# Ben-Bussch/Lunar_Module_Ascent_Trajectory_Optimiser

Measured on AMD Instinct MI355X. Metric: solved ascent NLPs/sec (N=200 collocation nodes), higher is better.
Workload: dtype f64; 1 GPU; BASELINE.json configs[2]: 4096-NLP Isp x dry-mass sweep (64x64, Isp 300-320 s, dry mass 2345-2545 kg), N=200 nodes, backward Euler (reference NODES=2), DCOST applied (the script's MV move penalty 1e-05, Launch_Optimiser.py:99, as an l1 term: the model the reference declares); move_penalty=True, batch_per_gpu=4096, global_batch=4096, n_nodes=200, parallelism=problem-sharded x1, gather only, converged=4096, of=4096

## Files before the change

### include/ascent.h

```cpp
#ifndef ASCENT_H
#define ASCENT_H
#include <stdint.h>

#ifdef __cplusplus
extern "C" {
#endif

typedef struct ascent_params {
  double G;
  double M;
  double R0;
  double Ft;
  double M0;
  double mdot;
  double fuel_mass;
  double mass_scalar;
  double ang_acc_max;
  double r_peri;
  double r_apo;
  double T_scale;
  double angle_ub;
  double tf_lb;
  double tf_ub;
  double dcost;
} ascent_params;

typedef struct ascent_opts {
  int32_t n_nodes;
  int32_t scheme;
  int32_t max_iter;
  int32_t warm_start;
  double tol;
  double mu_init;
  int32_t formulation;
  int32_t coarse_nodes;
  int32_t terminal;
  int32_t solver_path;
  int32_t move_penalty;
  int32_t reserved;
} ascent_opts;

enum ascent_status {
  ASCENT_OK = 0,
  ASCENT_E_ARG = -1,
  ASCENT_E_HIP = -2,
  ASCENT_E_NODEVICE = -3,
  ASCENT_E_NOMEM = -4,
  ASCENT_E_NOTERM = -5
};

enum ascent_problem_status {
  ASCENT_CONVERGED = 0,
  ASCENT_MAX_ITER = 1,
  ASCENT_LINESEARCH_FAILED = 2,
  ASCENT_REGULARISATION_FAILED = 3
};

#define ASCENT_BLOB_ROWS(n_nodes) (21 * ((n_nodes) - 1) + 10)
#define ASCENT_TRAJ_FIELDS 10

int ascent_version(void);
int ascent_device_count(void);
const char *ascent_strerror(int code);

int ascent_solve_batch(const ascent_params *p, int64_t batch, const ascent_opts *o,
                       const double *guess_or_null, double *traj_out, double *tf_out,
                       int32_t *status_out, int32_t *iters_out, double *sol_blob_out_or_null,
                       int device_id, void *hip_stream_or_null, int ptr_is_device);

int ascent_eval_nodes(const ascent_params *p, int64_t batch, const ascent_opts *o,
                      const double *iterate, double *defects, double *jac_blocks,
                      double *hess_blocks, int device_id);

int ascent_kkt_step(const ascent_params *p, int64_t batch, const ascent_opts *o,
                    const double *iterate, const double *mu, const double *delta_w, double *step,
                    int32_t *inertia_out, int device_id);

enum ascent_path { ASCENT_PATH_AUTO = 0, ASCENT_PATH_FUSED = 1, ASCENT_PATH_SPLIT_LANE = 2, ASCENT_PATH_SPLIT_WIDE = 3,
                   ASCENT_PATH_DENSE = 4,
                   ASCENT_PATH_PERSIST = 5  };
int ascent_default_path(int64_t batch, const ascent_opts *o);
int ascent_workspace_layout(int64_t batch, const ascent_opts *o, int64_t *out4);
int ascent_eval_nodes_path(const ascent_params *p, int64_t batch, const ascent_opts *o,
                           const double *iterate, double *defects, double *jac_blocks,
                           double *hess_blocks, int device_id, int path);
int ascent_kkt_step_path(const ascent_params *p, int64_t batch, const ascent_opts *o,
                         const double *iterate, const double *mu, const double *delta_w, double *step,
                         int32_t *inertia_out, int device_id, int path);

int ascent_dense_records(const ascent_params *p, int64_t batch, const ascent_opts *o, const double *iterate,
                         double *records, int device_id);

int ascent_coast_batch(const ascent_params *p, int64_t batch, const double *final_state, int32_t coast_nodes,
                       double *coast_traj, double *coast_tf, double *apsides, int device_id,
                       void *hip_stream_or_null, int ptr_is_device);

int ascent_param_sensitivity(const ascent_params *p, int64_t batch, const ascent_opts *o,
                             const double *sol_blob, double *grad_out,
                             int device_id, void *hip_stream_or_null, int ptr_is_device);

#define ASCENT_FLIGHT_ROWS 10
#define ASCENT_FLIGHT_MAX_SUBSTEPS 4096
int ascent_fly_batch(const ascent_params *p, int64_t batch, const ascent_opts *o, const double *sol_blob,
                     int32_t substeps, double *flown_traj_out_or_null, double *local_err_out_or_null,
                     double *summary_out, int device_id, void *hip_stream_or_null, int ptr_is_device);

int ascent_flight_jacobian(const ascent_params *p, int64_t batch, const ascent_opts *o, const double *sol_blob,
                           int32_t substeps, double *jac_out, double *jac_u_out_or_null, int device_id,
                           void *hip_stream_or_null, int ptr_is_device);

#define ASCENT_TRIM_ROWS 10
int ascent_trim_batch(const ascent_params *p, int64_t batch, const ascent_opts *o, const double *sol_blob, int32_t substeps,
                      int32_t rounds, double tol, double *trim_blob_out, double *summary_out, int device_id,
                      void *hip_stream_or_null, int ptr_is_device);

#define ASCENT_DISPERSE_COLS 24
#define ASCENT_DISPERSE_ROWS 9
#define ASCENT_DISPERSE_STAT_ROWS 82
#define ASCENT_DISPERSE_MAX_SAMPLES 65536
int ascent_disperse_batch(const ascent_params *p, int64_t batch, const ascent_opts *o, const double *sol_blob,
                          int32_t substeps, int32_t samples, const double *xi, const double *sigma,
                          const double *sigma_u_or_null, double *stats_out, double *samples_out_or_null, int device_id,
                          void *hip_stream_or_null, int ptr_is_device);

#define ASCENT_GUIDE_ROWS 5
int ascent_guidance_gains(const ascent_params *p, int64_t batch, const ascent_opts *o, const double *sol_blob, int32_t substeps,
                          const double *weights, double *gain_u_out, double *gain_t_out, double *summary_out,
                          double *jac_cl_out_or_null, double *jac_u_cl_out_or_null, int device_id, void *hip_stream_or_null,
                          int ptr_is_device);

#define ASCENT_GUIDED_SAMPLE_ROWS 12
int ascent_disperse_guided_batch(const ascent_params *p, int64_t batch, const ascent_opts *o, const double *sol_blob,
                                 int32_t substeps, int32_t samples, const double *xi, const double *sigma,
                                 const double *sigma_u_or_null, const double *gain_u, const double *gain_t_or_null,
                                 const double *stretch_max_or_null, double *stats_out, double *samples_out_or_null,
                                 int device_id, void *hip_stream_or_null, int ptr_is_device);

int ascent_kkt_solve(int64_t batch, int32_t n_nodes, int32_t bs, int32_t nb, const double *diag, const double *lower,
                     const double *upper, const double *border, const double *border_diag, const double *rhs,
                     double *sol, int device_id, int algo);

double ascent_last_kernel_ms(int device_id);

#ifdef __cplusplus
}
#endif
#endif
```

### lunar_module_ascent_trajectory_optimiser_amd/csrc/ascent_dense.hip

```cpp
#include <hip/hip_runtime.h>

#include <cstdio>
#include <cstdlib>

#include "ascent.h"
#include "ascent_device.hpp"
#include "ascent_tile.hpp"
#include "ascent_dense.hpp"
#include "ascent_blocktri.hpp"
#include "ascent_flight_dev.hpp"

using namespace ascent;

namespace {

constexpr int NIT = 26;
constexpr int O_Z = 0, O_U = 7, O_L = 8, O_ZB = 15;
constexpr int O_LU = 21, O_PP = 22, O_PN = 23, O_ZP = 24, O_ZN = 25;
constexpr int NV_GA = 0, NV_GB = 8, NV_P = 16, NNV = 27;
constexpr int G_JA = 0, G_JB = 1, G_HAA = 2, G_HAB = 3, G_HBB = 4, G_V = 5, NGRID = 6;
constexpr int F_EA = 0, F_LA = 1, F_EL2 = 2, F_GAIN = 3;
constexpr int FWD_DOUBLES = 3 * 64 + 16;
enum {
  X_STATE, X_ITERS, X_STATUS, X_CUR, X_FIRST, X_LS, X_MU, X_NUP, X_DWL, X_ALPHA, X_ADU, X_PHI0, X_DM, X_C1, X_SL,
  X_S,
  X_D = X_S + 10,
  X_T = X_D + 10,
  X_REFAC = X_T + 10, X_RTH, X_DW, X_MV,
  NSCAL = 64
};
enum { ST_TRIAL = 0, ST_NEWTON = 1, ST_DONE = 3 };

struct DGeo {
  int K, scheme, terminal, dc;
  __host__ __device__ size_t nlp_doubles() const {
    return (size_t)K * (3 * NIT + NNV + NGRID * 64 + FWD_DOUBLES) + NSCAL;
  }
  __host__ __device__ size_t off_it(int buf) const { return (size_t)buf * NIT * K; }
  __host__ __device__ size_t off_st() const { return (size_t)2 * NIT * K; }
  __host__ __device__ size_t off_nv() const { return (size_t)3 * NIT * K; }
  __host__ __device__ size_t off_rec() const { return (size_t)(3 * NIT + NNV) * K; }
  __host__ __device__ size_t off_fwd() const { return off_rec() + (size_t)K * NGRID * 64; }
  __host__ __device__ size_t off_sc() const { return off_fwd() + (size_t)K * FWD_DOUBLES; }
};

ASC_DEV Scal load_scal(const double *sc, int r0) {
  Scal s;
  s.th = sc[r0 + S_TH]; s.zlt = sc[r0 + S_ZLT]; s.zut = sc[r0 + S_ZUT]; s.s1 = sc[r0 + S_S1]; s.s2 = sc[r0 + S_S2];
  s.zs1 = sc[r0 + S_ZS1]; s.zs2 = sc[r0 + S_ZS2]; s.nu3 = sc[r0 + S_NU3]; s.nu1 = sc[r0 + S_NU1]; s.nu2 = sc[r0 + S_NU2];
  return s;
}
ASC_DEV void store_scal(double *sc, int r0, const Scal &s) {
  sc[r0 + S_TH] = s.th; sc[r0 + S_ZLT] = s.zlt; sc[r0 + S_ZUT] = s.zut; sc[r0 + S_S1] = s.s1; sc[r0 + S_S2] = s.s2;
  sc[r0 + S_ZS1] = s.zs1; sc[r0 + S_ZS2] = s.zs2; sc[r0 + S_NU3] = s.nu3; sc[r0 + S_NU1] = s.nu1; sc[r0 + S_NU2] = s.nu2;
}
ASC_DEV Scal trial_scal(const Der &d, const Scal &s, const Scal &ds, double alpha, double adu, double mu, bool first) {
  Scal t = s;
  if (first) return t;
  t.th += alpha * ds.th; t.s1 += alpha * ds.s1; t.s2 += alpha * ds.s2;
  t.nu3 += alpha * ds.nu3; t.nu1 += alpha * ds.nu1; t.nu2 += alpha * ds.nu2;
  t.zlt = clipz(s.zlt + adu * ds.zlt, t.th - d.tlb, mu);
  t.zut = clipz(s.zut + adu * ds.zut, d.tub - t.th, mu);
  t.zs1 = clipz(s.zs1 + adu * ds.zs1, t.s1, mu);
  t.zs2 = clipz(s.zs2 + adu * ds.zs2, t.s2, mu);
  return t;
}

__global__ __launch_bounds__(WAVE) void d_init(const ascent_params *params, long batch, DGeo g, double *ws,
                                               const double *guess, int warm, double mu_init, int probe,
                                               const double *probe_mu) {
  const long p = blockIdx.y;
  const int k = blockIdx.x * WAVE + threadIdx.x, K = g.K;
  if (k >= K) return;
  double *w = ws + (size_t)p * g.nlp_doubles();
  const Der d = derive_t(params[p], g.terminal);
  const int asked_warm = warm;
  if (warm && !(guess[(21L * K + S_TH) * batch + p] > 0.0)) warm = 0;
  const double tf0 = 0.9, dr = 0.166, aend = 0.5, vp = sqrt(d.vp2), dt0 = (1.0 / K) * d.T * tf0;
  const double sdr = sin(dr), cdr = cos(dr);
  const double xf = -d.rhof * sdr, yf = d.rhof * cdr - d.rho0;
  double z[7], l[7], zb[6], u;
  if (warm) {
    ASC_UNROLL
    for (int i = 0; i < 7; i++) {
      z[i] = guess[(7L * k + i) * batch + p];
      l[i] = guess[(8L * K + 7L * k + i) * batch + p];
    }
    u = guess[(7L * K + k) * batch + p];
    ASC_UNROLL
    for (int b = 0; b < 6; b++) zb[b] = guess[(15L * K + 6L * k + b) * batch + p];
  } else {
    const double fr = (double)(k + 1) / K;
    z[IX] = fr * xf; z[IY] = fr * yf; z[IVX] = -fr * vp * cdr; z[IVY] = -fr * vp * sdr; z[IA] = fr * aend;
    z[IW] = aend / (K * dt0); z[IM] = d.mrate * dt0 * (k + 1);
    u = 0.0;
  }
  if (!probe) {
    z[IA] = push_in(z[IA], 0.0, d.aub);
    z[IM] = push_in(z[IM], 0.0, 1.0);
    u = push_in(u, -1.0, 1.0);
  }
  ASC_UNROLL
  for (int b = 0; b < 6; b++) zb[b] = warm == 2 ? (probe ? zb[b] : fmax(zb[b], 1e-12)) : 1.0;
  ASC_UNROLL
  for (int i = 0; i < 7; i++) l[i] = warm == 2 ? l[i] : 0.0;
  double *it = w + g.off_it(0), *st = w + g.off_st();
  ASC_UNROLL
  for (int i = 0; i < 7; i++) { it[(O_Z + i) * K + k] = z[i]; it[(O_L + i) * K + k] = l[i]; }
  it[O_U * K + k] = u;
  ASC_UNROLL
  for (int b = 0; b < 6; b++) it[(O_ZB + b) * K + k] = zb[b];
  for (int r = 0; r < NIT; r++) st[r * K + k] = 0.0;
  if (g.dc) {
    double up = (k > 0 && warm) ? guess[(7L * K + k - 1) * batch + p] : 0.0;
    if (k > 0 && !probe) up = push_in(up, -1.0, 1.0);
    const double dl = u - up, eps = warm ? 1e-4 : 1e-2, dc = params[p].dcost;
    it[O_LU * K + k] = 0.0;
    it[O_PP * K + k] = fmax(dl, 0.0) + eps; it[O_PN * K + k] = fmax(-dl, 0.0) + eps;
    it[O_ZP * K + k] = dc; it[O_ZN * K + k] = dc;
  }
  if (k != K - 1) return;
  double *sc = w + g.off_sc();
  Scal s;
  if (warm) {
    const double *gs = guess + (21L * K) * batch + p;
    s.th = gs[S_TH * batch]; s.zlt = gs[S_ZLT * batch]; s.zut = gs[S_ZUT * batch]; s.s1 = gs[S_S1 * batch];
    s.s2 = gs[S_S2 * batch]; s.zs1 = gs[S_ZS1 * batch]; s.zs2 = gs[S_ZS2 * batch]; s.nu3 = gs[S_NU3 * batch];
    s.nu1 = gs[S_NU1 * batch]; s.nu2 = gs[S_NU2 * batch];
  } else {
    s.th = tf0;
  }
  if (!probe) s.th = push_in(s.th, d.tlb, d.tub);
  const Terminal tm = terminal_of(d, z);
  if (probe) {
  } else if (warm != 2) {
    s.s1 = fmax(tm.g1, 1e-2); s.s2 = fmax(tm.g2, 1e-2);
    s.zlt = s.zut = s.zs1 = s.zs2 = 1.0;
    s.nu3 = s.nu1 = s.nu2 = 0.0;
  } else {
    s.s1 = fmax(s.s1, 1e-10); s.s2 = fmax(s.s2, 1e-10);
    s.zlt = fmax(s.zlt, 1e-12); s.zut = fmax(s.zut, 1e-12);
    s.zs1 = fmax(s.zs1, 1e-12); s.zs2 = fmax(s.zs2, 1e-12);
  }
  for (int r = 0; r < NSCAL; r++) sc[r] = 0.0;
  store_scal(sc, X_S, s);
  sc[X_STATE] = ST_TRIAL; sc[X_FIRST] = 1.0; sc[X_STATUS] = ASCENT_MAX_ITER;
  sc[X_MU] = probe ? probe_mu[p] : ((asked_warm && !warm) ? 0.1 : mu_init);
  sc[X_NUP] = 1.0;
}

struct QMap { int q; double c; };

ASC_DEV void h4_full(const double *H10, double H4[4][4]) {
  H4[0][0] = H10[0]; H4[0][1] = H4[1][0] = H10[1]; H4[0][2] = H4[2][0] = H10[2]; H4[0][3] = H4[3][0] = H10[3];
  H4[1][1] = H10[4]; H4[1][2] = H4[2][1] = H10[5]; H4[1][3] = H4[3][1] = H10[6];
  H4[2][2] = H10[7]; H4[2][3] = H4[3][2] = H10[8]; H4[3][3] = H10[9];
}

__global__ __launch_bounds__(WAVE) void d_eval(const ascent_params *params, long batch, DGeo g, double *ws) {
  const long p = blockIdx.y;
  const int k = blockIdx.x * WAVE + threadIdx.x, K = g.K;
  double *w = ws + (size_t)p * g.nlp_doubles();
  double *sc = w + g.off_sc();
  if ((int)sc[X_STATE] != ST_TRIAL || k >= K) return;
  const Der d = derive_t(params[p], g.terminal);
  const bool first = sc[X_FIRST] != 0.0;
  const double alpha = first ? 0.0 : sc[X_ALPHA], adu = first ? 0.0 : sc[X_ADU], mu = sc[X_MU];
  const Scal s = load_scal(sc, X_S), ds = load_scal(sc, X_D);
  const Scal stt = trial_scal(d, s, ds, alpha, adu, mu, first);
  const int cur = (int)sc[X_CUR];
  const double *ic = w + g.off_it(cur), *st = w + g.off_st();
  double *in = w + g.off_it(1 - cur), *nv = w + g.off_nv(), *rec = w + g.off_rec() + (size_t)k * NGRID * 64;
  const double hT = (1.0 / K) * d.T, dt = hT * stt.th;
  const double wa = g.scheme == 0 ? 0.0 : g.scheme == 1 ? 0.5 : 1.0 / 6.0;
  const double wm = g.scheme == 2 ? 4.0 / 6.0 : 0.0;
  const double wb = g.scheme == 0 ? 1.0 : g.scheme == 1 ? 0.5 : 1.0 / 6.0;
  const double sa = dt * wa, sm = dt * wm, sb = dt * wb, e8 = 0.125 * dt, h8 = 0.125 * hT;
  double za[7], zb[7], lam[7], zbd[6], u;
  ASC_UNROLL
  for (int i = 0; i < 7; i++) {
    zb[i] = ic[(O_Z + i) * K + k] + alpha * st[(O_Z + i) * K + k];
    za[i] = k ? ic[(O_Z + i) * K + k - 1] + alpha * st[(O_Z + i) * K + k - 1] : 0.0;
    lam[i] = ic[(O_L + i) * K + k] + alpha * st[(O_L + i) * K + k];
  }
  u = ic[O_U * K + k] + alpha * st[O_U * K + k];
  const double dist[6] = {zb[IA], d.aub - zb[IA], zb[IM], 1.0 - zb[IM], u + 1.0, 1.0 - u};
  const double mlo = mu * 1e-10, mhi = mu * 1e10;
  ASC_UNROLL
  for (int b = 0; b < 6; b++) {
    double v = ic[(O_ZB + b) * K + k];
    if (!first) { const double id = rcp(dist[b]); v = fmin(fmax(v + adu * st[(O_ZB + b) * K + k], mlo * id), mhi * id); }
    zbd[b] = v;
    in[(O_ZB + b) * K + k] = v;
  }
  ASC_UNROLL
  for (int i = 0; i < 7; i++) { in[(O_Z + i) * K + k] = zb[i]; in[(O_L + i) * K + k] = lam[i]; }
  in[O_U * K + k] = u;
  double lu = 0.0, pp = 1.0, pn = 1.0, zp = 0.0, zn = 0.0, cu = 0.0;
  if (g.dc) {
    const double up = k ? ic[O_U * K + k - 1] + alpha * st[O_U * K + k - 1] : 0.0;
    lu = ic[O_LU * K + k] + alpha * st[O_LU * K + k];
    pp = ic[O_PP * K + k] + alpha * st[O_PP * K + k];
    pn = ic[O_PN * K + k] + alpha * st[O_PN * K + k];
    zp = ic[O_ZP * K + k]; zn = ic[O_ZN * K + k];
    if (!first) {
      const double ip = rcp(pp), in_ = rcp(pn);
      zp = fmin(fmax(zp + adu * st[O_ZP * K + k], mlo * ip), mhi * ip);
      zn = fmin(fmax(zn + adu * st[O_ZN * K + k], mlo * in_), mhi * in_);
    }
    in[O_LU * K + k] = lu; in[O_PP * K + k] = pp; in[O_PN * K + k] = pn; in[O_ZP * K + k] = zp; in[O_ZN * K + k] = zn;
    cu = u - up - pp + pn;
  }
  if (k == K - 1) store_scal(sc, X_T, stt);
  double Ga[8], Gb[8], Gm[8], Hw[10], fa[7], fb[7], fm[7], zm[7], ax, ay;
  ASC_UNROLL
  for (int i = 0; i < 8; i++) { Ga[i] = 0.0; Gm[i] = 0.0; }
  ASC_UNROLL
  for (int i = 0; i < 7; i++) { fa[i] = 0.0; fm[i] = 0.0; zm[i] = 0.0; }
  accel<1>(d, zb[IX], zb[IY], zb[IA], zb[IM], 0.0, 0.0, ax, ay, Gb, nullptr);
  rhs_f(d, zb, u, ax, ay, fb);
  if (g.scheme != 0) {
    accel<1>(d, za[IX], za[IY], za[IA], za[IM], 0.0, 0.0, ax, ay, Ga, nullptr);
    rhs_f(d, za, u, ax, ay, fa);
  }
  double H4m[4][4];
  ASC_UNROLL
  for (int i = 0; i < 4; i++) {
    ASC_UNROLL
    for (int j = 0; j < 4; j++) H4m[i][j] = 0.0;
  }
  double gm[7], mth[7];
  ASC_UNROLL
  for (int i = 0; i < 7; i++) { gm[i] = 0.0; mth[i] = 0.0; }
  if (g.scheme == 2) {
    ASC_UNROLL
    for (int i = 0; i < 7; i++) { mth[i] = h8 * (fa[i] - fb[i]); zm[i] = 0.5 * (za[i] + zb[i]) + e8 * (fa[i] - fb[i]); }
    accel<2>(d, zm[IX], zm[IY], zm[IA], zm[IM], lam[IVX], lam[IVY], ax, ay, Gm, Hw);
    rhs_f(d, zm, u, ax, ay, fm);
    h4_full(Hw, H4m);
    fzt_lambda(Gm, lam, gm);
  }
  double H4a[4][4], H4b[4][4];
  {
    double t1, t2, Gx[8];
    accel<2>(d, zb[IX], zb[IY], zb[IA], zb[IM], sb * lam[IVX] - sm * e8 * gm[IVX], sb * lam[IVY] - sm * e8 * gm[IVY], t1, t2, Gx, Hw);
    h4_full(Hw, H4b);
    if (g.scheme != 0) {
      accel<2>(d, za[IX], za[IY], za[IA], za[IM], sa * lam[IVX] + sm * e8 * gm[IVX], sa * lam[IVY] + sm * e8 * gm[IVY], t1, t2, Gx, Hw);
      h4_full(Hw, H4a);
    } else {
      ASC_UNROLL
      for (int i = 0; i < 4; i++) {
        ASC_UNROLL
        for (int j = 0; j < 4; j++) H4a[i][j] = 0.0;
      }
    }
  }
  const QMap qa[7] = {{0, 0.5}, {1, 0.5}, {0, e8}, {1, e8}, {2, 0.5}, {2, e8}, {3, 0.5}};
  const QMap qb[7] = {{0, 0.5}, {1, 0.5}, {0, -e8}, {1, -e8}, {2, 0.5}, {2, -e8}, {3, 0.5}};
  constexpr int q2s[4] = {IX, IY, IA, IM};
  double c[7], Jth[7], Hath[7], Hbth[7], ga[7], gb[7], t7[7], t7b[7];
  double Hmm[4];
  {
    const double mq[4] = {mth[IX], mth[IY], mth[IA], mth[IM]};
    ASC_UNROLL
    for (int i = 0; i < 4; i++) Hmm[i] = H4m[i][0] * mq[0] + H4m[i][1] * mq[1] + H4m[i][2] * mq[2] + H4m[i][3] * mq[3];
  }
  fz_mul(Gm, mth, t7);
  double c1 = 0.0, cinf = 0.0;
  ASC_UNROLL
  for (int i = 0; i < 7; i++) {
    c[i] = zb[i] - za[i] - dt * (wa * fa[i] + wm * fm[i] + wb * fb[i]);
    Jth[i] = -hT * (wa * fa[i] + wm * fm[i] + wb * fb[i]) - sm * t7[i];
    c1 += fabs(c[i]);
    cinf = fmax(cinf, fabs(c[i]));
  }
  double Fal[7], Fbl[7], Fag[7], Fbg[7];
  fzt_lambda(Ga, lam, Fal); fzt_lambda(Gb, lam, Fbl); fzt_lambda(Ga, gm, Fag); fzt_lambda(Gb, gm, Fbg);
  double rth = 0.0, mHm = 0.0, gmm = 0.0;
  ASC_UNROLL
  for (int i = 0; i < 7; i++) {
    const double Mag = 0.5 * gm[i] + e8 * Fag[i], Mbg = 0.5 * gm[i] - e8 * Fbg[i];
    ga[i] = -lam[i] - sa * Fal[i] - sm * Mag;
    gb[i] = lam[i] - sb * Fbl[i] - sm * Mbg;
    const double MaHm = qa[i].c * Hmm[qa[i].q], MbHm = qb[i].c * Hmm[qb[i].q];
    Hath[i] = -hT * (wa * Fal[i] + wm * Mag) - sm * (h8 * Fag[i] + MaHm);
    Hbth[i] = -hT * (wb * Fbl[i] + wm * Mbg) - sm * (-h8 * Fbg[i] + MbHm);
    rth += Jth[i] * lam[i];
    gmm += gm[i] * mth[i];
  }
  mHm = mth[IX] * Hmm[0] + mth[IY] * Hmm[1] + mth[IA] * Hmm[2] + mth[IM] * Hmm[3];
  (void)t7b;
  const double Hthth = -2.0 * hT * wm * gmm - sm * mHm;
  const double Huth = -hT * d.alpha * lam[IW];
  if (g.dc) { c1 += fabs(cu); cinf = fmax(cinf, fabs(cu)); }
  auto frow = [&](const double *G, int r, double *row) __attribute__((always_inline)) {
    ASC_UNROLL
    for (int j = 0; j < 7; j++) row[j] = 0.0;
    if (r == IX) row[IVX] = 1.0;
    if (r == IY) row[IVY] = 1.0;
    if (r == IVX) { row[IX] = G[0]; row[IY] = G[1]; row[IA] = G[2]; row[IM] = G[3]; }
// ... 1100 lines not shown
```

### lunar_module_ascent_trajectory_optimiser_amd/csrc/ascent_persist.hip

```cpp
#include <hip/hip_runtime.h>

#pragma clang fp contract(on)

#include <cstdio>
#include <cstdlib>

#include "ascent.h"
#include "ascent_device.hpp"
#include "ascent_tile.hpp"
#include "ascent_persist.hpp"
#include "ascent_persist_dev.hpp"

using namespace ascent;

namespace {


ASC_DEV void start_move(double *w, int Kp, int k, double u, double up, bool warm, double dcw) {
  const double dl = u - up, eps = warm ? 1e-4 : 1e-2;
  w[(R_IT + O_LU) * Kp + k] = 0.0;
  w[(R_IT + O_PP) * Kp + k] = fmax(dl, 0.0) + eps;
  w[(R_IT + O_PN) * Kp + k] = fmax(-dl, 0.0) + eps;
  w[(R_IT + O_ZP) * Kp + k] = dcw;
  w[(R_IT + O_ZN) * Kp + k] = dcw;
}
struct MovePivot { double ip, in_, sgp, sgn, rp, rn, Rd, gdl; };
ASC_DEV MovePivot move_pivot(double pp, double pn, double zp, double zn, double lu, double dcw, double mu, double dw) {
  MovePivot m;
  m.ip = rcp(pp); m.in_ = rcp(pn);
  m.sgp = zp * m.ip + dw; m.sgn = zn * m.in_ + dw;
  m.rp = dcw - mu * m.ip - lu; m.rn = dcw - mu * m.in_ + lu;
  const double isp = rcp(m.sgp), isn = rcp(m.sgn);
  m.Rd = rcp(isp + isn);
  m.gdl = m.Rd * (m.rp * isp - m.rn * isn);
  return m;
}

ASC_DEV void start_node(const Der &d, int K, int kk, int warm, bool probe, int form, double *z, double *l, double *zb, double &u) {
  if (!warm) {
    const double tf0 = 0.9, dr = 0.166, aend = 0.5, vp = sqrt(d.vp2), dt0 = (1.0 / K) * d.T * tf0;
    const double sdr = sin(dr), cdr = cos(dr);
    const double xf = -d.rhof * sdr, yf = d.rhof * cdr - d.rho0;
    const double fr = (double)(kk + 1) / K;
    z[IX] = fr * xf; z[IY] = fr * yf; z[IVX] = -fr * vp * cdr; z[IVY] = -fr * vp * sdr; z[IA] = fr * aend;
    z[IW] = aend / (K * dt0); z[IM] = d.mrate * dt0 * (kk + 1);
    u = 0.0;
    if (form == 1) {
      z[IW] = 0.0;
      u = z[IA] / (0.5 * d.aub) - 1.0;
    }
  }
  if (!probe) {
    z[IA] = push_in(z[IA], 0.0, d.aub);
    z[IM] = push_in(z[IM], 0.0, 1.0);
    u = push_in(u, -1.0, 1.0);
  }
  ASC_UNROLL
  for (int b = 0; b < 6; b++) zb[b] = probe ? zb[b] : warm == 2 ? fmax(zb[b], 1e-12) : 1.0;
  ASC_UNROLL
  for (int i = 0; i < 7; i++) l[i] = warm == 2 ? l[i] : 0.0;
}
ASC_DEV void start_scal(const Der &d, int warm, bool probe, const double *zK, Scal &s) {
  if (!warm) s.th = 0.9;
  if (!probe) s.th = push_in(s.th, d.tlb, d.tub);
  const Terminal tm = terminal_of(d, zK);
  if (probe) {
  } else if (warm != 2) {
    s.s1 = fmax(tm.g1, 1e-2); s.s2 = fmax(tm.g2, 1e-2);
    s.zlt = s.zut = s.zs1 = s.zs2 = 1.0;
    s.nu3 = s.nu1 = s.nu2 = 0.0;
  } else {
    s.s1 = fmax(s.s1, 1e-10); s.s2 = fmax(s.s2, 1e-10);
    s.zlt = fmax(s.zlt, 1e-12); s.zut = fmax(s.zut, 1e-12);
    s.zs1 = fmax(s.zs1, 1e-12); s.zs2 = fmax(s.zs2, 1e-12);
  }
}
ASC_DEV void store_start(double *w, int Kp, int k, const double *z, const double *l, const double *zb, double u) {
  ASC_UNROLL
  for (int i = 0; i < 7; i++) { w[(R_IT + O_Z + i) * Kp + k] = z[i]; w[(R_IT + O_L + i) * Kp + k] = l[i]; }
  w[(R_IT + O_U) * Kp + k] = u;
  ASC_UNROLL
  for (int b = 0; b < 6; b++) w[(R_IT + O_ZB + b) * Kp + k] = zb[b];
}

__global__ __launch_bounds__(WAVE) void p_init(const ascent_params *params, long batch, PGeo g, double *ws, const double *guess,
                                               int warm, double mu_init, const double *probe_mu, const double *probe_dw, int probe_kind) {
  const long p = blockIdx.y;
  const int k = blockIdx.x * WAVE + threadIdx.x, K = g.K, Kp = g.Kp;
  if (k >= Kp) return;
  double *w = ws + (size_t)p * g.nlp_doubles();
  const Der d = derive_t(params[p], g.term);
  const int asked_warm = warm;
  if (warm && !(guess[(21L * K + S_TH) * batch + p] > 0.0)) warm = 0;
  const bool probe = probe_mu != nullptr;
  double z[7], l[7], zb[6], u = 0.0;
  const int kk = k < K ? k : K - 1;
  if (warm) {
    ASC_UNROLL
    for (int i = 0; i < 7; i++) { z[i] = guess[(7L * kk + i) * batch + p]; l[i] = guess[(8L * K + 7L * kk + i) * batch + p]; }
    u = guess[(7L * K + kk) * batch + p];
    ASC_UNROLL
    for (int b = 0; b < 6; b++) zb[b] = guess[(15L * K + 6L * kk + b) * batch + p];
  }
  start_node(d, K, kk, warm, probe, g.form, z, l, zb, u);
  store_start(w, Kp, k, z, l, zb, u);
  if (g.mp) {
    const double ha = 0.5 * d.aub, f0 = (double)kk / K * 0.5;
    double up = kk == 0 ? (g.form == 1 ? -1.0 : 0.0) : warm ? guess[(7L * K + kk - 1) * batch + p] : (g.form == 1 ? f0 / ha - 1.0 : 0.0);
    if (kk > 0 && !probe) up = push_in(up, -1.0, 1.0);
    start_move(w, Kp, k, u, up, warm != 0, g.form == 1 ? params[p].dcost * ha : params[p].dcost);
  }
  if (k != K - 1) return;
  double *sc = w + (size_t)g.nrows() * Kp;
  Scal s;
  if (warm) {
    const double *gs = guess + (21L * K) * batch + p;
    s.th = gs[S_TH * batch]; s.zlt = gs[S_ZLT * batch]; s.zut = gs[S_ZUT * batch]; s.s1 = gs[S_S1 * batch];
    s.s2 = gs[S_S2 * batch]; s.zs1 = gs[S_ZS1 * batch]; s.zs2 = gs[S_ZS2 * batch]; s.nu3 = gs[S_NU3 * batch];
    s.nu1 = gs[S_NU1 * batch]; s.nu2 = gs[S_NU2 * batch];
  }
  start_scal(d, warm, probe, z, s);
  for (int r = 0; r < NSCAL; r++) sc[r] = 0.0;
  put_scal(sc, X_S, s);
  sc[X_STATE] = ST_TRIAL; sc[X_FIRST] = 1.0; sc[X_STATUS] = ASCENT_MAX_ITER;
  sc[X_MU] = (asked_warm && !warm) ? 0.1 : mu_init; sc[X_NUP] = 1.0;
  if (probe) { sc[X_MU] = probe_mu[p]; sc[X_PDW] = probe_dw[p]; sc[X_PROBE] = (double)probe_kind; }
}

__global__ __launch_bounds__(WAVE) void p_transfer(const ascent_params *params, long batch, PGeo gc, const double *wsc, PGeo gf,
                                                   double *wsf, double mu) {
  const long p = blockIdx.y;
  const int k = blockIdx.x * WAVE + threadIdx.x, Kc = gc.K, Kf = gf.K, Kpc = gc.Kp, Kpf = gf.Kp;
  if (k >= Kpf) return;
  const double *wc = wsc + (size_t)p * gc.nlp_doubles(), *scc = wc + (size_t)gc.nrows() * Kpc;
  double *wf = wsf + (size_t)p * gf.nlp_doubles();
  const Der d = derive_t(params[p], gf.term);
  const int warm = (int)scc[X_STATUS] == ASCENT_CONVERGED ? 2 : 0;
  const double *ic = wc + (size_t)((int)scc[X_CUR] * gc.nit()) * Kpc;
  double z[7], l[7], zb[6], u = 0.0, up = 0.0;
  const int kk = k < Kf ? k : Kf - 1;
  if (warm && gf.mp && kk > 0) {
    const double x = (double)kk / (double)Kf * (double)Kc;
    int j = (int)x;
    if (j > Kc - 1) j = Kc - 1;
    const double wt = x - (double)j;
    const int ja = j ? j - 1 : 0;
    const double a = ic[O_U * Kpc + ja], b = ic[O_U * Kpc + j];
    up = push_in(fma(wt, b - a, a), -1.0, 1.0);
  }
  if (warm) {
    const double x = (double)(kk + 1) / (double)Kf * (double)Kc;
    int j = (int)x;
    if (j > Kc - 1) j = Kc - 1;
    const double wt = x - (double)j;
    const int ja = j ? j - 1 : 0;
    const double zsc = (double)Kc / (double)Kf;
    ASC_UNROLL
    for (int i = 0; i < 7; i++) {
      const double a = j ? ic[(O_Z + i) * Kpc + ja] : ((gf.form == 1 && i == IA) ? ic[(O_Z + i) * Kpc] : 0.0), b = ic[(O_Z + i) * Kpc + j];
      z[i] = fma(wt, b - a, a);
      const double la = ic[(O_L + i) * Kpc + ja], lb = ic[(O_L + i) * Kpc + j];
      l[i] = fma(wt, lb - la, la);
    }
    { const double a = ic[O_U * Kpc + ja], b = ic[O_U * Kpc + j]; u = fma(wt, b - a, a); }
    ASC_UNROLL
    for (int b6 = 0; b6 < 6; b6++) {
      const double a = ic[(O_ZB + b6) * Kpc + ja], b = ic[(O_ZB + b6) * Kpc + j];
      zb[b6] = fma(wt, b - a, a) * zsc;
    }
  }
  start_node(d, Kf, kk, warm, false, gf.form, z, l, zb, u);
  store_start(wf, Kpf, k, z, l, zb, u);
  if (gf.mp) {
    if (kk == 0) up = gf.form == 1 ? -1.0 : 0.0;
    else if (!warm && gf.form == 1) up = push_in((double)kk / Kf * 0.5 / (0.5 * d.aub) - 1.0, -1.0, 1.0);
    start_move(wf, Kpf, k, u, up, warm != 0, gf.form == 1 ? params[p].dcost * 0.5 * d.aub : params[p].dcost);
  }
  if (k != Kf - 1) return;
  double *sc = wf + (size_t)gf.nrows() * Kpf;
  Scal s;
  if (warm) s = lds_scal(scc, X_S);
  start_scal(d, warm, false, z, s);
  for (int r = 0; r < NSCAL; r++) sc[r] = 0.0;
  put_scal(sc, X_S, s);
  sc[X_STATE] = ST_TRIAL; sc[X_FIRST] = 1.0; sc[X_STATUS] = ASCENT_MAX_ITER;
  sc[X_MU] = warm ? mu : 0.1; sc[X_NUP] = 1.0;
  sc[X_ITB] = scc[X_ITB] + scc[X_ITERS];
}

constexpr int FIN_WAVES = 8, FIN_SUB = CH / FIN_WAVES;
__global__ __launch_bounds__(WAVE * FIN_WAVES) void p_finish(const ascent_params *params, long batch, PGeo g, const double *ws, double *traj,
                                                 double *tf_out, int *status_out, int *iters_out, double *blob) {
  const long p = (long)blockIdx.y * WAVE + threadIdx.x;
  if (p >= batch) return;
  const int c = blockIdx.x, K = g.K, Kp = g.Kp, nt = K + 1;
  const double *w = ws + (size_t)p * g.nlp_doubles();
  const double *sc = w + (size_t)g.nrows() * Kp;
  const Der d = derive_t(params[p], g.term);
  const double *it = w + (size_t)((int)sc[X_CUR] * g.nit()) * Kp;
  if (c == 0 && threadIdx.y == 0) {
    const Scal s = lds_scal(sc, X_S);
    tf_out[p] = s.th;
    status_out[p] = (int)sc[X_STATUS];
    iters_out[p] = (int)sc[X_ITERS] + (int)sc[X_ITB];
    if (blob) {
      double *bs = blob + (21L * K) * batch + p;
      bs[S_TH * batch] = s.th; bs[S_ZLT * batch] = s.zlt; bs[S_ZUT * batch] = s.zut; bs[S_S1 * batch] = s.s1;
      bs[S_S2 * batch] = s.s2; bs[S_ZS1 * batch] = s.zs1; bs[S_ZS2 * batch] = s.zs2; bs[S_NU3 * batch] = s.nu3;
      bs[S_NU1 * batch] = s.nu1; bs[S_NU2 * batch] = s.nu2;
    }
    if (traj) {
      double ax, ay;
      accel<0>(d, 0.0, 0.0, 0.0, 0.0, 0.0, 0.0, ax, ay, nullptr, nullptr);
      const double v[10] = {0.0, 0.0, 0.0, 0.0, ax, ay, 0.0, 0.0, 0.0, 0.0};
      ASC_UNROLL
      for (int f = 0; f < 10; f++) traj[((long)f * nt) * batch + p] = v[f];
    }
  }
  for (int k = c * CH + threadIdx.y * FIN_SUB; k < min(K, c * CH + (threadIdx.y + 1) * FIN_SUB); k++) {
    double z[7];
    ASC_UNROLL
    for (int q = 0; q < 7; q++) z[q] = it[(O_Z + q) * Kp + k];
    const double u = it[O_U * Kp + k];
    if (blob) {
      ASC_UNROLL
      for (int q = 0; q < 7; q++) {
        blob[(7L * k + q) * batch + p] = z[q];
        blob[(8L * K + 7L * k + q) * batch + p] = it[(O_L + q) * Kp + k];
      }
      blob[(7L * K + k) * batch + p] = u;
      ASC_UNROLL
      for (int b = 0; b < 6; b++) blob[(15L * K + 6L * k + b) * batch + p] = it[(O_ZB + b) * Kp + k];
    }
    if (traj) {
      double ax, ay;
      accel<0>(d, z[IX], z[IY], z[IA], z[IM], 0.0, 0.0, ax, ay, nullptr, nullptr);
      const double v[10] = {z[IX], z[IY], z[IVX], z[IVY], ax, ay, z[IA], z[IW], u, z[IM]};
      ASC_UNROLL
      for (int f = 0; f < 10; f++) traj[((long)f * nt + k + 1) * batch + p] = v[f];
    }
  }
}

__global__ __launch_bounds__(WAVE) void p_probe_out(long batch, PGeo g, const double *ws, double *step, int *inertia) {
  const long p = blockIdx.y;
  const int k = blockIdx.x * WAVE + threadIdx.x, K = g.K, Kp = g.Kp;
  if (k >= K) return;
  const double *w = ws + (size_t)p * g.nlp_doubles();
  const double *sc = w + (size_t)g.nrows() * Kp, *stp = w + (size_t)g.r_st() * Kp;
  const bool ok = (int)sc[X_STATE] == ST_TRIAL;
  if (k == 0) {
    inertia[p] = ok ? 0 : 1;
    for (int r = 0; r < 10; r++) step[(21L * K + r) * batch + p] = ok ? sc[X_D + r] : 0.0;
  }
  ASC_UNROLL
  for (int i = 0; i < 7; i++) {
    step[(7L * k + i) * batch + p] = ok ? stp[(O_Z + i) * Kp + k] : 0.0;
    step[(8L * K + 7L * k + i) * batch + p] = ok ? stp[(O_L + i) * Kp + k] : 0.0;
  }
  step[(7L * K + k) * batch + p] = ok ? stp[O_U * Kp + k] : 0.0;
  ASC_UNROLL
  for (int b = 0; b < 6; b++) step[(15L * K + 6L * k + b) * batch + p] = ok ? stp[(O_ZB + b) * Kp + k] : 0.0;
}

__global__ __launch_bounds__(WAVE) void p_probe_rows_out(const ascent_params *params, long batch, PGeo g, const double *ws, double *defects,
                                                         double *jac, double *hess) {
  const long p = blockIdx.y;
  const int k = blockIdx.x * WAVE + threadIdx.x, K = g.K, Kp = g.Kp;
  if (k >= K) return;
  const double *w = ws + (size_t)p * g.nlp_doubles();
  const double *sc = w + (size_t)g.nrows() * Kp, *rows = w + (size_t)g.r_st() * Kp;
  const double *it = w + (size_t)((int)sc[X_CUR] * g.nit()) * Kp;
  const Der d = derive_t(params[p], g.term);
  const double a_ = it[(O_Z + IA) * Kp + k], m_ = it[(O_Z + IM) * Kp + k];
  const double siga = it[(O_ZB + 0) * Kp + k] * rcp(a_) + it[(O_ZB + 1) * Kp + k] * rcp(d.aub - a_);
  const double sigm = it[(O_ZB + 2) * Kp + k] * rcp(m_) + it[(O_ZB + 3) * Kp + k] * rcp(1.0 - m_);
  ASC_UNROLL
  for (int i = 0; i < 8; i++) jac[(8L * k + i) * batch + p] = rows[i * Kp + k];
  ASC_UNROLL
  for (int i = 0; i < 10; i++) hess[(10L * k + i) * batch + p] = rows[(8 + i) * Kp + k] - (i == 7 ? siga : i == 9 ? sigm : 0.0);
  ASC_UNROLL
  for (int i = 0; i < 7; i++) defects[(7L * k + i) * batch + p] = rows[(18 + i) * Kp + k];
}


template <int FORM>
ASC_DEV void ainv_vrows(const double *G, const double *E, double dt, double *rvx, double *rvy) {
  double c1[7], c2[7];
  c1[IX] = dt * G[0]; c1[IY] = dt * G[1]; c1[IVX] = 1.0; c1[IVY] = 0.0; c1[IA] = dt * G[2]; c1[IW] = FORM == 1 ? 0.0 : dt * c1[IA]; c1[IM] = dt * G[3];
  c2[IX] = dt * G[4]; c2[IY] = dt * G[5]; c2[IVX] = 0.0; c2[IVY] = 1.0; c2[IA] = dt * G[6]; c2[IW] = FORM == 1 ? 0.0 : dt * c2[IA]; c2[IM] = dt * G[7];
  ASC_UNROLL
  for (int i = 0; i < 7; i++) { rvx[i] = E[0] * c1[i] + E[1] * c2[i]; rvy[i] = E[2] * c1[i] + E[3] * c2[i]; }
}


struct TrialKeep { double G[8], F[7], dza, dzm, zb4, zb5, zpp, zpn; };

template <int SCHEME, int FORM, int MP = 0, int TERM = 0>
ASC_DEV void trial_primal(const Der &d, int K, int Kp, int k, const NodeIn &n, const NodeIn &dn, const TrialCtx &t, bool live,
                          double *in, Part &P, TrialKeep &kp) {
  const double alpha = t.alpha;
  double z[7], zp[7], zb[6];
  ASC_UNROLL
  for (int i = 0; i < 7; i++) { z[i] = n.z[i] + alpha * dn.z[i]; zp[i] = n.zp[i] + alpha * dn.zp[i]; }
  const double u = n.u + alpha * dn.u;
  const double dist[6] = {z[IA], d.aub - z[IA], z[IM], 1.0 - z[IM], u + 1.0, 1.0 - u};
  ASC_UNROLL
  for (int b = 0; b < 6; b++) {
    const double id = rcp(dist[b]);
    zb[b] = t.first ? n.zb[b] : fmin(fmax(n.zb[b] + t.adu * dn.zb[b], t.mlo * id), t.mhi * id);
  }
  if (live) {
    ASC_UNROLL
    for (int i = 0; i < 7; i++) in[(O_Z + i) * Kp + k] = z[i];
    in[O_U * Kp + k] = u;
    ASC_UNROLL
    for (int b = 0; b < 6; b++) in[(O_ZB + b) * Kp + k] = zb[b];
  }
  kp.zpp = 0.0; kp.zpn = 0.0;
  if constexpr (MP) {
    const double up = n.up + alpha * dn.up, pp = n.pp + alpha * dn.pp, pn = n.pn + alpha * dn.pn;
    const double ip = rcp(pp), in_ = rcp(pn);
    const double zpp = t.first ? n.zpp : fmin(fmax(n.zpp + t.adu * dn.zpp, t.mlo * ip), t.mhi * ip);
    const double zpn = t.first ? n.zpn : fmin(fmax(n.zpn + t.adu * dn.zpn, t.mlo * in_), t.mhi * in_);
    if (live) { in[O_PP * Kp + k] = pp; in[O_PN * Kp + k] = pn; in[O_ZP * Kp + k] = zpp; in[O_ZN * Kp + k] = zpn; }
    const double cu = u - up - pp + pn;
    P.c1 += fabs(cu);
    P.cinf = fmax(P.cinf, fabs(cu));
    const double prp = pp * zpp, prn = pn * zpn;
    P.pmin = fmin(P.pmin, fmin(prp, prn)); P.pmax = fmax(P.pmax, fmax(prp, prn));
    P.zsum += zpp + zpn;
    P.mv += pp + pn;
    const double ps = pp * pn;
    P.sl += ps > 0.0 ? log(ps) : NAN;
    kp.zpp = zpp; kp.zpn = zpn;
  }
  double ax, ay;
  accel<1>(d, z[IX], z[IY], z[IA], z[IM], 0.0, 0.0, ax, ay, kp.G, nullptr);
  rhs_f<FORM>(d, z, u, ax, ay, kp.F);
  if (SCHEME == 1) {
    double Fb[7], axp, ayp;
    accel<0>(d, zp[IX], zp[IY], zp[IA], zp[IM], 0.0, 0.0, axp, ayp, nullptr, nullptr);
    rhs_f<FORM>(d, zp, u, axp, ayp, Fb);
    ASC_UNROLL
    for (int i = 0; i < 7; i++) kp.F[i] = 0.5 * (kp.F[i] + Fb[i]);
  }
  ASC_UNROLL
  for (int i = 0; i < 7; i++) {
    const double cc = (FORM == 1 && i == IA) ? z[IA] - 0.5 * d.aub * (u + 1.0) : z[i] - zp[i] - t.dt * kp.F[i];
    P.c1 += fabs(cc);
    P.cinf = fmax(P.cinf, fabs(cc));
  }
  if (k == K - 1) {
    const Scal &stt = t.stt;
    const Terminal tt = TERM == 2 ? terminal_eval_any(d, z) : terminal_eval(d, z);
    const double e1 = fabs(tt.e3), e2 = fabs(tt.g1 - stt.s1), e3 = fabs(tt.g2 - stt.s2);
    P.cinf = fmax(P.cinf, fmax(e1, fmax(e2, e3)));
    P.c1 += e1 + e2 + e3;
    const double ps = ((stt.th - d.tlb) * (d.tub - stt.th)) * (stt.s1 * stt.s2);
    P.sl += ps > 0.0 ? log(ps) : NAN;
  }
  ASC_UNROLL
  for (int b = 0; b < 6; b++) { const double pr = dist[b] * zb[b]; P.pmin = fmin(P.pmin, pr); P.pmax = fmax(P.pmax, pr); P.zsum += zb[b]; }
  const double pa = dist[0] * dist[1], pm = dist[2] * dist[3], pu = dist[4] * dist[5];
  P.sl += (pa > 0.0 && pm > 0.0 && pu > 0.0) ? log(pa * pm * pu) : NAN;
  kp.dza = zb[1] - zb[0]; kp.dzm = zb[3] - zb[2]; kp.zb4 = zb[4]; kp.zb5 = zb[5];
}

template <int SCHEME, int FORM, int MP = 0, int TERM = 0>
ASC_DEV void trial_dual(const Der &d, int K, int Kp, int k, const TrialKeep &kp, const double *l, const double *ln, double lu, double lun,
                        const TrialCtx &t, bool live, double *in, Part &P) {
  if (live) {
    ASC_UNROLL
    for (int i = 0; i < 7; i++) in[(O_L + i) * Kp + k] = l[i];
    if constexpr (MP) in[O_LU * Kp + k] = lu;
  }
  if constexpr (MP) {
    P.l1 += fabs(lu);
    P.rd = fmax(P.rd, fmax(fabs(t.dcw - lu - kp.zpp), fabs(t.dcw + lu - kp.zpn)));
  }
  const double cs = SCHEME == 1 ? 0.5 * t.dt : t.dt;
  double fl[7], lt[7];
  ASC_UNROLL
  for (int i = 0; i < 7; i++) lt[i] = SCHEME == 1 ? l[i] + ln[i] : l[i];
  fzt_lambda<FORM>(kp.G, lt, fl);
  double r[7];
  ASC_UNROLL
  for (int i = 0; i < 7; i++) {
    r[i] = (FORM == 1 && i == IA) ? l[i] - cs * fl[i] : l[i] - cs * fl[i] - ln[i];
    P.rth -= t.hT * kp.F[i] * l[i];
    P.l1 += fabs(l[i]);
  }
  r[IA] += kp.dza;
  r[IM] += kp.dzm;
  if (k == K - 1) {
    const Scal &stt = t.stt;
    double z[7];
    ASC_UNROLL
    for (int i = 0; i < 7; i++) z[i] = in[(O_Z + i) * Kp + k];
    if constexpr (TERM == 2) {
      const Terminal tt = terminal_eval_any(d, z);
      double g4[4];
      terminal_grad_any(tt, stt.nu1, stt.nu2, g4);
      r[IX] += g4[0]; r[IY] += g4[1]; r[IVX] += g4[2]; r[IVY] += g4[3];
    } else {
      const Terminal tt = terminal_eval(d, z);
      r[IX] += stt.nu3 * tt.e3g[0] + stt.nu1 * tt.g1g[0];
      r[IY] += stt.nu3 * tt.e3g[1] + stt.nu1 * tt.g1g[1];
      r[IVX] += stt.nu3 * tt.e3g[2] + stt.nu2 * tt.g2g[0];
      r[IVY] += stt.nu3 * tt.e3g[3] + stt.nu2 * tt.g2g[1];
    }
  }
  ASC_UNROLL
  for (int i = 0; i < 7; i++) P.rd = fmax(P.rd, fabs(r[i]));
  double ruv = (FORM == 1 ? -0.5 * d.aub * l[IA] : -t.be * l[IW]) - kp.zb4 + kp.zb5;
  if constexpr (MP) ruv += lu - lun;
  P.rd = fmax(P.rd, fabs(ruv));
}

template <int SCHEME, int FORM, int MP = 0, int TERM = 0>
ASC_DEV void trial_node(const Der &d, int K, int Kp, int k, const NodeIn &n, const NodeIn &dn, const TrialCtx &t, bool live,
                        double *in, Part &P) {
  TrialKeep kp;
  trial_primal<SCHEME, FORM, MP, TERM>(d, K, Kp, k, n, dn, t, live, in, P, kp);
  double l[7], ln[7];
  ASC_UNROLL
  for (int i = 0; i < 7; i++) { l[i] = n.l[i] + t.alpha * dn.l[i]; ln[i] = n.ln[i] + t.alpha * dn.ln[i]; }
  const double lu = MP ? n.lu + t.alpha * dn.lu : 0.0, lun = MP ? n.lun + t.alpha * dn.lun : 0.0;
  trial_dual<SCHEME, FORM, MP, TERM>(d, K, Kp, k, kp, l, ln, lu, lun, t, live, in, P);
}


template <int SCHEME, int FORM, int MP = 0, int TERM = 0, int WIDE = 0>
__global__ __launch_bounds__(WAVE) void p_solve(const ascent_params *params, long batch, PGeo g, double *ws, int max_iter, double tol) {
  using L = Lay<MP>;
  constexpr int NS = L::NS, NIT = L::NIT, R_ST = L::R_ST, R_KA = L::R_KA, R_K0 = L::R_K0, NROWS = L::NROWS;
  constexpr int S_G = L::S_G, S_E = L::S_E, S_H = L::S_H, S_F = L::S_F, S_C = L::S_C, S_RZ = L::S_RZ, S_GT = L::S_GT, S_SC = L::S_SC;
  constexpr int RL = NS;
  static_assert(FORM == 0 || SCHEME == 0, "the v1 formulation is restated with backward Euler");
  __shared__ double stage[L::S_ROWS * LDW];
  __shared__ double outb[L::OUT_ROWS * LDW];
  __shared__ double lds_t[NPW][NS][NS];
  __shared__ double lds_d[NPW][3][8];
  __shared__ double lsc[NPW][NSCAL];
  __shared__ double lds_c[NPW][8];
  constexpr int CHN = WIDE ? 64 : CH;
  const int lane = threadIdx.x, grp = lane >> 4, role = lane & 15;
  const int nl = WIDE ? lane : role;
  const int cbase = WIDE ? 0 : grp * 16;
  const long p = WIDE ? (long)blockIdx.x : (long)blockIdx.x * NPW + grp;
  const bool live = p < batch;
  const long pc = live ? p : batch - 1;
  const int K = g.K, Kp = g.Kp, nch = g.nch;
  double *w = ws + (size_t)pc * g.nlp_doubles();
  double *gsc = w + (size_t)NROWS * Kp;
  double *sc = lsc[WIDE ? 0 : grp];
  const Der d = TERM == 2 ? derive_t(params[pc], 2) : derive(params[pc]);
  static_assert(TERM == 0 || (TERM == 2 && FORM == 0), "terminal 2 is carried for the current formulation");
  for (int r = role; r < NSCAL; r += 16) sc[r] = gsc[r];
  if (role < 8) lds_d[grp][2][role] = 0.0;
  wsync();
  if (!live && role == 0) sc[X_STATE] = ST_DONE;
  wsync();
  const int col = grp * 16 + role;
  const double hT = (1.0 / K) * d.T;
  constexpr int IB = FORM == 1 ? IA : IW;
  const double dcw = MP ? (FORM == 1 ? params[pc].dcost * 0.5 * d.aub : params[pc].dcost) : 0.0;
  constexpr double UINIT = FORM == 1 ? -1.0 : 0.0;

  PROF_DECL
  for (int round = 0; round < 64 * (max_iter + 2); round++) {
    PROF(9);
    int state = (int)sc[X_STATE];
    if (__all(state == ST_DONE)) break;
    int pass = 0;
    do {
      if (state == ST_TRIAL) {
        const bool first = sc[X_FIRST] != 0.0;
        const double alpha = first ? 0.0 : sc[X_ALPHA], adu = first ? 0.0 : sc[X_ADU], mu = sc[X_MU];
        const Scal s = lds_scal(sc, X_S), ds = lds_scal(sc, X_D);
        const Scal stt = trial_scal(d, s, ds, alpha, adu, mu, first);
        const int cur = (int)sc[X_CUR];
        const double *ic = w + (size_t)(cur * NIT) * Kp, *stp = w + (size_t)R_ST * Kp;
        double *in = w + (size_t)((1 - cur) * NIT) * Kp;
        const double dt = hT * stt.th, be = dt * d.alpha;
        const double mlo = mu * 1e-10, mhi = mu * 1e10;
        Part P;
        if (sc[X_TEVAL] != 0.0) {
          P.rd = sc[X_P + 0]; P.cinf = sc[X_P + 1]; P.pmin = sc[X_P + 2]; P.pmax = sc[X_P + 3]; P.l1 = sc[X_P + 4];
          P.zsum = sc[X_P + 5]; P.rth = sc[X_P + 6]; P.c1 = sc[X_P + 7]; P.sl = sc[X_P + 8]; P.mv = sc[X_P + 9];
        } else {
          TrialCtx t;
          t.alpha = alpha; t.adu = adu; t.mlo = mlo; t.mhi = mhi; t.dt = dt; t.be = be; t.hT = hT; t.first = first; t.stt = stt; t.dcw = dcw;
          P.clear();
          for (int c = 0; c < nch; c++) {
            const int k = c * CHN + nl;
            if (k < K) {
              NodeIn n, dn;
              load_node<MP>(ic, Kp, K, k, n, UINIT);
              if (first) dn = NodeIn{};
              else load_node<MP>(stp, Kp, K, k, dn);
              trial_node<SCHEME, FORM, MP, TERM>(d, K, Kp, k, n, dn, t, live, in, P);
            }
          }
          P.template reduceW<MP, WIDE>();
        }
        double rd = P.rd, cinf = P.cinf, pmin = P.pmin, pmax = P.pmax, l1 = P.l1, zsum = P.zsum;
        const double rth = 1.0 + P.rth, c1 = P.c1, sl = P.sl;
        double nu_pen = sc[X_NUP], iters = sc[X_ITERS], mu2 = mu;
        int nstate = ST_FACTOR;
        bool accepted = true;
        if (!first) {
          const double phi0 = sc[X_PHI0], Dm = sc[X_DM];
          const double phit = (MP ? stt.th + dcw * P.mv : stt.th) - mu * sl + nu_pen * c1;
          if (!(isfinite(phit) && phit <= phi0 + 1e-8 * alpha * Dm + 2.220446049250313e-15 * fabs(phi0))) {
            accepted = false;
            const int ls = (int)sc[X_LS] + 1;
            wsync();
            if (role == 0) {
              sc[X_LS] = ls; sc[X_TEVAL] = 0.0;
              if (ls >= 40) { sc[X_STATUS] = ASCENT_LINESEARCH_FAILED; sc[X_STATE] = ST_DONE; }
              else sc[X_ALPHA] = 0.5 * alpha;
            }
          } else {
            iters += 1.0;
          }
        }
        if (accepted) {
          ErrParts e;
          e.rd = fmax(rd, fabs(rth - stt.zlt + stt.zut));
          e.rd = fmax(e.rd, fmax(fabs(-stt.nu1 - stt.zs1), fabs(-stt.nu2 - stt.zs2)));
          e.cinf = cinf;
          const double pr[4] = {(stt.th - d.tlb) * stt.zlt, (d.tub - stt.th) * stt.zut, stt.s1 * stt.zs1, stt.s2 * stt.zs2};
          ASC_UNROLL
          for (int q = 0; q < 4; q++) { pmin = fmin(pmin, pr[q]); pmax = fmax(pmax, pr[q]); }
          e.pmin = pmin; e.pmax = pmax;
          l1 += fabs(stt.nu3) + fabs(stt.nu1) + fabs(stt.nu2);
          zsum += stt.zlt + stt.zut + stt.zs1 + stt.zs2;
          e.sd = fmax(100.0, (l1 + zsum) / (double)((MP ? 16 : 13) * K + 7)) * 0.01;
          int status = -1;
          const bool probe = sc[X_PROBE] != 0.0;
          if (probe) { }
          else if (e.err(0.0) <= tol) { status = ASCENT_CONVERGED; nstate = ST_DONE; }
          else if ((int)iters >= max_iter) { status = ASCENT_MAX_ITER; nstate = ST_DONE; }
          else {
            while (mu2 > tol * 0.1 && e.err(mu2) <= 10.0 * mu2) {
              mu2 = fmax(tol * 0.1, fmin(0.2 * mu2, mu2 * sqrt(mu2)));
              nu_pen = 1.0;
            }
          }
#ifdef PERSIST_TRACE
          if (role == 0 && p == PERSIST_TRACE && K > 100)
            printf("[persist] K=%d iter %2d mu %.1e E0 %.2e (dual %.1e primal %.1e compl %.1e..%.1e s_d %.2g) alpha %.3g adu %.3g ls %d dw %.1e nu_pen %.2g c1 %.2e\n", K, (int)iters, mu,
                   e.err(0.0), e.rd, e.cinf, e.pmin, e.pmax, e.sd, alpha, adu, (int)sc[X_LS], sc[X_DWL], nu_pen, c1);
          if (role == 0 && p == PERSIST_TRACE && K > 100)
            printf("[persist]      dual rows: nodes %.2e | th %.2e s1 %.2e s2 %.2e\n", rd, fabs(rth - stt.zlt + stt.zut), fabs(-stt.nu1 - stt.zs1), fabs(-stt.nu2 - stt.zs2));
#endif
          wsync();
          if (role == 0) {
            put_scal(sc, X_S, stt);
            sc[X_CUR] = 1 - cur; sc[X_FIRST] = 0.0; sc[X_ITERS] = iters; sc[X_LS] = 0.0; sc[X_C1] = c1; sc[X_SL] = sl; sc[X_RTH] = rth;
            sc[X_MU] = mu2; sc[X_NUP] = nu_pen; sc[X_DW] = probe ? sc[X_PDW] : 0.0; sc[X_STATE] = nstate; sc[X_TEVAL] = 0.0;
            if (MP) sc[X_MV] = P.mv;
            if (status >= 0) sc[X_STATUS] = status;
          }
        }
      }
      wsync();
      state = (int)sc[X_STATE];
    } while (__builtin_expect(__any(state == ST_TRIAL) && ++pass < 41, 0));
    PROF(0);
    state = (int)sc[X_STATE];
    if (__any(state == ST_FACTOR)) {
      const bool act = state == ST_FACTOR;
      const Scal s = lds_scal(sc, X_S);
      const double mu = sc[X_MU], dw = sc[X_DW];
      const double *it = w + (size_t)((int)sc[X_CUR] * NIT) * Kp;
      const double dt = hT * s.th, be = dt * d.alpha, ith = rcp(s.th), cs = SCHEME == 1 ? 0.5 * dt : dt;
      const double ha = 0.5 * d.aub, bu = FORM == 1 ? ha : be;
      const double hTc = SCHEME == 1 ? 0.5 * hT : hT;
      int grow[NS];
      double gsgn[NS];
      {
        constexpr int hmap[8] = {0, 1, -1, -1, 2, -1, 3, -1};
        constexpr int hrow[4][4] = {{0, 1, 2, 3}, {1, 4, 5, 6}, {2, 5, 7, 8}, {3, 6, 8, 9}};
        ASC_UNROLL
        for (int i = 0; i < NS; i++) {
          int row = S_H; double sgn = 0.0;
          if (role < 7) {
            ASC_UNROLL
            for (int c = 0; c < 7; c++)
              if (c == role && hmap[i] >= 0 && hmap[c] >= 0) { row = S_H + hrow[hmap[i]][hmap[c]]; sgn = 1.0; }
          } else if (MP && role == 7) { if (i == 7) { row = S_SC; sgn = 1.0; } }
          else if (role == RL) { row = S_RZ + i; sgn = -1.0; }
          else if (role == RL + 1) { row = S_GT + i; sgn = -1.0; }
          grow[i] = row * LDW;
          gsgn[i] = sgn;
        }
      }
      const double bsc = role == RL ? -mu : 0.0;
      const int rowA = (role < 8 ? S_G + role : role < 12 ? S_E + role - 8
                        : MP ? (role == 12 ? S_SC + 1 : role == 13 ? S_SC + 2 : S_SC)
                        : (role == 12 ? S_SC : role == 13 ? S_SC + 1 : role == 14 ? S_SC + 4 : S_SC + 2)) * LDW;
      const int rowB = (role < 7 ? S_C + role
                        : MP ? (role < 13 ? S_F + role - 7 : role == 15 ? S_C + 7 : S_SC)
                        : (role < 14 ? S_F + role - 7 : role == 14 ? S_SC + 3 : S_SC)) * LDW;
      const int rowK = (role < NS + 3 ? role : NS + 3) * LDW;
      const bool colr = role < NS;
      const int drow = role == RL ? 0 : role == RL + 1 ? 1 : 2;
      double a[NS];
      ASC_UNROLL
      for (int i = 0; i < NS; i++) a[i] = 0.0;
      double U = 0.0, V = 0.0, k10 = 0.0, k11 = 0.0, k12 = 0.0, k20 = 0.0, k22 = 0.0;
      int bad = 0;
      double zK[7];
      ASC_UNROLL
      for (int i = 0; i < 7; i++) zK[i] = it[(O_Z + i) * Kp + K - 1];
      const Terminal tm = TERM == 2 ? terminal_eval_any(d, zK) : terminal_eval(d, zK);
      const double is1 = rcp(s.s1), is2 = rcp(s.s2);
      const double sig1 = s.zs1 * is1 + dw, sig2 = s.zs2 * is2 + dw;
      const double rs1 = -mu * is1 - s.nu1, rs2 = -mu * is2 - s.nu2;
      {
        const double cg1 = tm.g1 - s.s1, cg2 = tm.g2 - s.s2;
        double Qt[28];
        ASC_UNROLL
        for (int i = 0; i < 28; i++) Qt[i] = 0.0;
        if constexpr (TERM == 2) terminal_hessian_any(Qt, tm, s.nu1, s.nu2, sig1, sig2);
        else terminal_hessian(Qt, tm, s.nu3, s.nu1, s.nu2, sig1, sig2);
        const double w1 = s.nu1 + sig1 * cg1 + rs1, w2 = s.nu2 + sig2 * cg2 + rs2;
        double r0[4] = {s.nu3 * tm.e3g[0] + w1 * tm.g1g[0], s.nu3 * tm.e3g[1] + w1 * tm.g1g[1],
                        s.nu3 * tm.e3g[2] + w2 * tm.g2g[0], s.nu3 * tm.e3g[3] + w2 * tm.g2g[1]};
        if constexpr (TERM == 2) terminal_grad_any(tm, w1, w2, r0);
        ASC_UNROLL
        for (int i = 0; i < 7; i++) {
          double v = 0.0;
          ASC_UNROLL
          for (int c = 0; c < 7; c++) v = role == c ? Qt[sid(i, c)] : v;
          if (i < 4) { v = role == RL ? -r0[i] : v; v = role == RL + 2 ? -tm.e3g[i] : v; }
          a[i] = v;
        }
      }
      const bool probe_rows = sc[X_PROBE] == 2.0;
      for (int c = nch - 1; c >= 0; c--) {
        {
          const int k = c * CHN + nl;
          if (k < K && act) {
            NodeIn n;
            load_node<MP>(it, Kp, K, k, n, UINIT);
            double G[8], E[4], H[10], F[7], fl[7], lt[7], ax, ay;
            ASC_UNROLL
            for (int i = 0; i < 7; i++) lt[i] = SCHEME == 1 ? n.l[i] + n.ln[i] : n.l[i];
            accel<2>(d, n.z[IX], n.z[IY], n.z[IA], n.z[IM], -cs * lt[IVX], -cs * lt[IVY], ax, ay, G, H);
            rhs_f<FORM>(d, n.z, n.u, ax, ay, F);
            if (SCHEME == 1) {
              double Fb[7], axp, ayp;
              accel<0>(d, n.zp[IX], n.zp[IY], n.zp[IA], n.zp[IM], 0.0, 0.0, axp, ayp, nullptr, nullptr);
              rhs_f<FORM>(d, n.zp, n.u, axp, ayp, Fb);
              ASC_UNROLL
              for (int i = 0; i < 7; i++) F[i] = 0.5 * (F[i] + Fb[i]);
            }
            implicit_block(G, cs, E);
            fzt_lambda<FORM>(G, lt, fl);
            const double dist[6] = {n.z[IA], d.aub - n.z[IA], n.z[IM], 1.0 - n.z[IM], n.u + 1.0, 1.0 - n.u};
            double id[6];
            ASC_UNROLL
            for (int b = 0; b < 6; b++) id[b] = rcp(dist[b]);
            H[7] += n.zb[0] * id[0] + n.zb[1] * id[1];
            H[9] += n.zb[2] * id[2] + n.zb[3] * id[3];
            ASC_UNROLL
            for (int i = 0; i < 8; i++) stage[(S_G + i) * LDW + col] = G[i];
            ASC_UNROLL
            for (int i = 0; i < 4; i++) stage[(S_E + i) * LDW + col] = E[i];
            ASC_UNROLL
            for (int i = 0; i < 10; i++) stage[(S_H + i) * LDW + col] = H[i];
            ASC_UNROLL
            for (int i = 0; i < 7; i++) {
              if (!MP || i != IM) stage[(S_F + i) * LDW + col] = hT * F[i];
              stage[(S_C + i) * LDW + col] = (FORM == 1 && i == IA) ? n.z[IA] - ha * (n.u + 1.0) : n.z[i] - n.zp[i] - dt * F[i];
              stage[(S_RZ + i) * LDW + col] = (FORM == 1 && i == IA) ? n.l[i] - cs * fl[i] : n.l[i] - cs * fl[i] - n.ln[i];
              stage[(S_GT + i) * LDW + col] = -hTc * fl[i];
            }
            const double scr[5] = {n.zb[4] * id[4] + n.zb[5] * id[5], FORM == 1 ? -ha * n.l[IA] : -be * n.l[IW], id[1] - id[0], id[3] - id[2],
                                   id[5] - id[4]};
            if constexpr (MP) {
              const MovePivot mvp = move_pivot(n.pp, n.pn, n.zpp, n.zpn, n.lu, dcw, mu, dw);
              stage[(S_C + 7) * LDW + col] = n.u - n.up - n.pp + n.pn;
              stage[(S_RZ + 7) * LDW + col] = (scr[1] + (n.lu - n.lun)) + mu * scr[4];
              stage[(S_GT + 7) * LDW + col] = FORM == 1 ? 0.0 : -hT * d.alpha * n.l[IW];
              stage[S_SC * LDW + col] = scr[0];
              stage[(S_SC + 1) * LDW + col] = mvp.Rd;
              stage[(S_SC + 2) * LDW + col] = mvp.gdl;
              stage[(S_RZ + IA) * LDW + col] += mu * scr[2];
              stage[(S_RZ + IM) * LDW + col] += mu * scr[3];
            } else {
              ASC_UNROLL
              for (int i = 0; i < 5; i++) stage[(S_SC + i) * LDW + col] = scr[i];
            }
          }
        }
        wsync();
        PROF(1);
        if (probe_rows) {
          const int k = c * CHN + nl;
          if (k < K && act && live) {
            ASC_UNROLL
            for (int i = 0; i < 8; i++) w[(size_t)(R_ST + i) * Kp + k] = stage[(S_G + i) * LDW + col];
            ASC_UNROLL
            for (int i = 0; i < 10; i++) w[(size_t)(R_ST + 8 + i) * Kp + k] = stage[(S_H + i) * LDW + col];
            ASC_UNROLL
            for (int i = 0; i < 7; i++) w[(size_t)(R_ST + 18 + i) * Kp + k] = stage[(S_C + i) * LDW + col];
          }
          wsync();
          continue;
        }
        if (act) {
          for (int jj = CHN - 1; jj >= 0; jj--) {
            const int k = c * CHN + jj;
            if (k >= K) continue;
            const int cj = cbase + jj;
            double gq[NS];
            ASC_UNROLL
            for (int i = 0; i < NS; i++) gq[i] = stage[grow[i] + cj];
            const double gA = stage[rowA + cj], gB = stage[rowB + cj];
            const double G[8] = {bcast16<0>(gA), bcast16<1>(gA), bcast16<2>(gA), bcast16<3>(gA),
                                 bcast16<4>(gA), bcast16<5>(gA), bcast16<6>(gA), bcast16<7>(gA)};
            const double E[4] = {bcast16<8>(gA), bcast16<9>(gA), bcast16<10>(gA), bcast16<11>(gA)};
            const double R0 = bcast16<12>(gA), ru0 = bcast16<13>(gA), bur = bcast16<14>(gA);
            const double bza = bcast16<15>(gA), bzm = bcast16<14>(gB);
            const double cc[8] = {bcast16<0>(gB), bcast16<1>(gB), bcast16<2>(gB), bcast16<3>(gB),
                                  bcast16<4>(gB), bcast16<5>(gB), bcast16<6>(gB), MP ? bcast16<15>(gB) : 0.0};
            const double rc1[7] = {bcast16<7>(gB), bcast16<8>(gB), bcast16<9>(gB), bcast16<10>(gB), bcast16<11>(gB),
                                   bcast16<12>(gB), MP ? hT * d.mrate : bcast16<13>(gB)};
            if (FORM == 1 && k < K - 1) {
              a[IA] = 0.0;
              if (role == IA) {
                ASC_UNROLL
                for (int i = 0; i < NS; i++) a[i] = 0.0;
              }
            }
            if (SCHEME == 1 && k < K - 1) {
              double t[7];
              fzt_lambda(G, a, t);
              ASC_UNROLL
              for (int i = 0; i < 7; i++) a[i] += cs * t[i];
              if (colr) {
                ASC_UNROLL
                for (int i = 0; i < NS; i++) lds_t[grp][role][i] = a[i];
                wsync();
                double r[NS];
                ASC_UNROLL
                for (int l2 = 0; l2 < NS; l2++) r[l2] = lds_t[grp][l2][role];
                fzt_lambda(G, r, t);
                ASC_UNROLL
                for (int i = 0; i < 7; i++) a[i] = r[i] + cs * t[i];
                if constexpr (MP) a[7] = r[7];
              }
              wsync();
            }
            ASC_UNROLL
            for (int i = 0; i < NS; i++) a[i] += gsgn[i] * gq[i];
            if constexpr (!MP) {
              a[IA] += bsc * bza;
              a[IM] += bsc * bzm;
            }
            if (dw != 0.0) {
              ASC_UNROLL
              for (int i = 0; i < NS; i++) a[i] += role == i ? dw : 0.0;
            }
            double b[NS];
            solveAT<FORM>(G, E, cs, a, b);
            if constexpr (MP) b[7] = a[7] + bu * b[IB];
            if (colr) {
              ASC_UNROLL
              for (int i = 0; i < NS; i++) lds_t[grp][role][i] = b[i];
              wsync();
              double t[NS];
              ASC_UNROLL
              for (int l2 = 0; l2 < NS; l2++) t[l2] = lds_t[grp][l2][role];
              solveAT<FORM>(G, E, cs, t, b);
              if constexpr (MP) b[7] = t[7] + bu * b[IB];
            }
            double mw[NS], D, coef;
            if constexpr (MP) {
              ASC_UNROLL
              for (int i = 0; i < NS; i++) mw[i] = bcast16<7>(b[i]);
              D = R0 + mw[7];
            } else {
              ASC_UNROLL
              for (int i = 0; i < NS; i++) mw[i] = bu * bcast16<IB>(b[i]);
              D = R0 + dw + bu * mw[IB];
            }
            const double iD = rcp(D);
            if constexpr (MP) {
              const double rsel = role == RL ? ru0 : 0.0;
              coef = (b[7] - rsel) * iD;
            } else {
              const double ru = ru0 + mu * bur, gu = FORM == 1 ? 0.0 : ru0 * ith;
              const double rsel = role == 7 ? ru : role == 8 ? gu : 0.0;
              coef = (bu * b[IB] - rsel) * iD;
            }
            ASC_UNROLL
            for (int i = 0; i < NS; i++) a[i] = b[i] - mw[i] * coef;
            outb[rowK + cj] = role < NS + 3 ? coef : D;
            if (colr) {
              double d0 = 0.0, d1 = 0.0;
              ASC_UNROLL
              for (int i = 0; i < NS; i++) {
                d0 -= a[i] * cc[i];
                if (i < 7) d1 += a[i] * rc1[i];
              }
              lds_d[grp][0][role] = d0;
              lds_d[grp][1][role] = d1;
            }
            wsync();
            {
              double prc[NS];
              ASC_UNROLL
              for (int i = 0; i < NS; i++) prc[i] = lds_d[grp][drow][i];
              double uu = 0.0, vv = 0.0;
              ASC_UNROLL
              for (int i = 0; i < NS; i++) {
                const double pj = a[i] - prc[i], sj = a[i] + pj;
                if (i < 7) uu += rc1[i] * sj;
                vv += cc[i] * sj;
                a[i] = pj;
              }
              U += uu; V += vv;
            }
          }
        }
        wsync();
        PROF(2);
        {
          const int k = c * CHN + nl;
          if (k < K && act) {
            if (live) {
              ASC_UNROLL
              for (int i = 0; i < NS + 3; i++) w[(size_t)(R_KA + i) * Kp + k] = outb[i * LDW + col];
            }
            const double k00 = outb[NS * LDW + col], k01 = outb[(NS + 1) * LDW + col], k02 = outb[(NS + 2) * LDW + col], D = outb[(NS + 3) * LDW + col];
            const double Dk1 = D * k01, Dk2 = D * k02;
            k10 += Dk1 * k00; k11 += Dk1 * k01; k12 += Dk1 * k02; k20 += Dk2 * k00; k22 += Dk2 * k02;
            if (!(D > 0.0)) bad = 1;
          }
        }
        wsync();
        PROF(3);
      }
      const double U0 = bcast16<RL>(U), U1 = bcast16<RL + 1>(U), V1 = bcast16<RL + 1>(V), U2 = bcast16<RL + 2>(U), V2 = bcast16<RL + 2>(V);
      k10 = gsumW<WIDE>(k10); k11 = gsumW<WIDE>(k11); k12 = gsumW<WIDE>(k12); k20 = gsumW<WIDE>(k20); k22 = gsumW<WIDE>(k22);
      bad = (int)gmaxW<WIDE>((double)bad);
      if (probe_rows) {
        if (act && role == 0) sc[X_STATE] = ST_DONE;
      } else if (act) {
        const double S10 = k10 + 0.5 * (U0 - V1), S11 = k11 + U1, S12 = k12 + 0.5 * U2, S20 = k20 - 0.5 * V2, S22 = k22;
        int ok = !bad;
        double dth = 0.0, dnu3 = 0.0;
        if (ok) {
          const double itl = rcp(s.th - d.tlb), itu = rcp(d.tub - s.th);
          const double rthp = sc[X_RTH] + mu * (itu - itl);
          const double sth = s.zlt * itl + s.zut * itu + dw;
          const double a11 = sth - S11, a12 = -S12, a22 = TERM == 2 ? -1.0 : -S22;
          const double b1 = -rthp + S10, b2 = -tm.e3 + S20;
          const double det = a11 * a22 - a12 * a12;
          if (det < 0.0) {
            const double idet = 1.0 / det;
            dth = (b1 * a22 - a12 * b2) * idet;
            dnu3 = (a11 * b2 - a12 * b1) * idet;
          } else {
            ok = 0;
          }
        }
        if (role == 0) {
          if (ok) {
            sc[X_DTH] = dth; sc[X_DNU3] = dnu3; sc[X_SIG1] = sig1; sc[X_SIG2] = sig2; sc[X_RS1] = rs1; sc[X_RS2] = rs2;
            sc[X_CG1] = tm.g1 - s.s1; sc[X_CG2] = tm.g2 - s.s2;
            sc[X_DWL] = dw; sc[X_STATE] = ST_FACTORED;
          } else {
            const double ndw = next_delta_w(dw, sc[X_DWL]);
            if (sc[X_PROBE] != 0.0) sc[X_STATE] = ST_DONE;
            else if (ndw > 1e10) { sc[X_STATUS] = ASCENT_REGULARISATION_FAILED; sc[X_STATE] = ST_DONE; }
            else sc[X_DW] = ndw;
          }
        }
      }
    }
    wsync();
    state = (int)sc[X_STATE];
    if (__any(state == ST_FACTORED)) {
      const bool act = state == ST_FACTORED;
      const Scal s = lds_scal(sc, X_S);
      const double mu = sc[X_MU], dw = sc[X_DWL], dth = sc[X_DTH], dnu3 = sc[X_DNU3];
      const double sig1 = sc[X_SIG1], sig2 = sc[X_SIG2], rs1 = sc[X_RS1], rs2 = sc[X_RS2];
      const double *it = w + (size_t)((int)sc[X_CUR] * NIT) * Kp;
      double *stp = w + (size_t)R_ST * Kp;
      const double dt = hT * s.th, be = dt * d.alpha, cs = SCHEME == 1 ? 0.5 * dt : dt, hTc = SCHEME == 1 ? 0.5 * hT : hT;
      const double ha = 0.5 * d.aub, bu = FORM == 1 ? ha : be;
      const double tau = fmax(0.99, 1.0 - mu);
      {
        constexpr int NC = 6 + MP, FS = NC + 1;
        const int fbase = (role < 7 ? FS * role : 0) * LDW;
        const int fout = (role < 6 ? role : role == 6 ? 7 : 8) * LDW;
        double yown = 0.0, carry_m = 0.0, carry_u = 0.0;
        double rmax = 0.0, gsum = 0.0, adu = 1.0, gmove = 0.0, clu = 0.0;
        double dzK[7] = {0, 0, 0, 0, 0, 0, 0};
        for (int c = 0; c < nch; c++) {
          const int kn = c * CHN + nl;
          const bool on = kn < K && act;
          double a_ = 0.5, m_ = 0.5, u_ = 0.0, zb[6] = {1, 1, 1, 1, 1, 1};
          double G[8], Gp[8], E[4], x0[7], ka[NS], du00 = 0.0;
          double x0u = 0.0, pp_ = 1.0, pn_ = 1.0, zpp_ = 0.0, zpn_ = 0.0, lu_ = 0.0;
          ASC_UNROLL
          for (int i = 0; i < 7; i++) x0[i] = 0.0;
          ASC_UNROLL
          for (int i = 0; i < NS; i++) ka[i] = 0.0;
          if (on) {
            double z[7], zp[7], F[7], ax, ay;
            ASC_UNROLL
            for (int i = 0; i < 7; i++) { z[i] = it[(O_Z + i) * Kp + kn]; zp[i] = kn > 0 ? it[(O_Z + i) * Kp + kn - 1] : 0.0; }
            u_ = it[O_U * Kp + kn];
            a_ = z[IA]; m_ = z[IM];
            ASC_UNROLL
            for (int b = 0; b < 6; b++) zb[b] = it[(O_ZB + b) * Kp + kn];
            ASC_UNROLL
            for (int i = 0; i < NS; i++) ka[i] = w[(size_t)(R_KA + i) * Kp + kn];
            if constexpr (MP) {
              pp_ = it[O_PP * Kp + kn]; pn_ = it[O_PN * Kp + kn]; zpp_ = it[O_ZP * Kp + kn]; zpn_ = it[O_ZN * Kp + kn]; lu_ = it[O_LU * Kp + kn];
              x0u = -(u_ - (kn > 0 ? it[O_U * Kp + kn - 1] : UINIT) - pp_ + pn_);
            }
            du00 = w[(size_t)R_K0 * Kp + kn] + w[(size_t)(R_K0 + 1) * Kp + kn] * dth + w[(size_t)(R_K0 + 2) * Kp + kn] * dnu3;
            accel<1>(d, z[IX], z[IY], z[IA], z[IM], 0.0, 0.0, ax, ay, G, nullptr);
            rhs_f<FORM>(d, z, u_, ax, ay, F);
            if (SCHEME == 1) {
              double Fb[7], axp, ayp;
              accel<1>(d, zp[IX], zp[IY], zp[IA], zp[IM], 0.0, 0.0, axp, ayp, Gp, nullptr);
              rhs_f<FORM>(d, zp, u_, axp, ayp, Fb);
              ASC_UNROLL
              for (int i = 0; i < 7; i++) F[i] = 0.5 * (F[i] + Fb[i]);
            }
            implicit_block(G, cs, E);
            ASC_UNROLL
            for (int i = 0; i < 7; i++) {
              x0[i] = hT * F[i] * dth - ((FORM == 1 && i == IA) ? z[IA] - ha * (u_ + 1.0) : z[i] - zp[i] - dt * F[i]);
              du00 -= ka[i] * x0[i];
            }
            if constexpr (MP) du00 -= ka[7] * x0u;
          }
          double incl = x0[IM];
          ASC_UNROLL
          for (int sft = 1; sft < CHN; sft *= 2) {
            const double t = __shfl_up(incl, sft, CHN);
            if (nl >= sft) incl += t;
          }
          const double dzm_k = carry_m + incl, dzm_p = dzm_k - x0[IM];
          carry_m += WIDE ? __shfl(incl, 63) : bcast16<15>(incl);
          if (on) {
            const double du00p = du00 - ka[IM] * dzm_p;
            double rvx[7], rvy[7];
            ainv_vrows<FORM>(G, E, cs, rvx, rvy);
            auto emit = [&](int i, const double *r, double aw) {
              const double bw = bu * aw;
              if constexpr (MP) stage[(FS * i + 6) * LDW + col] = bw * (1.0 - ka[7]);
              if (SCHEME == 1) {
                double m7[7], t[7];
                ASC_UNROLL
                for (int j = 0; j < 7; j++) m7[j] = r[j] - bw * ka[j];
                fzt_lambda(Gp, m7, t);
                ASC_UNROLL
                for (int j = 0; j < 7; j++) m7[j] += cs * t[j];
                double v = bw * (MP ? x0u + du00 : du00) + m7[IM] * dzm_p;
                ASC_UNROLL
                for (int j = 0; j < 7; j++) v += r[j] * x0[j];
                ASC_UNROLL
                for (int j = 0; j < 6; j++) stage[(FS * i + j) * LDW + col] = m7[j];
                stage[(FS * i + NC) * LDW + col] = v;
                return;
              }
              double v = bw * (MP ? x0u + du00p : du00p) + r[IM] * dzm_p;
              ASC_UNROLL
              for (int j = 0; j < 7; j++) v += r[j] * x0[j];
              ASC_UNROLL
              for (int j = 0; j < 6; j++) stage[(FS * i + j) * LDW + col] = (FORM == 1 && j == IA) ? 0.0 : r[j] - bw * ka[j];
              stage[(FS * i + NC) * LDW + col] = v;
            };
            emit(IVX, rvx, rvx[IB]);
            emit(IVY, rvy, rvy[IB]);
            {
              double r[7];
              ASC_UNROLL
              for (int j = 0; j < 7; j++) r[j] = (j == IX ? 1.0 : 0.0) + cs * rvx[j];
              emit(IX, r, cs * rvx[IB]);
              ASC_UNROLL
              for (int j = 0; j < 7; j++) r[j] = (j == IY ? 1.0 : 0.0) + cs * rvy[j];
              emit(IY, r, cs * rvy[IB]);
              ASC_UNROLL
              for (int j = 0; j < 7; j++) r[j] = j == IA ? 1.0 : (j == IW && FORM == 0) ? cs : 0.0;
              emit(IA, r, FORM == 1 ? 1.0 : cs);
              ASC_UNROLL
              for (int j = 0; j < 7; j++) r[j] = j == IW ? 1.0 : 0.0;
              emit(IW, r, FORM == 1 ? 0.0 : 1.0);
            }
            if constexpr (MP) {
              double kj[7], v0;
              if (SCHEME == 1) {
                double t[7];
                fzt_lambda(Gp, ka, t);
                ASC_UNROLL
                for (int j = 0; j < 7; j++) kj[j] = ka[j] + cs * t[j];
                v0 = du00 - kj[IM] * dzm_p;
              } else {
                ASC_UNROLL
                for (int j = 0; j < 7; j++) kj[j] = ka[j];
                v0 = du00p;
              }
              ASC_UNROLL
              for (int j = 0; j < 6; j++) stage[(FS * 6 + j) * LDW + col] = (FORM == 1 && j == IA) ? 0.0 : -kj[j];
              stage[(FS * 6 + 6) * LDW + col] = 1.0 - ka[7];
              stage[(FS * 6 + NC) * LDW + col] = x0u + v0;
            } else if (SCHEME == 1) {
              double t[7];
              fzt_lambda(Gp, ka, t);
              ASC_UNROLL
              for (int j = 0; j < 6; j++) stage[(42 + j) * LDW + col] = -(ka[j] + cs * t[j]);
              stage[48 * LDW + col] = du00 - (ka[IM] + cs * t[IM]) * dzm_p;
            } else {
              ASC_UNROLL
              for (int j = 0; j < 6; j++) stage[(42 + j) * LDW + col] = (FORM == 1 && j == IA) ? 0.0 : -ka[j];
              stage[48 * LDW + col] = du00p;
            }
            outb[6 * LDW + col] = dzm_k;
          }
          wsync();
          PROF(4);
          if (act) {
            const int jn = min(CHN, K - c * CHN);
            for (int jj = 0; jj < jn; jj++) {
              const int cj = cbase + jj;
              const double *sj = stage + fbase + cj;
              const double m0 = sj[0], m1 = sj[LDW], m2 = sj[2 * LDW], m3 = sj[3 * LDW], m4 = sj[4 * LDW], m5 = sj[5 * LDW], vv = sj[NC * LDW];
              const double b0 = bcast16<0>(yown), b1 = bcast16<1>(yown), b2 = bcast16<2>(yown), b3 = bcast16<3>(yown),
                           b4 = bcast16<4>(yown), b5 = bcast16<5>(yown);
              const double e0 = (vv + m0 * b0) + m2 * b2, e1 = m1 * b1 + m3 * b3, e2 = m4 * b4 + m5 * b5;
              if constexpr (MP) {
                const double m6 = sj[6 * LDW], b6 = bcast16<6>(yown);
                yown = ((e0 + e1) + e2) + m6 * b6;
              } else {
                yown = (e0 + e1) + e2;
              }
              outb[fout + cj] = yown;
            }
          }
          wsync();
          PROF(5);
          if (kn < K && act) {
            double dzn[8];
            ASC_UNROLL
            for (int i = 0; i < 8; i++) dzn[i] = outb[i * LDW + col];
            const double id[6] = {rcp(a_), rcp(d.aub - a_), rcp(m_), rcp(1.0 - m_), rcp(u_ + 1.0), rcp(1.0 - u_)};
            const double dza = dzn[IA], dzm = dzn[IM], du = dzn[7];
            if (kn == K - 1) cpy<7>(dzK, dzn);
            ASC_FTBR(rmax, id[0], dza); ASC_FTBR(rmax, id[1], -dza);
            ASC_FTBR(rmax, id[2], dzm); ASC_FTBR(rmax, id[3], -dzm);
            ASC_FTBR(rmax, id[4], du); ASC_FTBR(rmax, id[5], -du);
            gsum += dza * (id[1] - id[0]) + dzm * (id[3] - id[2]) + du * (id[5] - id[4]);
            const double dx3[3] = {dza, dzm, du};
            double dzb[6];
            ASC_UNROLL
            for (int b = 0; b < 3; b++) {
              const double zl = zb[2 * b], zu = zb[2 * b + 1];
              dzb[2 * b] = id[2 * b] * (mu - zl * dx3[b]) - zl;
              dzb[2 * b + 1] = id[2 * b + 1] * (mu + zu * dx3[b]) - zu;
              ASC_FTB(adu, zl, dzb[2 * b]);
              ASC_FTB(adu, zu, dzb[2 * b + 1]);
            }
            if (live) {
              ASC_UNROLL
              for (int i = 0; i < 7; i++) stp[(O_Z + i) * Kp + kn] = dzn[i];
              stp[O_U * Kp + kn] = du;
              ASC_UNROLL
              for (int b = 0; b < 6; b++) stp[(O_ZB + b) * Kp + kn] = dzb[b];
            }
            if constexpr (MP) {
              const double du_p = nl > 0 ? outb[7 * LDW + col - 1] : carry_u;
              const double ddel = (du - du_p) - x0u;
              const MovePivot mvp = move_pivot(pp_, pn_, zpp_, zpn_, lu_, dcw, mu, dw);
              const double dlu = mvp.Rd * ddel + mvp.gdl;
              double dpp, dpn;
              if (mvp.sgp >= mvp.sgn) { dpp = (dlu - mvp.rp) * rcp(mvp.sgp); dpn = dpp - ddel; }
              else { dpn = (-dlu - mvp.rn) * rcp(mvp.sgn); dpp = ddel + dpn; }
              const double dzp = mvp.ip * (mu - zpp_ * dpp) - zpp_, dzn_ = mvp.in_ * (mu - zpn_ * dpn) - zpn_;
              ASC_FTBR(rmax, mvp.ip, dpp); ASC_FTBR(rmax, mvp.in_, dpn);
              ASC_FTB(adu, zpp_, dzp); ASC_FTB(adu, zpn_, dzn_);
              gsum -= dpp * mvp.ip + dpn * mvp.in_;
              gmove += dpp + dpn;
              clu -= x0u * (lu_ + dlu);
              if (live) {
                stp[O_LU * Kp + kn] = dlu; stp[O_PP * Kp + kn] = dpp; stp[O_PN * Kp + kn] = dpn; stp[O_ZP * Kp + kn] = dzp; stp[O_ZN * Kp + kn] = dzn_;
              }
            }
          }
          if constexpr (MP) carry_u = outb[7 * LDW + cbase + CHN - 1];
          wsync();
          PROF(6);
        }
        rmax = gmaxW<WIDE>(rmax); gsum = gsumW<WIDE>(gsum); adu = gminW<WIDE>(adu);
        if constexpr (MP) { gmove = gsumW<WIDE>(gmove); clu = gsumW<WIDE>(clu); }
        ASC_UNROLL
        for (int i = 0; i < 7; i++) dzK[i] = gsumW<WIDE>(dzK[i]);
        double zK[7];
        ASC_UNROLL
        for (int i = 0; i < 7; i++) zK[i] = it[(O_Z + i) * Kp + K - 1];
        const Terminal tmK = TERM == 2 ? terminal_eval_any(d, zK) : terminal_eval(d, zK);
        Scal ds;
        ds.th = dth; ds.nu3 = dnu3;
        ds.s1 = sc[X_CG1] + tmK.g1g[0] * dzK[IX] + tmK.g1g[1] * dzK[IY];
        ds.s2 = sc[X_CG2] + tmK.g2g[0] * dzK[IVX] + tmK.g2g[1] * dzK[IVY];
        if constexpr (TERM == 2) {
          ds.s1 += tmK.g1v[0] * dzK[IVX] + tmK.g1v[1] * dzK[IVY];
          ds.s2 += tmK.g2p[0] * dzK[IX] + tmK.g2p[1] * dzK[IY];
        }
        ds.nu1 = sig1 * ds.s1 + rs1;
        ds.nu2 = sig2 * ds.s2 + rs2;
        ds.zs1 = mu / s.s1 - s.zs1 - s.zs1 / s.s1 * ds.s1;
        ds.zs2 = mu / s.s2 - s.zs2 - s.zs2 / s.s2 * ds.s2;
        const double dl_ = s.th - d.tlb, dU = d.tub - s.th;
        ds.zlt = mu / dl_ - s.zlt - s.zlt / dl_ * ds.th;
        ds.zut = mu / dU - s.zut + s.zut / dU * ds.th;
        double apr = 1.0;
        if (rmax * apr > tau) apr = tau / rmax;
        ASC_FTB(apr, dl_, ds.th); ASC_FTB(apr, dU, -ds.th);
        ASC_FTB(apr, s.s1, ds.s1); ASC_FTB(apr, s.s2, ds.s2);
        ASC_FTB(adu, s.zlt, ds.zlt); ASC_FTB(adu, s.zut, ds.zut);
        ASC_FTB(adu, s.zs1, ds.zs1); ASC_FTB(adu, s.zs2, ds.zs2);
        TrialCtx tc;
        tc.alpha = apr; tc.adu = adu; tc.mlo = mu * 1e-10; tc.mhi = mu * 1e10; tc.hT = hT; tc.first = false; tc.dcw = dcw;
        tc.stt = trial_scal(d, s, ds, apr, adu, mu, false);
        tc.dt = hT * tc.stt.th; tc.be = tc.dt * d.alpha;
        double *in = w + (size_t)((1 - (int)sc[X_CUR]) * NIT) * Kp;
        Part P;
        P.clear();
        const int abase = (role < 7 ? 6 * role : 0) * LDW;
        const int aout = (role < 7 ? role : 8) * LDW;
        const double aself = (role == IW || role == IM) ? 1.0 : 0.0;
        double lown = 0.0;
        double cl = 0.0, ccl = 0.0;
        for (int c = nch - 1; c >= 0; c--) {
          const int kn = c * CHN + nl;
          double ccn[7] = {0, 0, 0, 0, 0, 0, 0};
          TrialKeep kp;
          if (kn < K && act) {
            NodeIn n, dn;
            load_node<MP>(it, Kp, K, kn, n, UINIT);
            ASC_UNROLL
            for (int i = 0; i < 7; i++) { dn.z[i] = stp[(O_Z + i) * Kp + kn]; dn.zp[i] = kn > 0 ? stp[(O_Z + i) * Kp + kn - 1] : 0.0; }
            dn.u = stp[O_U * Kp + kn];
            ASC_UNROLL
            for (int b = 0; b < 6; b++) dn.zb[b] = stp[(O_ZB + b) * Kp + kn];
            if constexpr (MP) {
              dn.up = kn > 0 ? stp[O_U * Kp + kn - 1] : 0.0;
              dn.lu = stp[O_LU * Kp + kn];
              dn.lun = kn + 1 < K ? stp[O_LU * Kp + kn + 1] : 0.0;
              dn.pp = stp[O_PP * Kp + kn]; dn.pn = stp[O_PN * Kp + kn]; dn.zpp = stp[O_ZP * Kp + kn]; dn.zpn = stp[O_ZN * Kp + kn];
            }
            const double *dz = dn.z;
            double G[8], E[4], H[10], F[7], fl[7], lt[7], ax, ay;
            ASC_UNROLL
            for (int i = 0; i < 7; i++) lt[i] = SCHEME == 1 ? n.l[i] + n.ln[i] : n.l[i];
            accel<2>(d, n.z[IX], n.z[IY], n.z[IA], n.z[IM], -cs * lt[IVX], -cs * lt[IVY], ax, ay, G, H);
            rhs_f<FORM>(d, n.z, n.u, ax, ay, F);
            if (SCHEME == 1) {
              double Fb[7], axp, ayp;
              accel<0>(d, n.zp[IX], n.zp[IY], n.zp[IA], n.zp[IM], 0.0, 0.0, axp, ayp, nullptr, nullptr);
              rhs_f<FORM>(d, n.zp, n.u, axp, ayp, Fb);
              ASC_UNROLL
              for (int i = 0; i < 7; i++) F[i] = 0.5 * (F[i] + Fb[i]);
            }
            implicit_block(G, cs, E);
            fzt_lambda<FORM>(G, lt, fl);
            const double id0 = rcp(n.z[IA]), id1 = rcp(d.aub - n.z[IA]), id2 = rcp(n.z[IM]), id3 = rcp(1.0 - n.z[IM]);
            H[7] += n.zb[0] * id0 + n.zb[1] * id1;
            H[9] += n.zb[2] * id2 + n.zb[3] * id3;
            double r[7];
            ASC_UNROLL
            for (int i = 0; i < 7; i++) {
              const double rz = (FORM == 1 && i == IA) ? n.l[i] - cs * fl[i] : n.l[i] - cs * fl[i] - n.ln[i], gt = -hTc * fl[i];
              r[i] = -rz - gt * dth - dw * dz[i];
              ccn[i] = (FORM == 1 && i == IA) ? n.z[IA] - ha * (n.u + 1.0) : n.z[i] - n.zp[i] - dt * F[i];
              ccl += ccn[i] * n.l[i];
            }
            r[IA] -= mu * (id1 - id0);
            r[IM] -= mu * (id3 - id2);
            r[IX] -= H[0] * dz[IX] + H[1] * dz[IY] + H[2] * dz[IA] + H[3] * dz[IM];
            r[IY] -= H[1] * dz[IX] + H[4] * dz[IY] + H[5] * dz[IA] + H[6] * dz[IM];
            r[IA] -= H[2] * dz[IX] + H[5] * dz[IY] + H[7] * dz[IA] + H[8] * dz[IM];
            r[IM] -= H[3] * dz[IX] + H[6] * dz[IY] + H[8] * dz[IA] + H[9] * dz[IM];
            if (kn == K - 1) {
              double QT[28], qd[7];
              const Terminal tm = TERM == 2 ? terminal_eval_any(d, n.z) : terminal_eval(d, n.z);
              ASC_UNROLL
              for (int i = 0; i < 28; i++) QT[i] = 0.0;
              if constexpr (TERM == 2) terminal_hessian_any(QT, tm, s.nu1, s.nu2, sig1, sig2);
              else terminal_hessian(QT, tm, s.nu3, s.nu1, s.nu2, sig1, sig2);
              symv(QT, dz, qd);
              ASC_UNROLL
              for (int i = 0; i < 7; i++) r[i] -= qd[i];
              const double w1 = s.nu1 + sig1 * sc[X_CG1] + rs1, w2 = s.nu2 + sig2 * sc[X_CG2] + rs2;
              if constexpr (TERM == 2) {
                double g4[4];
                terminal_grad_any(tm, w1, w2, g4);
                r[IX] -= g4[0]; r[IY] -= g4[1]; r[IVX] -= g4[2]; r[IVY] -= g4[3];
              } else {
              r[IX] -= s.nu3 * tm.e3g[0] + w1 * tm.g1g[0] + tm.e3g[0] * dnu3;
              r[IY] -= s.nu3 * tm.e3g[1] + w1 * tm.g1g[1] + tm.e3g[1] * dnu3;
              r[IVX] -= s.nu3 * tm.e3g[2] + w2 * tm.g2g[0] + tm.e3g[2] * dnu3;
              r[IVY] -= s.nu3 * tm.e3g[3] + w2 * tm.g2g[1] + tm.e3g[3] * dnu3;
              }
            }
            double wv[7];
            solveAT<FORM>(G, E, cs, r, wv);
            {
              double rvx[7], rvy[7];
              ainv_vrows<FORM>(G, E, cs, rvx, rvy);
              ASC_UNROLL
              for (int i = 0; i < 7; i++) {
                double nr[7];
                nr[IVX] = rvx[i]; nr[IVY] = rvy[i];
                nr[IX] = (i == IX ? 1.0 : 0.0) + cs * rvx[i];
                nr[IY] = (i == IY ? 1.0 : 0.0) + cs * rvy[i];
                nr[IA] = FORM == 1 ? 0.0 : i == IA ? 1.0 : i == IW ? cs : 0.0;
                nr[IW] = i == IW ? 1.0 : 0.0;
                nr[IM] = i == IM ? 1.0 : 0.0;
                if (SCHEME == 1) {
                  double t[7];
                  fz_mul(G, nr, t);
                  ASC_UNROLL
                  for (int j = 0; j < 7; j++) nr[j] += cs * t[j];
                }
                ASC_UNROLL
                for (int j = 0; j < 5; j++) stage[(6 * i + j) * LDW + col] = nr[j];
              }
            }
            ASC_UNROLL
            for (int i = 0; i < 7; i++) stage[(6 * i + 5) * LDW + col] = wv[i];
            trial_primal<SCHEME, FORM, MP, TERM>(d, K, Kp, kn, n, dn, tc, live, in, P, kp);
          }
          wsync();
          PROF(7);
          if (act) {
            const int jj0 = min(CHN, K - c * CHN) - 1;
            for (int jj = jj0; jj >= 0; jj--) {
              const int cj = cbase + jj;
              const double *sj = stage + abase + cj;
              const double n0 = sj[0], n1 = sj[LDW], n2 = sj[2 * LDW], n3 = sj[3 * LDW], n4 = sj[4 * LDW], wv = sj[5 * LDW];
              const double b0 = bcast16<0>(lown), b1 = bcast16<1>(lown), b2 = bcast16<2>(lown), b3 = bcast16<3>(lown), b4 = bcast16<4>(lown);
              const double e0 = (wv + aself * lown) + n0 * b0, e1 = n1 * b1 + n2 * b2, e2 = n3 * b3 + n4 * b4;
              lown = (e0 + e1) + e2;
              outb[aout + cj] = lown;
            }
          }
          wsync();
          double dl[7], dln[7];
          if (kn < K && act) {
            ASC_UNROLL
            for (int i = 0; i < 7; i++) {
              dl[i] = outb[i * LDW + col];
              dln[i] = kn + 1 < K ? (nl < CHN - 1 ? outb[i * LDW + col + 1] : lds_c[WIDE ? 0 : grp][i]) : 0.0;
              ccl += ccn[i] * dl[i];
            }
            if (live) {
              ASC_UNROLL
              for (int i = 0; i < 7; i++) stp[(O_L + i) * Kp + kn] = dl[i];
            }
          }
          wsync();
          PROF(8);
          if (kn < K && act) {
            if (nl == 0) {
              ASC_UNROLL
              for (int i = 0; i < 7; i++) lds_c[WIDE ? 0 : grp][i] = dl[i];
            }
            double l[7], ln[7], lu = 0.0, lun = 0.0;
            ASC_UNROLL
            for (int i = 0; i < 7; i++) {
              l[i] = it[(O_L + i) * Kp + kn] + tc.alpha * dl[i];
              ln[i] = (kn + 1 < K ? it[(O_L + i) * Kp + kn + 1] : 0.0) + tc.alpha * dln[i];
            }
            if constexpr (MP) {
              lu = it[O_LU * Kp + kn] + tc.alpha * stp[O_LU * Kp + kn];
              lun = (kn + 1 < K ? it[O_LU * Kp + kn + 1] : 0.0) + tc.alpha * (kn + 1 < K ? stp[O_LU * Kp + kn + 1] : 0.0);
            }
            trial_dual<SCHEME, FORM, MP, TERM>(d, K, Kp, kn, kp, l, ln, lu, lun, tc, live, in, P);
          }
          PROF(0);
        }
        P.template reduceW<MP, WIDE>();
        ccl = gsumW<WIDE>(ccl);
        if (act) {
          cl += ccl;
          const Terminal &tm = tmK;
          double gd = MP ? mu * gsum + dcw * gmove : mu * gsum;
          if constexpr (MP) cl += clu;
          gd += ds.th * (1.0 - mu / dl_ + mu / dU) - mu * ds.s1 / s.s1 - mu * ds.s2 / s.s2;
          cl += tm.e3 * (s.nu3 + ds.nu3) + sc[X_CG1] * (s.nu1 + ds.nu1) + sc[X_CG2] * (s.nu2 + ds.nu2);
          const double c1 = sc[X_C1], slog = sc[X_SL];
          double nu_pen = sc[X_NUP];
          const double curv = -gd + cl;
          if (c1 > 0.0) {
            const double need = (gd + 0.5 * fmax(curv, 0.0)) / (0.9 * c1);
            if (nu_pen < need) nu_pen = need + 1.0;
          }
          wsync();
          if (role == 0) {
            put_scal(sc, X_D, ds);
            sc[X_NUP] = nu_pen;
            sc[X_DM] = gd - nu_pen * c1;
            sc[X_PHI0] = (MP ? s.th + dcw * sc[X_MV] : s.th) - mu * slog + nu_pen * c1;
            sc[X_ALPHA] = apr; sc[X_ADU] = adu; sc[X_LS] = 0.0;
            sc[X_P + 0] = P.rd; sc[X_P + 1] = P.cinf; sc[X_P + 2] = P.pmin; sc[X_P + 3] = P.pmax; sc[X_P + 4] = P.l1;
            sc[X_P + 5] = P.zsum; sc[X_P + 6] = P.rth; sc[X_P + 7] = P.c1; sc[X_P + 8] = P.sl; sc[X_P + 9] = P.mv;
            sc[X_TEVAL] = 1.0;
            sc[X_STATE] = ST_TRIAL;
          }
        }
      }
    }
    wsync();
    if (sc[X_PROBE] != 0.0) break;
  }
  wsync();
  PROF_END;
  if (live)
    for (int r = role; r < NSCAL; r += 16) gsc[r] = sc[r];
}

}

namespace ascent {

static PGeo geo_of(int K, int form = 0, int mp = 0, int term = 0, int wide = 0, int scheme = 0) {
  PGeo g;
  const int ch = scheme == 2 ? hs_chunk_nodes(wide) : wide ? 64 : CH;
  g.K = K; g.nch = (K + ch - 1) / ch; g.Kp = (g.nch * ch + 15) / 16 * 16;
  g.form = form; g.mp = mp ? 1 : 0; g.term = term == 2 ? 2 : 0; g.wide = wide ? 1 : 0;
  return g;
}

static size_t level_doubles(int K, int mp) {
  size_t m = 0;
  for (int scheme = 0; scheme <= 2; scheme += 2)
    for (int wide = 0; wide <= 1; wide++) {
      const size_t n = geo_of(K, 0, mp, 0, wide, scheme).nlp_doubles();
      m = n > m ? n : m;
    }
  return m;
}
size_t persist_ws_bytes(int K, long batch, int mp) {
  const size_t b = (size_t)batch * level_doubles(K, mp) * sizeof(double) + 64;
  return (b + 255) & ~(size_t)255;
}
size_t persist_region1_offset(const int *levels, long batch, int mp) { return persist_ws_bytes(levels[0] - 1, batch, mp); }
size_t persist_level_bytes_used(int K, long batch, int mp) { return (size_t)batch * level_doubles(K, mp) * sizeof(double); }
size_t persist_ws_bytes_nested(const int *levels, int nlev, long batch, int mp) {
  size_t b = persist_region1_offset(levels, batch, mp);
  if (nlev > 1) b += persist_ws_bytes(levels[1] - 1, batch, mp);
  return b;
}

using SolveKernel = void (*)(const ascent_params *, long, PGeo, double *, int, double);
struct SolveVariant { int scheme, form, mp, term, wide; SolveKernel kernel; };
#define ASC_VARIANT(S, F, M, T, W) {S, F, M, T, W, p_solve<S, F, M, T, W>}
static const SolveVariant solve_variants[] = {
    ASC_VARIANT(1, 0, 1, 2, 1), ASC_VARIANT(0, 0, 1, 2, 1), ASC_VARIANT(1, 0, 0, 2, 1), ASC_VARIANT(0, 0, 0, 2, 1),
    ASC_VARIANT(1, 0, 1, 0, 1), ASC_VARIANT(0, 1, 1, 0, 1), ASC_VARIANT(0, 1, 0, 0, 1), ASC_VARIANT(0, 0, 1, 0, 1),
    ASC_VARIANT(1, 0, 0, 0, 1), ASC_VARIANT(0, 0, 0, 0, 1),
    ASC_VARIANT(1, 0, 1, 2, 0), ASC_VARIANT(0, 0, 1, 2, 0), ASC_VARIANT(1, 0, 0, 2, 0), ASC_VARIANT(0, 0, 0, 2, 0),
    ASC_VARIANT(1, 0, 1, 0, 0), ASC_VARIANT(0, 1, 1, 0, 0), ASC_VARIANT(0, 0, 1, 0, 0), ASC_VARIANT(1, 0, 0, 0, 0),
    ASC_VARIANT(0, 1, 0, 0, 0), ASC_VARIANT(0, 0, 0, 0, 0)};
#undef ASC_VARIANT

static void launch_solve(int scheme, int form, int mp, long batch, hipStream_t stream, const ascent_params *dp, const PGeo &g, double *w,
                         int max_iter, double tol) {
  if (scheme == 2) {
    hs_launch_solve(batch, stream, dp, g.K, g.Kp, g.nch, g.term, g.wide, w, max_iter, tol);
    return;
  }
  SolveKernel kernel = g.wide ? p_solve<0, 0, 0, 0, 1> : p_solve<0, 0, 0, 0, 0>;
  for (const SolveVariant &v : solve_variants)
    if (v.scheme == scheme && v.form == form && v.mp == (mp ? 1 : 0) && v.term == g.term && v.wide == g.wide) kernel = v.kernel;
  hipLaunchKernelGGL(kernel, dim3((unsigned)(g.wide ? batch : (batch + NPW - 1) / NPW)), dim3(WAVE), 0, stream, dp, batch, g, w, max_iter, tol);
}

int persist_run_nested(const Call &c, bool wide, const int *levels, int nlev, double *ws, const SolveIO &io, double tol_coarse,
                       double mu_first, double mu_next) {
  const ascent_params *dp = c.dp;
  const long batch = c.batch;
  const int scheme = c.scheme, form = c.form, mp = c.mp, term = c.term;
  hipStream_t stream = c.stream;
  double *region[2] = {ws, (double *)((char *)ws + persist_region1_offset(levels, batch, mp))};
  PGeo g = geo_of(levels[nlev - 1] - 1, form, mp, term, wide, scheme);
  double *w = region[(nlev - 1) & 1];
  hipLaunchKernelGGL(p_init, dim3((unsigned)((g.Kp + WAVE - 1) / WAVE), (unsigned)batch), dim3(WAVE), 0, stream, dp, batch, g, w, io.guess,
                     io.warm, io.mu0, (const double *)nullptr, (const double *)nullptr, 0);
  for (int l = nlev - 1; l >= 0; l--) {
    launch_solve(scheme, form, mp, batch, stream, dp, g, w, io.max_iter, l == 0 ? io.tol : tol_coarse);
    if (l > 0) {
      const PGeo gf = geo_of(levels[l - 1] - 1, form, mp, term, wide, scheme);
      double *wf = region[(l - 1) & 1];
      hipLaunchKernelGGL(p_transfer, dim3((unsigned)((gf.Kp + WAVE - 1) / WAVE), (unsigned)batch), dim3(WAVE), 0, stream, dp, batch, g,
                         (const double *)w, gf, wf, l == nlev - 1 ? mu_first : mu_next);
      g = gf; w = wf;
    }
  }
  hipLaunchKernelGGL(p_finish, dim3((unsigned)((g.K + CH - 1) / CH), (unsigned)((batch + WAVE - 1) / WAVE)), dim3(WAVE, FIN_WAVES), 0, stream, dp, batch, g,
                     (const double *)w, io.traj, io.tf, io.status, io.iters, io.blob);
  ASC_CHK(c.err, c.errlen, hipGetLastError());
  return ASCENT_OK;
}

int persist_probe(const Call &c, bool wide, double *ws, const ProbeIO &io) {
  const PGeo g = geo_of(c.K, c.form, c.mp, c.term, wide, c.scheme);
  const dim3 ng((unsigned)((g.Kp + WAVE - 1) / WAVE), (unsigned)c.batch);
  hipLaunchKernelGGL(p_init, ng, dim3(WAVE), 0, c.stream, c.dp, c.batch, g, ws, io.iterate, 2, 0.1, io.mu, io.dw, 1);
  launch_solve(c.scheme, c.form, c.mp, c.batch, c.stream, c.dp, g, ws, 1000, -1.0);
  hipLaunchKernelGGL(p_probe_out, ng, dim3(WAVE), 0, c.stream, c.batch, g, (const double *)ws, io.step, io.inertia);
  ASC_CHK(c.err, c.errlen, hipGetLastError());
  return ASCENT_OK;
}

int persist_probe_rows(const Call &c, bool wide, double *ws, const ProbeIO &io) {
  const PGeo g = geo_of(c.K, c.form, 0, 0, wide);
  const dim3 ng((unsigned)((g.Kp + WAVE - 1) / WAVE), (unsigned)c.batch);
  hipLaunchKernelGGL(p_init, ng, dim3(WAVE), 0, c.stream, c.dp, c.batch, g, ws, io.iterate, 2, 0.1, io.mu, io.mu, 2);
  launch_solve(c.scheme, c.form, 0, c.batch, c.stream, c.dp, g, ws, 1000, -1.0);
  hipLaunchKernelGGL(p_probe_rows_out, ng, dim3(WAVE), 0, c.stream, c.dp, c.batch, g, (const double *)ws, io.defects, io.jac, io.hess);
  ASC_CHK(c.err, c.errlen, hipGetLastError());
  return ASCENT_OK;
}

}
```

### lunar_module_ascent_trajectory_optimiser_amd/csrc/ascent_persist.hpp

```cpp
#pragma once
#include <hip/hip_runtime.h>
#include <cstddef>
#include "ascent.h"
#include "ascent_host.hpp"

namespace ascent {

size_t persist_ws_bytes(int K, long batch, int mp);

size_t persist_region1_offset(const int *levels, long batch, int mp);
size_t persist_ws_bytes_nested(const int *levels, int nlev, long batch, int mp);
size_t persist_level_bytes_used(int K, long batch, int mp);
int persist_run_nested(const Call &c, bool wide, const int *levels, int nlev, double *ws, const SolveIO &io, double tol_coarse,
                       double mu_first, double mu_next);

int persist_probe(const Call &c, bool wide, double *ws, const ProbeIO &io);

int persist_probe_rows(const Call &c, bool wide, double *ws, const ProbeIO &io);

void hs_launch_solve(long batch, hipStream_t stream, const ascent_params *dp, int K, int Kp, int nch, int term, int wide, double *w, int max_iter, double tol);
int hs_chunk_nodes(int wide);

}
```

### lunar_module_ascent_trajectory_optimiser_amd/csrc/ascent_persist_dev.hpp

```cpp
#pragma once
#include <hip/hip_runtime.h>

#include "ascent.h"
#include "ascent_device.hpp"
#include "ascent_tile.hpp"

namespace {
using namespace ascent;

constexpr int NPW = 4, CH = 16;
constexpr int O_Z = 0, O_U = 7, O_L = 8, O_ZB = 15;
constexpr int O_LU = 21, O_PP = 22, O_PN = 23, O_ZP = 24, O_ZN = 25;
template <int MP>
struct Lay {
  static constexpr int NS = 7 + MP, NIT = 21 + 5 * MP;
  static constexpr int R_IT = 0, R_ST = 2 * NIT, R_KA = 3 * NIT, R_K0 = R_KA + NS, NROWS = R_K0 + 3;
  static constexpr int S_G = 0, S_E = 8, S_H = 12, S_F = 22, S_C = S_F + 7 - MP, S_RZ = S_C + NS, S_GT = S_RZ + NS, S_SC = S_GT + NS;
  static constexpr int S_ROWS = MP ? 56 : 55;
  static constexpr int OUT_ROWS = 11 + MP;
  static_assert(S_SC + (MP ? 3 : 5) <= S_ROWS, "stage rows");
};
constexpr int R_IT = 0;
constexpr int LDW = 65;
enum {
  X_STATE, X_ITERS, X_STATUS, X_CUR, X_FIRST, X_LS, X_MU, X_NUP, X_DW, X_DWL, X_ALPHA, X_ADU, X_PHI0, X_DM, X_C1, X_SL,
  X_RTH, X_DTH, X_DNU3, X_SIG1, X_SIG2, X_RS1, X_RS2, X_CG1, X_CG2,
  X_ITB,
  X_PROBE, X_PDW,
  X_TEVAL,
  X_P,
  X_PEND = X_P + 9,
  X_MV,
  X_S,
  X_D = X_S + 10,
  NSCAL = X_D + 10
};
constexpr int NSCAL_PAD = 64;
static_assert(NSCAL <= NSCAL_PAD, "scalar record");
enum { ST_TRIAL = 0, ST_FACTOR = 1, ST_FACTORED = 2, ST_DONE = 3 };

struct PGeo {
  int K, Kp, nch, form, mp, term, wide;
  __host__ __device__ int nit() const { return mp ? Lay<1>::NIT : Lay<0>::NIT; }
  __host__ __device__ int r_st() const { return 2 * nit(); }
  __host__ __device__ int nrows() const { return mp ? Lay<1>::NROWS : Lay<0>::NROWS; }
  __host__ __device__ size_t nlp_doubles() const { return (size_t)nrows() * Kp + NSCAL_PAD; }
};

template <int SRC>
ASC_DEV double bcast16(double v) {
  const long x = __builtin_amdgcn_mov_dpp(__builtin_bit_cast(long, v), 0x150 + SRC, 0xf, 0xf, false);
  return __builtin_bit_cast(double, x);
}
template <int N>
struct OneHot {
  double m[N];
  ASC_DEV explicit OneHot(int role) {
    ASC_UNROLL
    for (int i = 0; i < N; i++) m[i] = (role == i || (i == 0 && role >= N)) ? 1.0 : 0.0;
  }
  ASC_DEV double pick(const double *v) const {
    double r = m[0] * v[0];
    ASC_UNROLL
    for (int i = 1; i < N; i++) r += m[i] * v[i];
    return r;
  }
};
ASC_DEV void wsync() {
  __builtin_amdgcn_fence(__ATOMIC_RELEASE, "wavefront");
  __builtin_amdgcn_wave_barrier();
  __builtin_amdgcn_fence(__ATOMIC_ACQUIRE, "wavefront");
}
ASC_DEV double gsum16(double v) { v += __shfl_xor(v, 1); v += __shfl_xor(v, 2); v += __shfl_xor(v, 4); v += __shfl_xor(v, 8); return v; }
ASC_DEV double gmax16(double v) { v = fmax(v, __shfl_xor(v, 1)); v = fmax(v, __shfl_xor(v, 2)); v = fmax(v, __shfl_xor(v, 4)); return fmax(v, __shfl_xor(v, 8)); }
ASC_DEV double gmin16(double v) { v = fmin(v, __shfl_xor(v, 1)); v = fmin(v, __shfl_xor(v, 2)); v = fmin(v, __shfl_xor(v, 4)); return fmin(v, __shfl_xor(v, 8)); }
template <int WIDE> ASC_DEV double gsumW(double v) { v = gsum16(v); if constexpr (WIDE) { v += __shfl_xor(v, 16); v += __shfl_xor(v, 32); } return v; }
template <int WIDE> ASC_DEV double gmaxW(double v) { v = gmax16(v); if constexpr (WIDE) { v = fmax(v, __shfl_xor(v, 16)); v = fmax(v, __shfl_xor(v, 32)); } return v; }
template <int WIDE> ASC_DEV double gminW(double v) { v = gmin16(v); if constexpr (WIDE) { v = fmin(v, __shfl_xor(v, 16)); v = fmin(v, __shfl_xor(v, 32)); } return v; }

template <typename PT>
ASC_DEV Scal lds_scal(PT sc, int r0) {
  Scal s;
  s.th = sc[r0 + S_TH]; s.zlt = sc[r0 + S_ZLT]; s.zut = sc[r0 + S_ZUT]; s.s1 = sc[r0 + S_S1]; s.s2 = sc[r0 + S_S2];
  s.zs1 = sc[r0 + S_ZS1]; s.zs2 = sc[r0 + S_ZS2]; s.nu3 = sc[r0 + S_NU3]; s.nu1 = sc[r0 + S_NU1]; s.nu2 = sc[r0 + S_NU2];
  return s;
}
ASC_DEV void put_scal(double *sc, int r0, const Scal &s) {
  sc[r0 + S_TH] = s.th; sc[r0 + S_ZLT] = s.zlt; sc[r0 + S_ZUT] = s.zut; sc[r0 + S_S1] = s.s1; sc[r0 + S_S2] = s.s2;
  sc[r0 + S_ZS1] = s.zs1; sc[r0 + S_ZS2] = s.zs2; sc[r0 + S_NU3] = s.nu3; sc[r0 + S_NU1] = s.nu1; sc[r0 + S_NU2] = s.nu2;
}
ASC_DEV Scal trial_scal(const Der &d, const Scal &s, const Scal &ds, double alpha, double adu, double mu, bool first) {
  Scal t = s;
  if (first) return t;
  t.th += alpha * ds.th; t.s1 += alpha * ds.s1; t.s2 += alpha * ds.s2;
  t.nu3 += alpha * ds.nu3; t.nu1 += alpha * ds.nu1; t.nu2 += alpha * ds.nu2;
  t.zlt = clipz(s.zlt + adu * ds.zlt, t.th - d.tlb, mu);
  t.zut = clipz(s.zut + adu * ds.zut, d.tub - t.th, mu);
  t.zs1 = clipz(s.zs1 + adu * ds.zs1, t.s1, mu);
  t.zs2 = clipz(s.zs2 + adu * ds.zs2, t.s2, mu);
  return t;
}

struct NodeIn {
  double z[7], zp[7], l[7], ln[7], zb[6], u;
  double up, lu, lun, pp, pn, zpp, zpn;
};
template <int MP = 0>
ASC_DEV void load_node(const double *it, int Kp, int K, int k, NodeIn &n, double uinit = 0.0) {
  ASC_UNROLL
  for (int i = 0; i < 7; i++) {
    n.z[i] = it[(O_Z + i) * Kp + k];
    n.l[i] = it[(O_L + i) * Kp + k];
    n.zp[i] = k > 0 ? it[(O_Z + i) * Kp + k - 1] : 0.0;
    n.ln[i] = k + 1 < K ? it[(O_L + i) * Kp + k + 1] : 0.0;
  }
  n.u = it[O_U * Kp + k];
  ASC_UNROLL
  for (int b = 0; b < 6; b++) n.zb[b] = it[(O_ZB + b) * Kp + k];
  if constexpr (MP) {
    n.up = k > 0 ? it[O_U * Kp + k - 1] : uinit;
    n.lu = it[O_LU * Kp + k];
    n.lun = k + 1 < K ? it[O_LU * Kp + k + 1] : 0.0;
    n.pp = it[O_PP * Kp + k]; n.pn = it[O_PN * Kp + k]; n.zpp = it[O_ZP * Kp + k]; n.zpn = it[O_ZN * Kp + k];
  }
}

struct Part {
  double rd, cinf, pmin, pmax, l1, zsum, rth, c1, sl, mv;
  ASC_DEV void clear() { rd = 0.0; cinf = 0.0; pmin = 1e300; pmax = -1e300; l1 = 0.0; zsum = 0.0; rth = 0.0; c1 = 0.0; sl = 0.0; mv = 0.0; }
  template <int MP = 0>
  ASC_DEV void reduce16() {
    rd = gmax16(rd); cinf = gmax16(cinf); pmin = gmin16(pmin); pmax = gmax16(pmax);
    l1 = gsum16(l1); zsum = gsum16(zsum); rth = gsum16(rth); c1 = gsum16(c1); sl = gsum16(sl);
    if constexpr (MP) mv = gsum16(mv);
  }
  template <int MP, int WIDE>
  ASC_DEV void reduceW() {
    rd = gmaxW<WIDE>(rd); cinf = gmaxW<WIDE>(cinf); pmin = gminW<WIDE>(pmin); pmax = gmaxW<WIDE>(pmax);
    l1 = gsumW<WIDE>(l1); zsum = gsumW<WIDE>(zsum); rth = gsumW<WIDE>(rth); c1 = gsumW<WIDE>(c1); sl = gsumW<WIDE>(sl);
    if constexpr (MP) mv = gsumW<WIDE>(mv);
  }
};
struct TrialCtx {
  double alpha, adu, mlo, mhi, dt, be, hT, dcw;
  bool first;
  Scal stt;
};

#ifdef PERSIST_PROFILE
#define PROF_DECL long long prof_[10] = {0, 0, 0, 0, 0, 0, 0, 0, 0, 0}; long long pt_ = clock64();
#define PROF(i_) do { const long long t1_ = clock64(); prof_[i_] += t1_ - pt_; pt_ = t1_; } while (0)
#define PROF_END do { if (blockIdx.x == 0 && threadIdx.x == 0) printf("[persist profile] cycles: A %lld | B eval %lld serial %lld flush %lld | F eval %lld serial %lld post %lld | Adj eval %lld serial %lld | rest %lld\n", prof_[0], prof_[1], prof_[2], prof_[3], prof_[4], prof_[5], prof_[6], prof_[7], prof_[8], prof_[9]); } while (0)
#else
#define PROF_DECL
#define PROF(i_) do { } while (0)
#define PROF_END do { } while (0)
#endif

}
```

### lunar_module_ascent_trajectory_optimiser_amd/csrc/ascent_solver.hip

```cpp
#include <hip/hip_runtime.h>

#include <cstdio>
#include <cstdlib>
#include <cstring>
#include <mutex>
#include <vector>
#include <cmath>

#include "ascent.h"
#include "ascent_host.hpp"
#include "ascent_device.hpp"
#include "ascent_tile.hpp"
#include "ascent_pipeline.hpp"
#include "ascent_dense.hpp"
#include "ascent_blocktri.hpp"
#include "ascent_persist.hpp"
#include "ascent_fused.hpp"
#include "ascent_sens.hpp"
#include "ascent_flight.hpp"
#include "ascent_trim.hpp"
#include "ascent_disperse.hpp"
#include "ascent_guide.hpp"

using namespace ascent;
// ... 324 lines not shown
  unsigned long long z[8] = {0};
  if (hipMemcpyFromSymbol(out8, HIP_SYMBOL(g_prof), sizeof z) != hipSuccess) return -1;
  if (reset && hipMemcpyToSymbol(HIP_SYMBOL(g_prof), z, sizeof z) != hipSuccess) return -1;
  return 0;
}
#endif

int ascent_version(void) { return 300; }

int ascent_device_count(void) {
  int n = 0;
  if (hipGetDeviceCount(&n) != hipSuccess) return 0;
  return n;
}

const char *ascent_strerror(int code) {
  switch (code) {
    case ASCENT_OK: return "ok";
    case ASCENT_E_ARG: case ASCENT_E_HIP: case ASCENT_E_NODEVICE: case ASCENT_E_NOMEM: case ASCENT_E_NOTERM:
      return g_err[0] ? g_err : "error";
    default: return "unknown error code";
  }
}

double ascent_last_kernel_ms(int device_id) {
  if (device_id < 0 || device_id >= MAX_DEV) return -1.0;
  std::lock_guard<std::mutex> lock(g_mu[device_id]);
  DeviceWs &w = g_wss[device_id][g_ws_last[device_id]];
  if (!w.launched) return -1.0;
  if (hipSetDevice(device_id) != hipSuccess) return -1.0;
  if (hipEventSynchronize(w.ev1) != hipSuccess) return -1.0;
  float ms = -1.f;
  if (hipEventElapsedTime(&ms, w.ev0, w.ev1) != hipSuccess) return -1.0;
  return ms;
}

int ascent_solve_batch(const ascent_params *p, int64_t batch, const ascent_opts *o,
                       const double *guess, double *traj_out, double *tf_out, int32_t *status_out,
                       int32_t *iters_out, double *sol_blob_out, int device_id, void *stream_,
                       int ptr_is_device) {
  int rc = check_options(p, batch, o);
  if (rc) return rc;
  if (!tf_out || !status_out || !iters_out) { snprintf(g_err, sizeof g_err, "null output pointer"); return ASCENT_E_ARG; }
  if (o->warm_start < 0 || o->warm_start > 2 || (o->warm_start && !guess)) { snprintf(g_err, sizeof g_err, "warm_start needs a guess blob"); return ASCENT_E_ARG; }
  if (!(o->tol > 0) || o->max_iter < 0) { snprintf(g_err, sizeof g_err, "tol must be > 0, max_iter >= 0"); return ASCENT_E_ARG; }
  Route r{};
  if ((rc = check_solvable(p, batch, o, ptr_is_device, &r))) return rc;
  if ((rc = check_device(device_id))) return rc;
  std::lock_guard<std::mutex> lock(g_mu[device_id]);
  HIPCHK(hipSetDevice(device_id));
  hipStream_t stream = (hipStream_t)stream_;
  const int K = o->n_nodes - 1, nt = o->n_nodes;
  const size_t rows = 21 * (size_t)K + NSC;
  const bool persist = r.path == ASCENT_PATH_PERSIST;
  int levels[8];
  const int nlev = nested_levels(o, levels);
  const int slot = slot_for(device_id, stream);
  DeviceWs &w = g_wss[device_id][slot];
  g_ws_last[device_id] = slot;
  rc = ensure_ws(w, persist ? persist_ws_bytes_nested(levels, nlev, (long)batch, (int)o->move_penalty) : ws_bytes(r, K, batch, (int)o->move_penalty));
  if (rc) return rc;
  const double mu0 = o->mu_init > 0 ? o->mu_init : (o->warm_start ? 1e-4 : 0.1);

  const ascent_params *dp = p;
  const double *dguess = guess;
  double *dtraj = traj_out, *dtf = tf_out, *dblob = sol_blob_out;
  int *dstatus = status_out, *diters = iters_out;
  if (w.launched) HIPCHK(hipStreamWaitEvent(stream, w.ev1, 0));
  if (!ptr_is_device) {
    if ((rc = grow(w.h_p, w.h_p_n, (size_t)batch))) return rc;
    HIPCHK(hipMemcpyAsync(w.h_p, p, batch * sizeof(ascent_params), hipMemcpyHostToDevice, stream));
    dp = w.h_p;
    if (o->warm_start) {
      if ((rc = grow(w.h_guess, w.h_guess_n, rows * batch))) return rc;
      HIPCHK(hipMemcpyAsync(w.h_guess, guess, rows * batch * sizeof(double), hipMemcpyHostToDevice, stream));
      dguess = w.h_guess;
    }
    if (traj_out) { if ((rc = grow(w.h_traj, w.h_traj_n, (size_t)10 * nt * batch))) return rc; dtraj = w.h_traj; }
    if (sol_blob_out) { if ((rc = grow(w.h_blob, w.h_blob_n, rows * batch))) return rc; dblob = w.h_blob; }
    if ((rc = grow(w.h_tf, w.h_tf_n, (size_t)batch))) return rc;
    dtf = w.h_tf;
    if ((rc = grow(w.h_status, w.h_status_n, (size_t)batch))) return rc;
    dstatus = w.h_status;
    if ((rc = grow(w.h_iters, w.h_iters_n, (size_t)batch))) return rc;
    diters = w.h_iters;
  }
  if (o->terminal == 1) {
    if ((rc = grow(w.t_p, w.t_p_n, (size_t)batch))) return rc;
    hipLaunchKernelGGL(k_terminal_params, dim3((unsigned)((batch + WAVE - 1) / WAVE)), dim3(WAVE), 0, stream, dp, w.t_p, (long)batch);
    HIPCHK(hipGetLastError());
    dp = w.t_p;
  }
  if (nlev > 1 && !persist) {
    size_t n3 = w.int_n, n3b = w.int_n, n3c = w.int_n, ntf = w.int_n;
    rc = grow(w.sol, w.sol_n, (21 * (size_t)(levels[1] - 1) + NSC) * batch);
    if (!rc) rc = grow(w.gss, w.gss_n, rows * batch);
    if (!rc) rc = grow(w.st_c, n3, (size_t)batch);
    if (!rc) rc = grow(w.it_c, n3b, (size_t)batch);
    if (!rc) rc = grow(w.acc, n3c, (size_t)batch);
    if (!rc) rc = grow(w.tfc, ntf, (size_t)batch);
    if (rc) return rc;
    w.int_n = n3;
  }
  HIPCHK(hipEventRecord(w.ev0, stream));
  double mu_first = o->move_penalty ? NESTED_MU_FIRST_MP : NESTED_MU_FIRST, mu_next = o->move_penalty ? nested_mu_next_mp(o->tol) : nested_mu_next(o->tol);
  if (const char *e = getenv("ASCENT_NESTED_MU")) sscanf(e, "%lf,%lf", &mu_first, &mu_next);
  const Call c = call_of(dp, batch, o, stream);
  const double tol_coarse = fmax(o->tol, NESTED_COARSE_TOL);
  if (persist) {
    const SolveIO io{dguess, (int)o->warm_start, (int)o->max_iter, o->tol, mu0, dtraj, dtf, dstatus, diters, dblob};
    if ((rc = persist_run_nested(c, r.wide, levels, nlev, w.ws, io, tol_coarse, mu_first, mu_next))) return rc;
  }
  for (int l = nlev - 1; l >= 0 && !persist; l--) {
    const bool fin = l == 0, first = l == nlev - 1;
    Call cl = c;
    cl.K = levels[l] - 1;
    const SolveIO io{first ? dguess : w.gss, first ? (int)o->warm_start : 2, (int)o->max_iter, fin ? o->tol : tol_coarse,
                     first ? mu0 : (l == nlev - 2 ? mu_first : mu_next), fin ? dtraj : nullptr, fin ? dtf : w.tfc,
                     fin ? dstatus : w.st_c, fin ? diters : w.it_c, fin ? dblob : w.sol};
    switch (r.path) {
      case ASCENT_PATH_DENSE: rc = dense_run(cl, w.ws, io, r.pcr); break;
      case ASCENT_PATH_FUSED: rc = fused_run(cl, w.ws, io); break;
      default: rc = pipeline_run(cl, w.ws, io, r.path == ASCENT_PATH_SPLIT_WIDE, nullptr);
    }
    if (rc) return rc;
    if (!fin) {
      const int Kf = levels[l - 1] - 1;
      hipLaunchKernelGGL(k_prolong, dim3((unsigned)((batch + WAVE - 1) / WAVE), (unsigned)Kf), dim3(WAVE), 0, stream, w.sol,
                         w.st_c, w.it_c, cl.K, w.gss, Kf, (long)batch, (int)o->formulation, w.acc, first ? 1 : 0);
      HIPCHK(hipGetLastError());
    }
  }
  if (nlev > 1 && !persist) {
    hipLaunchKernelGGL(k_add_iters, dim3((unsigned)((batch + WAVE - 1) / WAVE)), dim3(WAVE), 0, stream, diters, w.acc, (long)batch);
    HIPCHK(hipGetLastError());
  }
  HIPCHK(hipEventRecord(w.ev1, stream));
  w.launched = true;
  if (!ptr_is_device) {
    if (traj_out) HIPCHK(hipMemcpyAsync(traj_out, dtraj, (size_t)10 * nt * batch * sizeof(double), hipMemcpyDeviceToHost, stream));
    if (sol_blob_out) HIPCHK(hipMemcpyAsync(sol_blob_out, dblob, rows * batch * sizeof(double), hipMemcpyDeviceToHost, stream));
    HIPCHK(hipMemcpyAsync(tf_out, dtf, batch * sizeof(double), hipMemcpyDeviceToHost, stream));
    HIPCHK(hipMemcpyAsync(status_out, dstatus, batch * sizeof(int), hipMemcpyDeviceToHost, stream));
    HIPCHK(hipMemcpyAsync(iters_out, diters, batch * sizeof(int), hipMemcpyDeviceToHost, stream));
  }
  if (!ptr_is_device || !stream) HIPCHK(hipStreamSynchronize(stream));
  return ASCENT_OK;
}

int ascent_workspace_layout(int64_t batch, const ascent_opts *o, int64_t *out4) {
  if (!o || !out4 || batch <= 0 || o->n_nodes < 3) return ASCENT_E_ARG;
  int levels[8];
  const int nlev = nested_levels(o, levels), mp = (int)o->move_penalty;
  out4[0] = (int64_t)persist_ws_bytes_nested(levels, nlev, (long)batch, mp);
  out4[1] = (int64_t)persist_level_bytes_used(levels[0] - 1, (long)batch, mp);
  out4[2] = nlev > 1 ? (int64_t)persist_region1_offset(levels, (long)batch, mp) : 0;
  out4[3] = nlev > 1 ? (int64_t)persist_level_bytes_used(levels[1] - 1, (long)batch, mp) : 0;
  return nlev;
}

int ascent_default_path(int64_t batch, const ascent_opts *o) {
  if (!o || batch <= 0) return ASCENT_E_ARG;
  return route(o, batch, ASCENT_PATH_AUTO, false).path;
}

int ascent_eval_nodes_path(const ascent_params *p, int64_t batch, const ascent_opts *o, const double *iterate,
                           double *defects, double *jac_blocks, double *hess_blocks, int device_id, int path) {
  int rc = check_options(p, batch, o);
  if (rc) return rc;
  if (o->move_penalty) { snprintf(g_err, sizeof g_err, "the parity surfaces take the unpenalised NLP only (move_penalty = 1 is an option of ascent_solve_batch)"); return ASCENT_E_ARG; }
  if (!iterate || !defects || !jac_blocks || !hess_blocks) { snprintf(g_err, sizeof g_err, "null pointer"); return ASCENT_E_ARG; }
  if (path < ASCENT_PATH_AUTO || path > ASCENT_PATH_PERSIST) { snprintf(g_err, sizeof g_err, "unknown path %d", path); return ASCENT_E_ARG; }
  const Route r = route(o, batch, path, true);
  if (r.path == ASCENT_PATH_DENSE) { snprintf(g_err, sizeof g_err, "the dense-block path exposes its node evaluation through ascent_dense_records"); return ASCENT_E_ARG; }
  if (o->scheme == 2) { snprintf(g_err, sizeof g_err, "the node evaluation of scheme 2 is exposed through ascent_dense_records"); return ASCENT_E_ARG; }
  ascent_opts rows_o = *o;
  rows_o.terminal = 0;
  if (const char *why = unsupported(r.path, &rows_o)) { snprintf(g_err, sizeof g_err, "%s", why); return ASCENT_E_ARG; }
  if ((rc = check_device(device_id))) return rc;
  std::lock_guard<std::mutex> lock(g_mu[device_id]);
  HIPCHK(hipSetDevice(device_id));
  if ((rc = claim_slot0(device_id))) return rc;
  const int K = o->n_nodes - 1;
  Staging st(nullptr, 0);
  const Call c = call_of(st.in(p, (size_t)batch), batch, &rows_o, nullptr);
  ProbeIO io{};
  io.iterate = st.in(iterate, (21 * (size_t)K + NSC) * batch);
  io.defects = st.out(defects, (size_t)7 * K * batch);
  io.jac = st.out(jac_blocks, (size_t)8 * K * batch);
  io.hess = st.out(hess_blocks, (size_t)10 * K * batch);
  double *ws = nullptr;
  if (r.path != ASCENT_PATH_FUSED) {
    if ((rc = ensure_ws(g_ws_slot0(device_id), ws_bytes(r, K, batch, 0)))) return rc;
    ws = g_ws_slot0(device_id).ws;
    double *zero = st.scratch<double>((size_t)batch);
    if (zero) HIPCHK(hipMemset(zero, 0, batch * sizeof(double)));
    io.mu = io.dw = zero;
  }
  if ((rc = st.failed())) return rc;
  switch (r.path) {
    case ASCENT_PATH_FUSED: rc = fused_eval_nodes(c, io); break;
    case ASCENT_PATH_PERSIST: rc = persist_probe_rows(c, r.wide, ws, io); break;
    default: rc = pipeline_probe(c, ws, io, r.path == ASCENT_PATH_SPLIT_WIDE);
  }
  return rc ? rc : st.finish();
}

int ascent_eval_nodes(const ascent_params *p, int64_t batch, const ascent_opts *o, const double *iterate,
                      double *defects, double *jac_blocks, double *hess_blocks, int device_id) {
  return ascent_eval_nodes_path(p, batch, o, iterate, defects, jac_blocks, hess_blocks, device_id, ASCENT_PATH_AUTO);
}

static int terminal_params_in_place(const ascent_opts *o, const ascent_params *dp, int64_t batch) {
  if (o->terminal != 1) return 0;
  hipLaunchKernelGGL(k_terminal_params, dim3((unsigned)((batch + WAVE - 1) / WAVE)), dim3(WAVE), 0, 0, dp, const_cast<ascent_params *>(dp), (long)batch);
  HIPCHK(hipGetLastError());
  return 0;
}

int ascent_kkt_step_path(const ascent_params *p, int64_t batch, const ascent_opts *o, const double *iterate,
                         const double *mu, const double *delta_w, double *step, int32_t *inertia_out, int device_id,
                         int path) {
  int rc = check_options(p, batch, o);
  if (rc) return rc;
  if (!iterate || !mu || !delta_w || !step || !inertia_out) { snprintf(g_err, sizeof g_err, "null pointer"); return ASCENT_E_ARG; }
  if (path < ASCENT_PATH_AUTO || path > ASCENT_PATH_PERSIST) { snprintf(g_err, sizeof g_err, "unknown path %d", path); return ASCENT_E_ARG; }
  const Route r = route(o, batch, path, true);
  if (const char *why = unsupported(r.path, o)) { snprintf(g_err, sizeof g_err, "%s", why); return ASCENT_E_ARG; }
  if (o->move_penalty && (rc = check_dcost(p, batch))) return rc;
  if ((rc = check_device(device_id))) return rc;
  std::lock_guard<std::mutex> lock(g_mu[device_id]);
  HIPCHK(hipSetDevice(device_id));
  if ((rc = claim_slot0(device_id))) return rc;
  const int K = o->n_nodes - 1;
  const size_t rows = 21 * (size_t)K + NSC;
  if ((rc = ensure_ws(g_ws_slot0(device_id), ws_bytes(r, K, batch, (int)o->move_penalty)))) return rc;
  double *ws = g_ws_slot0(device_id).ws;
  Staging st(nullptr, 0);
  const Call c = call_of(st.in(p, (size_t)batch), batch, o, nullptr);
  ProbeIO io{};
  io.iterate = st.in(iterate, rows * batch);
  io.mu = st.in(mu, (size_t)batch);
  io.dw = st.in(delta_w, (size_t)batch);
  io.step = st.out(step, rows * batch);
  io.inertia = st.out(inertia_out, (size_t)batch);
  if ((rc = st.failed())) return rc;
  HIPCHK(hipMemset(io.step, 0, rows * batch * sizeof(double)));
  if ((rc = terminal_params_in_place(o, c.dp, batch))) return rc;
  switch (r.path) {
    case ASCENT_PATH_DENSE: rc = dense_probe(c, ws, io, r.pcr); break;
    case ASCENT_PATH_PERSIST: rc = persist_probe(c, r.wide, ws, io); break;
    case ASCENT_PATH_FUSED: rc = fused_probe(c, ws, io); break;
    default: rc = pipeline_probe(c, ws, io, r.path == ASCENT_PATH_SPLIT_WIDE);
  }
  if (rc || (rc = st.finish())) return rc;
  for (int64_t q = 0; q < batch; q++) inertia_out[q] = inertia_out[q] != 0;
  return ASCENT_OK;
}

int ascent_dense_records(const ascent_params *p, int64_t batch, const ascent_opts *o, const double *iterate,
                         double *records, int device_id) {
  int rc = check_options(p, batch, o);
  if (rc) return rc;
  if (o->move_penalty) { snprintf(g_err, sizeof g_err, "the parity surfaces take the unpenalised NLP only (move_penalty = 1 is an option of ascent_solve_batch)"); return ASCENT_E_ARG; }
  if (!iterate || !records) { snprintf(g_err, sizeof g_err, "null pointer"); return ASCENT_E_ARG; }
  if (const char *why = unsupported(ASCENT_PATH_DENSE, o)) { snprintf(g_err, sizeof g_err, "%s", why); return ASCENT_E_ARG; }
  if ((rc = check_device(device_id))) return rc;
  std::lock_guard<std::mutex> lock(g_mu[device_id]);
  HIPCHK(hipSetDevice(device_id));
  if ((rc = claim_slot0(device_id))) return rc;
  const int K = o->n_nodes - 1;
  if ((rc = ensure_ws(g_ws_slot0(device_id), dense_ws_bytes(K, (long)batch)))) return rc;
  Staging st(nullptr, 0);
  Call c = call_of(st.in(p, (size_t)batch), batch, o, nullptr);
  c.term = 0;
  ProbeIO io{};
  io.iterate = st.in(iterate, (21 * (size_t)K + NSC) * batch);
  io.records = st.out(records, (size_t)batch * K * 6 * 64);
  double *zero = st.scratch<double>((size_t)batch);
  if ((rc = st.failed())) return rc;
  HIPCHK(hipMemset(zero, 0, batch * sizeof(double)));
  io.mu = io.dw = zero;
  if ((rc = terminal_params_in_place(o, c.dp, batch))) return rc;
  if ((rc = dense_probe(c, g_ws_slot0(device_id).ws, io, false))) return rc;
  return st.finish();
}

int ascent_coast_batch(const ascent_params *p, int64_t batch, const double *final_state, int32_t coast_nodes,
                       double *coast_traj, double *coast_tf, double *apsides, int device_id, void *stream_,
                       int ptr_is_device) {
  if (!p || batch <= 0 || !final_state || !coast_traj || !coast_tf || !apsides) { snprintf(g_err, sizeof g_err, "null pointer or batch <= 0"); return ASCENT_E_ARG; }
  if (coast_nodes < 1 || coast_nodes > 65535) { snprintf(g_err, sizeof g_err, "coast_nodes out of range (1 .. 65535)"); return ASCENT_E_ARG; }
  int rc = check_device(device_id);
  if (rc) return rc;
  std::lock_guard<std::mutex> lock(g_mu[device_id]);
  HIPCHK(hipSetDevice(device_id));
  hipStream_t stream = (hipStream_t)stream_;
  Staging st(stream, ptr_is_device);
  const Call c = call_of(st.in(p, (size_t)batch), batch, nullptr, stream);
  const double *ds = st.in(final_state, (size_t)4 * batch);
  double *dc = st.out(coast_traj, (size_t)4 * (coast_nodes + 1) * batch), *dt = st.out(coast_tf, (size_t)batch), *da = st.out(apsides, (size_t)2 * batch);
  if ((rc = st.failed()) || (rc = coast_run(c, ds, coast_nodes, dc, dt, da))) return rc;
  return st.finish();
}

int ascent_param_sensitivity(const ascent_params *p, int64_t batch, const ascent_opts *o, const double *sol_blob,
// ... 278 lines not shown
```

### lunar_module_ascent_trajectory_optimiser_amd/distributed.py

```python
from __future__ import annotations

import numpy as np

from .params import pack
from .solver import solve_batch, solve_batch_torch


def shard_indices(n: int, rank: int, world: int) -> np.ndarray:
    return np.arange(rank, n, world)


def _dist():
    import torch.distributed as dist
    return dist if dist.is_available() and dist.is_initialized() else None


def solve_sharded(params, nt: int = 200, tol: float = 1e-9, max_iter: int = 300, device: int | None = None,
                  gather_traj: bool = False, solver=None, **kw):
    import torch
    P = pack(params)
    n = P.shape[0]
    dist = _dist()
    rank, world = (dist.get_rank(), dist.get_world_size()) if dist else (0, 1)
    if device is None:
        device = rank % max(1, torch.cuda.device_count()) if torch.cuda.is_available() else 0
    idx = shard_indices(n, rank, world)
    m = (n + world - 1) // world
    width = 3 + (10 * nt if gather_traj else 0)
    k = len(idx)
    on_device = solver is None and dist is not None and dist.get_backend() == "nccl"
    failure = None
    if on_device:
        dev = torch.device("cuda", device)
        local = torch.zeros((m + 1, width), dtype=torch.float64, device=dev)
        if k:
            try:
                o = solve_batch_torch(torch.from_numpy(np.ascontiguousarray(P[idx])).to(dev), nt, tol=tol, max_iter=max_iter,
                                      want_traj=gather_traj, **kw)
                local[:k, 0], local[:k, 1], local[:k, 2] = o["tf"], o["status"].double(), o["iters"].double()
                if gather_traj:
                    local[:k, 3:] = o["traj"].permute(2, 0, 1).reshape(k, -1)
            except Exception as e:
                failure = e
                local[m, 0] = 1.0
    else:
        local = np.zeros((m + 1, width))
        if k:
            try:
                res = (solver or solve_batch)(P[idx], nt=nt, tol=tol, max_iter=max_iter, device=device,
                                              want_traj=gather_traj, **kw)
                local[:k, 0], local[:k, 1], local[:k, 2] = res.tf, res.status, res.iters
                if gather_traj:
                    local[:k, 3:] = np.moveaxis(res.traj, 2, 0).reshape(k, -1)
            except Exception as e:
                failure = e
                local[m, 0] = 1.0
    if not dist:
        if failure:
            raise failure
        gathered = [local]
    else:
        if on_device:
            t = local
        else:
            t = torch.from_numpy(local)
            if dist.get_backend() == "nccl":
                t = t.to(torch.device("cuda", device))
        bufs = [torch.empty_like(t) for _ in range(world)] if rank == 0 else None
        dist.gather(t, bufs, dst=0)
        if failure:
            raise failure
        if rank != 0:
            return None
        gathered = [b.cpu().numpy() for b in bufs]
        bad = [r for r, g in enumerate(gathered) if g[m, 0] != 0.0]
        if bad:
            raise RuntimeError(f"solve_sharded: the solver failed on rank(s) {bad}")
    out = np.zeros((n, width))
    for r, g in enumerate(gathered):
        ids = shard_indices(n, r, world)
        out[ids] = g[: len(ids)]
    result = dict(tf=out[:, 0], status=out[:, 1].astype(np.int32), iters=out[:, 2].astype(np.int32))
    if gather_traj:
        result["traj"] = np.moveaxis(out[:, 3:].reshape(n, 10, nt), 0, 2)
    return result
```

### lunar_module_ascent_trajectory_optimiser_amd/solver.py

```python
from __future__ import annotations

import ctypes as C
import dataclasses

import numpy as np

from . import _lib
from .params import AscentParams, pack

TRAJ_FIELDS = ("x", "y", "xdot", "ydot", "xdoubledot", "ydoubledot", "angle", "angledot",
               "angledoubledot", "mass")
STATUS_NAMES = {0: "converged", 1: "max_iter", 2: "linesearch_failed", 3: "regularisation_failed"}


def blob_rows(nt: int) -> int:
    return 21 * (nt - 1) + 10


SCHEMES = {"backward_euler": 0, "trapezoid": 1, "hermite_simpson": 2}
TERMINALS = {"reference": 0, "ellipse": 1, "ellipse_free": 2}


FORMULATIONS = {"current": 0, "v1": 1}


def _opts(nt, max_iter, tol, warm_start, mu_init, scheme=0, formulation=0, coarse_nodes=0, terminal=0, path="auto", move_penalty=False):
    scheme = SCHEMES.get(scheme, scheme)
    formulation = FORMULATIONS.get(formulation, formulation)
    terminal = TERMINALS.get(terminal, terminal)
    if path not in ("auto", "dense"):
        raise ValueError('solver path must be "auto" or "dense"')
    return _lib.AscentOptsC(n_nodes=nt, scheme=int(scheme), max_iter=max_iter, warm_start=warm_start, tol=tol,
                            mu_init=mu_init, formulation=int(formulation), coarse_nodes=int(coarse_nodes),
                            terminal=int(terminal), solver_path=_lib.PATHS[path], move_penalty=int(bool(move_penalty)), reserved=0)


def _ptr(a):
    return None if a is None else a.ctypes.data_as(C.c_void_p)


def _blob_call(params, sol_blob, nt, scheme=0, formulation=0, terminal=0, move_penalty=False, what="sol_blob"):
    P = pack(params)
    B = P.shape[0]
    blob = np.ascontiguousarray(sol_blob, dtype=np.float64)
    if blob.shape != (blob_rows(nt), B):
        raise ValueError(f"sol_blob must have shape {(blob_rows(nt), B)}" if what == "sol_blob" else f"{what} has the wrong shape")
    o = _opts(nt, 0, 1.0, 0, 0.0, scheme, formulation, terminal=terminal, move_penalty=move_penalty)
    return _lib.load(), P, B, nt - 1, blob, o


FLIGHT_ROWS = ("miss_position", "miss_velocity", "flown_periapsis_alt", "flown_apoapsis_alt", "nlp_periapsis_alt",
               "nlp_apoapsis_alt", "max_local_position_error", "max_local_velocity_error", "max_local_step", "substeps")


@dataclasses.dataclass
class FlightResult:
    traj: np.ndarray | None
    local_error: np.ndarray | None
    summary: np.ndarray


for _i, _n in enumerate(FLIGHT_ROWS):
    setattr(FlightResult, _n, property(lambda self, _i=_i: self.summary[:, _i]))


JACOBIAN_ROWS = ("x", "y", "xdot", "ydot", "angle", "angledot", "mass", "periapsis_alt", "apoapsis_alt")
TRIM_ROWS = ("status", "rounds", "residual", "residual_before", "delta_tf_seconds", "max_delta_u", "free_controls",
             "flown_periapsis_alt", "flown_apoapsis_alt", "angle_violation")
TRIM_STATUS_NAMES = {0: "converged", 1: "rounds_exhausted", 2: "frozen"}


@dataclasses.dataclass
class FlightJacobian:
    dz0: np.ndarray
    dparams: np.ndarray
    dtf: np.ndarray
    dcontrols: np.ndarray | None

    def predict(self, dparams=None, dtf=None, dcontrols=None, dz0=None) -> np.ndarray:
        out = np.zeros(self.dtf.shape)
        if dparams is not None:
            out += np.einsum("bqc,bc->bq", self.dparams, np.broadcast_to(np.asarray(dparams, dtype=np.float64), self.dparams[:, 0].shape))
        if dtf is not None:
            out += self.dtf * np.broadcast_to(np.asarray(dtf, dtype=np.float64), self.dtf.shape[:1])[:, None]
        if dcontrols is not None:
            if self.dcontrols is None:
                raise ValueError("this FlightJacobian was computed without the control columns")
            out += np.einsum("bqk,bk->bq", self.dcontrols, np.broadcast_to(np.asarray(dcontrols, dtype=np.float64), self.dcontrols[:, 0].shape))
        if dz0 is not None:
            out += np.einsum("bqc,bc->bq", self.dz0, np.broadcast_to(np.asarray(dz0, dtype=np.float64), self.dz0[:, 0].shape))
        return out

    def sigma(self, param_sigma=None, control_sigma=None) -> np.ndarray:
        var = np.zeros(self.dtf.shape)
        if param_sigma is not None:
            var += ((self.dparams * np.broadcast_to(np.asarray(param_sigma, dtype=np.float64), self.dparams[:, 0].shape)[:, None, :]) ** 2).sum(axis=2)
        if control_sigma is not None:
            if self.dcontrols is None:
                raise ValueError("this FlightJacobian was computed without the control columns")
            var += ((self.dcontrols * np.broadcast_to(np.asarray(control_sigma, dtype=np.float64), self.dcontrols[:, 0].shape)[:, None, :]) ** 2).sum(axis=2)
        return np.sqrt(var)


def _sigma_rows(v, n, B, what):
    if v is None:
        return np.zeros((B, n))
    a = np.asarray(v, dtype=np.float64)
    try:
        return np.ascontiguousarray(np.broadcast_to(a, (B, n)))
    except ValueError:
        raise ValueError(f"{what} must broadcast to {(B, n)}") from None


def _cov_from_upper(rows):
    B = rows.shape[0]
    cov = np.empty((B, 9, 9))
    iu = np.triu_indices(9)
    cov[:, iu[0], iu[1]] = rows
    cov[:, iu[1], iu[0]] = rows
    return cov


@dataclasses.dataclass
class DispersionResult:
    n_valid: np.ndarray
    nominal: np.ndarray
    mean: np.ndarray
    cov: np.ndarray
    min: np.ndarray
    max: np.ndarray
    samples: np.ndarray | None
    xi: np.ndarray
    z0_sigma: np.ndarray
    param_sigma: np.ndarray
    tf_sigma: np.ndarray
    control_sigma: np.ndarray
    effort: np.ndarray | None = None

    @property
    def std(self) -> np.ndarray:
        return np.sqrt(np.diagonal(self.cov, axis1=1, axis2=2))

    def linear_covariance(self, J: FlightJacobian) -> np.ndarray:
        A = [J.dz0 * self.z0_sigma[:, None, :], J.dparams * self.param_sigma[:, None, :], (J.dtf * self.tf_sigma[:, None])[:, :, None]]
        n = 24
        if self.control_sigma.any():
            if J.dcontrols is None:
                raise ValueError("this FlightJacobian was computed without the control columns")
            A.append(J.dcontrols * self.control_sigma[:, None, :])
            n += self.control_sigma.shape[1]
        A = np.concatenate(A, axis=2)
        C = np.atleast_2d(np.cov(self.xi[:n]))
        return np.einsum("bqc,cd,brd->bqr", A, C, A)


EFFORT_ROWS = ("clipped_steps", "max_feedback", "stretch")
GUIDE_ROWS = ("status", "free_controls", "max_gain", "max_cutoff_gain", "substeps")
GUIDE_STATUS_NAMES = {0: "ok", 2: "frozen"}


@dataclasses.dataclass
class GuidanceResult:
    gain_u: np.ndarray
    gain_t: np.ndarray
    summary: np.ndarray
# ... 200 lines not shown
                          None if ju is None else np.ascontiguousarray(ju.transpose(2, 0, 1)))


def trim_batch(params, sol_blob: np.ndarray, nt: int, scheme=0, formulation=0, terminal=0, move_penalty: bool = False,
               substeps: int = 0, rounds: int = 0, tol: float = 0.0, device: int = 0) -> TrimResult:
    L, P, B, K, blob, o = _blob_call(params, sol_blob, nt, scheme, formulation, terminal, move_penalty)
    out = np.empty_like(blob)
    summ = np.empty((len(TRIM_ROWS), B))
    _lib.check(L.ascent_trim_batch(_ptr(P), B, C.byref(o), _ptr(blob), int(substeps), int(rounds), float(tol), _ptr(out), _ptr(summ),
                                   device, None, 0))
    return TrimResult(out, np.ascontiguousarray(summ.T), nt)


def disperse_batch(params, sol_blob: np.ndarray, nt: int, *, param_sigma=None, control_sigma=None, tf_sigma=None, z0_sigma=None,
                   samples: int = 256, seed: int = 0, xi=None, keep_samples: bool = False, scheme=0, formulation=0, terminal=0,
                   move_penalty: bool = False, substeps: int = 0, device: int = 0, guidance: GuidanceResult | None = None) -> DispersionResult:
    L, P, B, K, blob, o = _blob_call(params, sol_blob, nt, scheme, formulation, terminal, move_penalty)
    if xi is None:
        xi = np.random.default_rng(seed).standard_normal((24 + K, int(samples)))
    xi = np.ascontiguousarray(xi, dtype=np.float64)
    if xi.ndim != 2 or xi.shape[0] != 24 + K:
        raise ValueError(f"xi must have shape (24 + K, samples) = ({24 + K}, samples)")
    S = xi.shape[1]
    zs, ps = _sigma_rows(z0_sigma, 7, B, "z0_sigma"), _sigma_rows(param_sigma, 16, B, "param_sigma")
    ts = _sigma_rows(None if tf_sigma is None else np.asarray(tf_sigma, dtype=np.float64)[..., None], 1, B, "tf_sigma")
    us = _sigma_rows(control_sigma, K, B, "control_sigma")
    sig = np.ascontiguousarray(np.concatenate([zs, ps, ts], axis=1).T)
    sig_u = np.ascontiguousarray(us.T) if control_sigma is not None else None
    stats = np.empty((82, B))
    smp = np.empty((9 if guidance is None else 12, S, B)) if keep_samples else None
    if guidance is None:
        _lib.check(L.ascent_disperse_batch(_ptr(P), B, C.byref(o), _ptr(blob), int(substeps), S, _ptr(xi), _ptr(sig), _ptr(sig_u),
                                           _ptr(stats), _ptr(smp), device, None, 0))
    else:
        gu = np.ascontiguousarray(np.asarray(guidance.gain_u, dtype=np.float64).transpose(2, 1, 0))
        if gu.shape != (7, K, B):
            raise ValueError(f"guidance.gain_u must have shape {(B, K, 7)}")
        gt = None if guidance.gain_t is None else np.ascontiguousarray(np.asarray(guidance.gain_t, dtype=np.float64).T)
        if gt is not None and gt.shape != (7, B):
            raise ValueError(f"guidance.gain_t must have shape {(B, 7)}")
        sm = None if gt is None else _sigma_rows(np.asarray(guidance.stretch_max, dtype=np.float64)[..., None], 1, B, "stretch_max")[:, 0].copy()
        _lib.check(L.ascent_disperse_guided_batch(_ptr(P), B, C.byref(o), _ptr(blob), int(substeps), S, _ptr(xi), _ptr(sig), _ptr(sig_u),
                                                  _ptr(gu), _ptr(gt), _ptr(sm), _ptr(stats), _ptr(smp), device, None, 0))
    st = stats.T
    return DispersionResult(st[:, 0].astype(np.int64), np.ascontiguousarray(st[:, 1:10]), np.ascontiguousarray(st[:, 10:19]),
                            _cov_from_upper(st[:, 19:64]), np.ascontiguousarray(st[:, 64:73]), np.ascontiguousarray(st[:, 73:82]),
                            None if smp is None else np.ascontiguousarray(smp[:9].transpose(2, 1, 0)), xi, zs, ps, ts[:, 0].copy(), us,
                            None if smp is None or guidance is None else np.ascontiguousarray(smp[9:].transpose(2, 1, 0)))


def guidance_gains(params, sol_blob: np.ndarray, nt: int, scheme=0, formulation=0, terminal=0, move_penalty: bool = False,
                   substeps: int = 0, device: int = 0, cond_weights=(1e6, 1e6, 1e6), control_weight=1.0, cutoff_weight=1.0,
                   stretch_max=0.5, want_jacobian: bool = True) -> GuidanceResult:
    L, P, B, K, blob, o = _blob_call(params, sol_blob, nt, scheme, formulation, terminal, move_penalty)
    w = np.ascontiguousarray(np.concatenate([_sigma_rows(cond_weights, 3, B, "cond_weights")] + [
        _sigma_rows(np.asarray(v, dtype=np.float64)[..., None], 1, B, n)
        for v, n in ((control_weight, "control_weight"), (cutoff_weight, "cutoff_weight"), (stretch_max, "stretch_max"))], axis=1).T)
    gu, gt, summ = np.empty((7, K, B)), np.empty((7, B)), np.empty((len(GUIDE_ROWS), B))
    jac = np.empty((9, 24, B)) if want_jacobian else None
    ju = np.empty((9, K, B)) if want_jacobian else None
    _lib.check(L.ascent_guidance_gains(_ptr(P), B, C.byref(o), _ptr(blob), int(substeps), _ptr(w), _ptr(gu), _ptr(gt), _ptr(summ),
                                       _ptr(jac), _ptr(ju), device, None, 0))
    J = None
    if want_jacobian:
        j = jac.transpose(2, 0, 1)
        J = FlightJacobian(np.ascontiguousarray(j[:, :, :7]), np.ascontiguousarray(j[:, :, 7:23]), np.ascontiguousarray(j[:, :, 23]),
                           np.ascontiguousarray(ju.transpose(2, 0, 1)))
    return GuidanceResult(np.ascontiguousarray(gu.transpose(2, 1, 0)), np.ascontiguousarray(gt.T), np.ascontiguousarray(summ.T),
                          w[5].copy(), J)


def eval_nodes(params, iterate: np.ndarray, nt: int = 200, device: int = 0, path="auto", scheme=0, formulation=0):
    L, P, B, K, it, o = _blob_call(params, iterate, nt, scheme, formulation, what="iterate")
    d, j, h = np.empty((7 * K, B)), np.empty((8 * K, B)), np.empty((10 * K, B))
    _lib.check(L.ascent_eval_nodes_path(_ptr(P), B, C.byref(o), _ptr(it), _ptr(d), _ptr(j), _ptr(h), device,
                                        _lib.PATHS[path]))
    return d, j, h


def kkt_step(params, iterate: np.ndarray, mu, delta_w, nt: int = 200, device: int = 0, path="auto", scheme=0,
             formulation=0, terminal=0, move_penalty: bool = False):
    L, P, B, K, it, o = _blob_call(params, iterate, nt, scheme, formulation, terminal, move_penalty, what="iterate")
    mu = np.ascontiguousarray(np.broadcast_to(np.asarray(mu, dtype=np.float64), (B,)))
    dw = np.ascontiguousarray(np.broadcast_to(np.asarray(delta_w, dtype=np.float64), (B,)))
    step = np.empty_like(it)
    inertia = np.empty(B, dtype=np.int32)
    _lib.check(L.ascent_kkt_step_path(_ptr(P), B, C.byref(o), _ptr(it), _ptr(mu), _ptr(dw), _ptr(step), _ptr(inertia),
                                      device, _lib.PATHS[path]))
    return step, inertia


def dense_records(params, iterate: np.ndarray, nt: int = 200, scheme=2, device: int = 0) -> np.ndarray:
    L, P, B, K, it, o = _blob_call(params, iterate, nt, scheme, what="iterate")
    rec = np.empty((B, K, 6, 8, 8))
    _lib.check(L.ascent_dense_records(_ptr(P), B, C.byref(o), _ptr(it), _ptr(rec), device))
    return rec


def coast_batch(params, final_state: np.ndarray, coast_nodes: int = 200, device: int = 0) -> dict:
    L = _lib.load()
    P = pack(params)
    B = P.shape[0]
    fs = np.ascontiguousarray(final_state, dtype=np.float64)
    if fs.shape != (4, B):
        raise ValueError(f"final_state must have shape {(4, B)}")
    traj = np.empty((4, coast_nodes + 1, B)); tf = np.empty(B); aps = np.empty((2, B))
    _lib.check(L.ascent_coast_batch(_ptr(P), B, _ptr(fs), coast_nodes, _ptr(traj), _ptr(tf), _ptr(aps), device, None, 0))
    return dict(traj=traj, tf=tf, periapsis_alt=aps[0], apoapsis_alt=aps[1])


def kkt_solve(diag, lower, upper, rhs, border=None, border_diag=None, algo="pcr", device: int = 0):
    L = _lib.load()
    D = np.ascontiguousarray(diag, dtype=np.float64)
    B, n, bs, _ = D.shape
    Lo = np.ascontiguousarray(lower, dtype=np.float64); Up = np.ascontiguousarray(upper, dtype=np.float64)
    nb = 0 if border is None else int(np.shape(border)[-1])
    r = np.ascontiguousarray(rhs, dtype=np.float64)
    if Lo.shape != D.shape or Up.shape != D.shape or r.shape != (B, n * bs + nb):
        raise ValueError("inconsistent shapes")
    bo = bd = None
    if nb:
        bo = np.ascontiguousarray(border, dtype=np.float64); bd = np.ascontiguousarray(border_diag, dtype=np.float64)
        if bo.shape != (B, n, bs, nb) or bd.shape != (B, nb, nb):
            raise ValueError("inconsistent border shapes")
    sol = np.empty_like(r)
    _lib.check(L.ascent_kkt_solve(B, n, bs, nb, _ptr(D), _ptr(Lo), _ptr(Up), _ptr(bo), _ptr(bd), _ptr(r), _ptr(sol), device,
                                  {"thomas": 0, "pcr": 1}[algo]))
    return sol, L.ascent_last_kernel_ms(device)


def solve_batch_torch(params_t, nt: int = 200, tol: float = 1e-9, max_iter: int = 300, guess_t=None,
                      warm_start: int = 0, mu_init: float = 0.0, want_traj: bool = True, want_blob: bool = False,
                      out: dict | None = None, sync: bool = False, coarse_nodes: int = 0, scheme=0,
                      formulation=0, move_penalty: bool = False, terminal=0, path: str = "auto",
                      sensitivity: bool = False, flight: bool = False) -> dict:
    import torch
    L = _lib.load()
    _lib.require_single_hip_runtime()
    if not (params_t.is_cuda and params_t.dtype == torch.float64 and params_t.is_contiguous()):
        raise ValueError("params_t must be a contiguous float64 CUDA tensor")
    B = params_t.shape[0]
    dev = params_t.device
    rows = blob_rows(nt)
    out = out if out is not None else {}
    def buf(name, shape, dtype):
        t = out.get(name)
        if t is None:
            t = out[name] = torch.empty(shape, dtype=dtype, device=dev)
        elif not (t.device == dev and t.dtype == dtype and tuple(t.shape) == tuple(shape) and t.is_contiguous()):
            raise ValueError(f"out[{name!r}] must be a contiguous {dtype} tensor of shape {tuple(shape)} on {dev}")
        return t
    if params_t.dim() != 2 or params_t.shape[1] != 16:
        raise ValueError("params_t must have shape (batch, 16)")
    if move_penalty and not bool((params_t[:, 15] > 0).all()):
        raise ValueError("move_penalty needs dcost > 0 (column 15 of params_t) for every problem")
    if warm_start not in (0, 1, 2) or (warm_start and guess_t is None):
        raise ValueError("warm_start 1/2 needs guess_t")
    if guess_t is not None and not (guess_t.device == dev and guess_t.dtype == torch.float64 and guess_t.is_contiguous()
                                    and tuple(guess_t.shape) == (rows, B)):
        raise ValueError(f"guess_t must be a contiguous float64 tensor of shape {(rows, B)} on {dev}")
    tf = buf("tf", (B,), torch.float64)
    status = buf("status", (B,), torch.int32)
    iters = buf("iters", (B,), torch.int32)
    traj = buf("traj", (10, nt, B), torch.float64) if want_traj else None
    blob = buf("blob", (rows, B), torch.float64) if want_blob else None
    if (sensitivity or flight) and blob is None:
        blob = torch.empty((rows, B), dtype=torch.float64, device=dev)
    sens = buf("sensitivity", (B, 16), torch.float64) if sensitivity else None
    if flight:
        fsum, ftraj = buf("flight_summary", (B, len(FLIGHT_ROWS)), torch.float64), buf("flight_traj", (B, 10, nt), torch.float64)
        floc = buf("flight_local", (B, nt - 1, 7), torch.float64)
    o = _opts(nt, max_iter, tol, warm_start, mu_init, scheme, formulation, coarse_nodes, terminal, path, move_penalty)
    stream = torch.cuda.current_stream(dev).cuda_stream
    _lib.check(L.ascent_solve_batch(params_t.data_ptr(), B, C.byref(o),
                                    guess_t.data_ptr() if guess_t is not None else None,
                                    traj.data_ptr() if traj is not None else None, tf.data_ptr(), status.data_ptr(),
                                    iters.data_ptr(), blob.data_ptr() if blob is not None else None,
                                    dev.index or 0, C.c_void_p(stream), 1))
    if sensitivity:
        g = torch.empty((16, B), dtype=torch.float64, device=dev)
        _lib.check(L.ascent_param_sensitivity(params_t.data_ptr(), B, C.byref(o), blob.data_ptr(), g.data_ptr(),
                                              dev.index or 0, C.c_void_p(stream), 1))
        J = _penalised_objective(params_t, blob, nt - 1, formulation) if move_penalty else blob[21 * (nt - 1)]
        s_ = g.t() * params_t[:, 11:12]
        s_[:, 11] += J
        sens.copy_(torch.where((status == 0)[:, None], s_, torch.full_like(s_, float("nan"))))
    if flight:
        K = nt - 1
        rs = torch.empty((len(FLIGHT_ROWS), B), dtype=torch.float64, device=dev)
        rt = torch.empty((10, nt, B), dtype=torch.float64, device=dev)
        rl = torch.empty((K, 7, B), dtype=torch.float64, device=dev)
        _lib.check(L.ascent_fly_batch(params_t.data_ptr(), B, C.byref(o), blob.data_ptr(), 0, rt.data_ptr(), rl.data_ptr(),
                                      rs.data_ptr(), dev.index or 0, C.c_void_p(stream), 1))
        ok, nan = status == 0, torch.full((), float("nan"), dtype=torch.float64, device=dev)
        fsum.copy_(torch.where(ok[:, None], rs.t(), nan))
        ftraj.copy_(torch.where(ok[:, None, None], rt.permute(2, 0, 1), nan))
        floc.copy_(torch.where(ok[:, None, None], rl.permute(2, 0, 1), nan))
    if sync:
        torch.cuda.synchronize(dev)
    return out


class _FinalTime:
    fn = None

    @classmethod
    def get(cls):
        if cls.fn is None:
            import torch

            class FinalTime(torch.autograd.Function):
                @staticmethod
                def forward(ctx, params_t, kw):
                    out = solve_batch_torch(params_t.detach().contiguous(), sensitivity=True, want_traj=False,
                                            want_blob=kw.get("move_penalty", False), **kw)
                    T = params_t[:, 11].detach()
                    if kw.get("move_penalty", False):
                        y = T * _penalised_objective(params_t.detach(), out["blob"], kw.get("nt", 200) - 1, kw.get("formulation", 0))
                    else:
                        y = T * out["tf"]
                    y = torch.where(out["status"] == 0, y, torch.full_like(y, float("nan")))
                    ctx.save_for_backward(out["sensitivity"])
                    return y

                @staticmethod
                def backward(ctx, grad_out):
                    (sens,) = ctx.saved_tensors
                    return grad_out[:, None] * sens, None

            cls.fn = FinalTime
        return cls.fn


def final_time(params_t, **solve_kw):
    return _FinalTime.get().apply(params_t, dict(solve_kw))


def default_path(batch: int, nt: int = 200, scheme=0, formulation=0, move_penalty: bool = False, terminal=0) -> str:
    o = _opts(nt, 300, 1e-9, 0, 0.0, scheme, formulation, move_penalty=move_penalty, terminal=terminal)
    code = _lib.load().ascent_default_path(int(batch), C.byref(o))
    return {v: k for k, v in _lib.PATHS.items()}[code]


def last_kernel_ms(device: int = 0) -> float:
    return _lib.load().ascent_last_kernel_ms(device)
```

Measured before the change: 699,500 NLPs/s.

## Address workspace via scalar row base plus 32-bit lane offsets in persistent kernel

Rewrites global workspace accesses in the persistent solver kernel to use a wave-uniform scalar base pointer per row plus a per-lane 32-bit byte offset (URow), so the compiler can emit SGPR-base + VGPR-offset global loads instead of 64-bit per-lane address arithmetic. It also moves the dcost>0 check from a host-side torch reduction (which forces a device sync) into the device init kernels as a new status code. Geometry guards refuse grids whose offsets would overflow 32 bits. The inline asm constraints add compiler fragility, and the reordered node loads change access order.

After: 703,500 NLPs/s, median of 6. About the same (+0.6%).

```diff
diff --git a/include/ascent.h b/include/ascent.h
--- a/include/ascent.h
+++ b/include/ascent.h
@@ -53,7 +53,8 @@
   ASCENT_CONVERGED = 0,
   ASCENT_MAX_ITER = 1,
   ASCENT_LINESEARCH_FAILED = 2,
-  ASCENT_REGULARISATION_FAILED = 3
+  ASCENT_REGULARISATION_FAILED = 3,
+  ASCENT_BAD_DCOST = 4
 };
 
 #define ASCENT_BLOB_ROWS(n_nodes) (21 * ((n_nodes) - 1) + 10)
diff --git a/lunar_module_ascent_trajectory_optimiser_amd/csrc/ascent_dense.hip b/lunar_module_ascent_trajectory_optimiser_amd/csrc/ascent_dense.hip
--- a/lunar_module_ascent_trajectory_optimiser_amd/csrc/ascent_dense.hip
+++ b/lunar_module_ascent_trajectory_optimiser_amd/csrc/ascent_dense.hip
@@ -147,6 +147,7 @@
   sc[X_STATE] = ST_TRIAL; sc[X_FIRST] = 1.0; sc[X_STATUS] = ASCENT_MAX_ITER;
   sc[X_MU] = probe ? probe_mu[p] : ((asked_warm && !warm) ? 0.1 : mu_init);
   sc[X_NUP] = 1.0;
+  if (g.dc && !(params[p].dcost > 0.0)) { sc[X_STATE] = ST_DONE; sc[X_STATUS] = ASCENT_BAD_DCOST; }
 }
 
 struct QMap { int q; double c; };
diff --git a/lunar_module_ascent_trajectory_optimiser_amd/csrc/ascent_persist.hip b/lunar_module_ascent_trajectory_optimiser_amd/csrc/ascent_persist.hip
--- a/lunar_module_ascent_trajectory_optimiser_amd/csrc/ascent_persist.hip
+++ b/lunar_module_ascent_trajectory_optimiser_amd/csrc/ascent_persist.hip
@@ -124,6 +124,7 @@
   put_scal(sc, X_S, s);
   sc[X_STATE] = ST_TRIAL; sc[X_FIRST] = 1.0; sc[X_STATUS] = ASCENT_MAX_ITER;
   sc[X_MU] = (asked_warm && !warm) ? 0.1 : mu_init; sc[X_NUP] = 1.0;
+  if (g.mp && !(params[p].dcost > 0.0)) { sc[X_STATE] = ST_DONE; sc[X_STATUS] = ASCENT_BAD_DCOST; }
   if (probe) { sc[X_MU] = probe_mu[p]; sc[X_PDW] = probe_dw[p]; sc[X_PROBE] = (double)probe_kind; }
 }
 
@@ -186,6 +187,7 @@
   sc[X_STATE] = ST_TRIAL; sc[X_FIRST] = 1.0; sc[X_STATUS] = ASCENT_MAX_ITER;
   sc[X_MU] = warm ? mu : 0.1; sc[X_NUP] = 1.0;
   sc[X_ITB] = scc[X_ITB] + scc[X_ITERS];
+  if (gf.mp && !(params[p].dcost > 0.0)) { sc[X_STATE] = ST_DONE; sc[X_STATUS] = ASCENT_BAD_DCOST; }
 }
 
 constexpr int FIN_WAVES = 8, FIN_SUB = CH / FIN_WAVES;
@@ -297,8 +299,8 @@
 struct TrialKeep { double G[8], F[7], dza, dzm, zb4, zb5, zpp, zpn; };
 
 template <int SCHEME, int FORM, int MP = 0, int TERM = 0>
-ASC_DEV void trial_primal(const Der &d, int K, int Kp, int k, const NodeIn &n, const NodeIn &dn, const TrialCtx &t, bool live,
-                          double *in, Part &P, TrialKeep &kp) {
+ASC_DEV void trial_primal(const Der &d, int K, size_t rb, int k, const NodeIn &n, const NodeIn &dn, const TrialCtx &t, bool live,
+                          double *in, unsigned &on, Part &P, TrialKeep &kp) {
   const double alpha = t.alpha;
   double z[7], zp[7], zb[6];
   ASC_UNROLL
@@ -311,11 +313,13 @@
     zb[b] = t.first ? n.zb[b] : fmin(fmax(n.zb[b] + t.adu * dn.zb[b], t.mlo * id), t.mhi * id);
   }
   if (live) {
+    URow r(in);
     ASC_UNROLL
-    for (int i = 0; i < 7; i++) in[(O_Z + i) * Kp + k] = z[i];
-    in[O_U * Kp + k] = u;
+    for (int i = 0; i < 7; i++) { r.st(on, z[i]); r.next(rb); }
+    r.st(on, u);
+    r.next(rb, O_ZB - O_U);
     ASC_UNROLL
-    for (int b = 0; b < 6; b++) in[(O_ZB + b) * Kp + k] = zb[b];
+    for (int b = 0; b < 6; b++) { r.st(on, zb[b]); r.next(rb); }
   }
   kp.zpp = 0.0; kp.zpn = 0.0;
   if constexpr (MP) {
@@ -323,7 +327,13 @@
     const double ip = rcp(pp), in_ = rcp(pn);
     const double zpp = t.first ? n.zpp : fmin(fmax(n.zpp + t.adu * dn.zpp, t.mlo * ip), t.mhi * ip);
     const double zpn = t.first ? n.zpn : fmin(fmax(n.zpn + t.adu * dn.zpn, t.mlo * in_), t.mhi * in_);
-    if (live) { in[O_PP * Kp + k] = pp; in[O_PN * Kp + k] = pn; in[O_ZP * Kp + k] = zpp; in[O_ZN * Kp + k] = zpn; }
+    if (live) {
+      URow r(in, rb, O_PP);
+      r.st(on, pp); r.next(rb);
+      r.st(on, pn); r.next(rb);
+      r.st(on, zpp); r.next(rb);
+      r.st(on, zpn);
+    }
     const double cu = u - up - pp + pn;
     P.c1 += fabs(cu);
     P.cinf = fmax(P.cinf, fabs(cu));
@@ -368,12 +378,13 @@
 }
 
 template <int SCHEME, int FORM, int MP = 0, int TERM = 0>
-ASC_DEV void trial_dual(const Der &d, int K, int Kp, int k, const TrialKeep &kp, const double *l, const double *ln, double lu, double lun,
-                        const TrialCtx &t, bool live, double *in, Part &P) {
+ASC_DEV void trial_dual(const Der &d, int K, size_t rb, int k, const TrialKeep &kp, const double *l, const double *ln, double lu, double lun,
+                        const TrialCtx &t, bool live, double *in, unsigned &on, Part &P) {
   if (live) {
+    URow q(in, rb, O_L);
     ASC_UNROLL
-    for (int i = 0; i < 7; i++) in[(O_L + i) * Kp + k] = l[i];
-    if constexpr (MP) in[O_LU * Kp + k] = lu;
+    for (int i = 0; i < 7; i++) { q.st(on, l[i]); q.next(rb); }
+    if constexpr (MP) { q.next(rb, O_LU - O_ZB); q.st(on, lu); }
   }
   if constexpr (MP) {
     P.l1 += fabs(lu);
@@ -396,8 +407,9 @@
   if (k == K - 1) {
     const Scal &stt = t.stt;
     double z[7];
+    URow q(in);
     ASC_UNROLL
-    for (int i = 0; i < 7; i++) z[i] = in[(O_Z + i) * Kp + k];
+    for (int i = 0; i < 7; i++) { z[i] = q.ld(on); q.next(rb); }
     if constexpr (TERM == 2) {
       const Terminal tt = terminal_eval_any(d, z);
       double g4[4];
@@ -419,15 +431,15 @@
 }
 
 template <int SCHEME, int FORM, int MP = 0, int TERM = 0>
-ASC_DEV void trial_node(const Der &d, int K, int Kp, int k, const NodeIn &n, const NodeIn &dn, const TrialCtx &t, bool live,
-                        double *in, Part &P) {
+ASC_DEV void trial_node(const Der &d, int K, size_t rb, int k, const NodeIn &n, const NodeIn &dn, const TrialCtx &t, bool live,
+                        double *in, unsigned &on, Part &P) {
   TrialKeep kp;
-  trial_primal<SCHEME, FORM, MP, TERM>(d, K, Kp, k, n, dn, t, live, in, P, kp);
+  trial_primal<SCHEME, FORM, MP, TERM>(d, K, rb, k, n, dn, t, live, in, on, P, kp);
   double l[7], ln[7];
   ASC_UNROLL
   for (int i = 0; i < 7; i++) { l[i] = n.l[i] + t.alpha * dn.l[i]; ln[i] = n.ln[i] + t.alpha * dn.ln[i]; }
   const double lu = MP ? n.lu + t.alpha * dn.lu : 0.0, lun = MP ? n.lun + t.alpha * dn.lun : 0.0;
-  trial_dual<SCHEME, FORM, MP, TERM>(d, K, Kp, k, kp, l, ln, lu, lun, t, live, in, P);
+  trial_dual<SCHEME, FORM, MP, TERM>(d, K, rb, k, kp, l, ln, lu, lun, t, live, in, on, P);
 }
 
 
@@ -451,13 +463,17 @@
   const long p = WIDE ? (long)blockIdx.x : (long)blockIdx.x * NPW + grp;
   const bool live = p < batch;
   const long pc = live ? p : batch - 1;
-  const int K = g.K, Kp = g.Kp, nch = g.nch;
-  double *w = ws + (size_t)pc * g.nlp_doubles();
-  double *gsc = w + (size_t)NROWS * Kp;
+  const int K = g.K, nch = g.nch;
+  const unsigned Kp = g.Kp;
+  const size_t nlpd = g.nlp_doubles(), rb = (size_t)Kp * sizeof(double);
+  double *wb = ws + (size_t)(WIDE ? pc : (long)blockIdx.x * NPW) * nlpd;
+  unsigned og = WIDE ? 0u : (unsigned)(pc - (long)blockIdx.x * NPW) * (unsigned)(nlpd * sizeof(double));
+  unsigned ow = og + (unsigned)nl * 8u;
+  double *gsc = wb + NROWS * Kp;
   double *sc = lsc[WIDE ? 0 : grp];
   const Der d = TERM == 2 ? derive_t(params[pc], 2) : derive(params[pc]);
   static_assert(TERM == 0 || (TERM == 2 && FORM == 0), "terminal 2 is carried for the current formulation");
-  for (int r = role; r < NSCAL; r += 16) sc[r] = gsc[r];
+  for (int r = role; r < NSCAL; r += 16) { unsigned o = og + (unsigned)r * 8u; sc[r] = URow(gsc).ld(o); }
   if (role < 8) lds_d[grp][2][role] = 0.0;
   wsync();
   if (!live && role == 0) sc[X_STATE] = ST_DONE;
@@ -481,8 +497,10 @@
         const Scal s = lds_scal(sc, X_S), ds = lds_scal(sc, X_D);
         const Scal stt = trial_scal(d, s, ds, alpha, adu, mu, first);
         const int cur = (int)sc[X_CUR];
-        const double *ic = w + (size_t)(cur * NIT) * Kp, *stp = w + (size_t)R_ST * Kp;
-        double *in = w + (size_t)((1 - cur) * NIT) * Kp;
+        double *ic, *in, *stp = wb + R_ST * Kp;
+        unsigned oc, on;
+        buf_ref<WIDE>(wb, ow, (unsigned)cur * NIT * Kp, ic, oc);
+        buf_ref<WIDE>(wb, ow, (unsigned)(1 - cur) * NIT * Kp, in, on);
         const double dt = hT * stt.th, be = dt * d.alpha;
         const double mlo = mu * 1e-10, mhi = mu * 1e10;
         Part P;
@@ -494,13 +512,14 @@
           t.alpha = alpha; t.adu = adu; t.mlo = mlo; t.mhi = mhi; t.dt = dt; t.be = be; t.hT = hT; t.first = first; t.stt = stt; t.dcw = dcw;
           P.clear();
           for (int c = 0; c < nch; c++) {
+            const unsigned cb = (unsigned)c * CHN;
             const int k = c * CHN + nl;
             if (k < K) {
               NodeIn n, dn;
-              load_node<MP>(ic, Kp, K, k, n, UINIT);
+              load_node<MP>(ic + cb, rb, K, k, oc, n, UINIT);
               if (first) dn = NodeIn{};
-              else load_node<MP>(stp, Kp, K, k, dn);
-              trial_node<SCHEME, FORM, MP, TERM>(d, K, Kp, k, n, dn, t, live, in, P);
+              else load_node<MP>(stp + cb, rb, K, k, ow, dn);
+              trial_node<SCHEME, FORM, MP, TERM>(d, K, rb, k, n, dn, t, live, in + cb, on, P);
             }
           }
           P.template reduceW<MP, WIDE>();
@@ -575,7 +594,9 @@
       const bool act = state == ST_FACTOR;
       const Scal s = lds_scal(sc, X_S);
       const double mu = sc[X_MU], dw = sc[X_DW];
-      const double *it = w + (size_t)((int)sc[X_CUR] * NIT) * Kp;
+      double *it;
+      unsigned oc;
+      buf_ref<WIDE>(wb, ow, (unsigned)(int)sc[X_CUR] * NIT * Kp, it, oc);
       const double dt = hT * s.th, be = dt * d.alpha, ith = rcp(s.th), cs = SCHEME == 1 ? 0.5 * dt : dt;
       const double ha = 0.5 * d.aub, bu = FORM == 1 ? ha : be;
       const double hTc = SCHEME == 1 ? 0.5 * hT : hT;
@@ -615,7 +636,7 @@
       int bad = 0;
       double zK[7];
       ASC_UNROLL
-      for (int i = 0; i < 7; i++) zK[i] = it[(O_Z + i) * Kp + K - 1];
+      for (int i = 0; i < 7; i++) { unsigned o = oc - (unsigned)nl * 8u; zK[i] = URow(it + (K - 1), rb, O_Z + i).ld(o); }
       const Terminal tm = TERM == 2 ? terminal_eval_any(d, zK) : terminal_eval(d, zK);
       const double is1 = rcp(s.s1), is2 = rcp(s.s2);
       const double sig1 = s.zs1 * is1 + dw, sig2 = s.zs2 * is2 + dw;
@@ -646,7 +667,7 @@
           const int k = c * CHN + nl;
           if (k < K && act) {
             NodeIn n;
-            load_node<MP>(it, Kp, K, k, n, UINIT);
+            load_node<MP>(it + (unsigned)c * CHN, rb, K, k, oc, n, UINIT);
             double G[8], E[4], H[10], F[7], fl[7], lt[7], ax, ay;
             ASC_UNROLL
             for (int i = 0; i < 7; i++) lt[i] = SCHEME == 1 ? n.l[i] + n.ln[i] : n.l[i];
@@ -703,12 +724,13 @@
         if (probe_rows) {
           const int k = c * CHN + nl;
           if (k < K && act && live) {
-            ASC_UNROLL
-            for (int i = 0; i < 8; i++) w[(size_t)(R_ST + i) * Kp + k] = stage[(S_G + i) * LDW + col];
-            ASC_UNROLL
-            for (int i = 0; i < 10; i++) w[(size_t)(R_ST + 8 + i) * Kp + k] = stage[(S_H + i) * LDW + col];
-            ASC_UNROLL
-            for (int i = 0; i < 7; i++) w[(size_t)(R_ST + 18 + i) * Kp + k] = stage[(S_C + i) * LDW + col];
+            URow r(wb + (unsigned)c * CHN, rb, R_ST);
+            ASC_UNROLL
+            for (int i = 0; i < 8; i++) { r.st(ow, stage[(S_G + i) * LDW + col]); r.next(rb); }
+            ASC_UNROLL
+            for (int i = 0; i < 10; i++) { r.st(ow, stage[(S_H + i) * LDW + col]); r.next(rb); }
+            ASC_UNROLL
+            for (int i = 0; i < 7; i++) { r.st(ow, stage[(S_C + i) * LDW + col]); r.next(rb); }
           }
           wsync();
           continue;
@@ -835,8 +857,9 @@
           const int k = c * CHN + nl;
           if (k < K && act) {
             if (live) {
-              ASC_UNROLL
-              for (int i = 0; i < NS + 3; i++) w[(size_t)(R_KA + i) * Kp + k] = outb[i * LDW + col];
+              URow r(wb + (unsigned)c * CHN, rb, R_KA);
+              ASC_UNROLL
+              for (int i = 0; i < NS + 3; i++) { r.st(ow, outb[i * LDW + col]); r.next(rb); }
             }
             const double k00 = outb[NS * LDW + col], k01 = outb[(NS + 1) * LDW + col], k02 = outb[(NS + 2) * LDW + col], D = outb[(NS + 3) * LDW + col];
             const double Dk1 = D * k01, Dk2 = D * k02;
@@ -892,8 +915,11 @@
       const Scal s = lds_scal(sc, X_S);
       const double mu = sc[X_MU], dw = sc[X_DWL], dth = sc[X_DTH], dnu3 = sc[X_DNU3];
       const double sig1 = sc[X_SIG1], sig2 = sc[X_SIG2], rs1 = sc[X_RS1], rs2 = sc[X_RS2];
-      const double *it = w + (size_t)((int)sc[X_CUR] * NIT) * Kp;
-      double *stp = w + (size_t)R_ST * Kp;
+      const int cur = (int)sc[X_CUR];
+      double *it, *in, *stp = wb + R_ST * Kp;
+      unsigned oc, on;
+      buf_ref<WIDE>(wb, ow, (unsigned)cur * NIT * Kp, it, oc);
+      buf_ref<WIDE>(wb, ow, (unsigned)(1 - cur) * NIT * Kp, in, on);
       const double dt = hT * s.th, be = dt * d.alpha, cs = SCHEME == 1 ? 0.5 * dt : dt, hTc = SCHEME == 1 ? 0.5 * hT : hT;
       const double ha = 0.5 * d.aub, bu = FORM == 1 ? ha : be;
       const double tau = fmax(0.99, 1.0 - mu);
@@ -905,8 +931,9 @@
         double rmax = 0.0, gsum = 0.0, adu = 1.0, gmove = 0.0, clu = 0.0;
         double dzK[7] = {0, 0, 0, 0, 0, 0, 0};
         for (int c = 0; c < nch; c++) {
+          const unsigned cb = (unsigned)c * CHN;
           const int kn = c * CHN + nl;
-          const bool on = kn < K && act;
+          const bool on_ = kn < K && act;
           double a_ = 0.5, m_ = 0.5, u_ = 0.0, zb[6] = {1, 1, 1, 1, 1, 1};
           double G[8], Gp[8], E[4], x0[7], ka[NS], du00 = 0.0;
           double x0u = 0.0, pp_ = 1.0, pn_ = 1.0, zpp_ = 0.0, zpn_ = 0.0, lu_ = 0.0;
@@ -914,21 +941,33 @@
           for (int i = 0; i < 7; i++) x0[i] = 0.0;
           ASC_UNROLL
           for (int i = 0; i < NS; i++) ka[i] = 0.0;
-          if (on) {
+          if (on_) {
             double z[7], zp[7], F[7], ax, ay;
-            ASC_UNROLL
-            for (int i = 0; i < 7; i++) { z[i] = it[(O_Z + i) * Kp + kn]; zp[i] = kn > 0 ? it[(O_Z + i) * Kp + kn - 1] : 0.0; }
-            u_ = it[O_U * Kp + kn];
+            URow r(it + cb);
+            double up_ = UINIT;
+            ASC_UNROLL
+            for (int i = 0; i < 7; i++) { z[i] = r.ld(oc); zp[i] = kn > 0 ? r.ld(oc, -1) : 0.0; r.next(rb); }
+            u_ = r.ld(oc);
+            if constexpr (MP) up_ = kn > 0 ? r.ld(oc, -1) : UINIT;
+            r.next(rb, O_ZB - O_U);
             a_ = z[IA]; m_ = z[IM];
             ASC_UNROLL
-            for (int b = 0; b < 6; b++) zb[b] = it[(O_ZB + b) * Kp + kn];
-            ASC_UNROLL
-            for (int i = 0; i < NS; i++) ka[i] = w[(size_t)(R_KA + i) * Kp + kn];
+            for (int b = 0; b < 6; b++) { zb[b] = r.ld(oc); r.next(rb); }
             if constexpr (MP) {
-              pp_ = it[O_PP * Kp + kn]; pn_ = it[O_PN * Kp + kn]; zpp_ = it[O_ZP * Kp + kn]; zpn_ = it[O_ZN * Kp + kn]; lu_ = it[O_LU * Kp + kn];
-              x0u = -(u_ - (kn > 0 ? it[O_U * Kp + kn - 1] : UINIT) - pp_ + pn_);
-            }
-            du00 = w[(size_t)R_K0 * Kp + kn] + w[(size_t)(R_K0 + 1) * Kp + kn] * dth + w[(size_t)(R_K0 + 2) * Kp + kn] * dnu3;
+              lu_ = r.ld(oc); r.next(rb);
+              pp_ = r.ld(oc); r.next(rb);
+              pn_ = r.ld(oc); r.next(rb);
+              zpp_ = r.ld(oc); r.next(rb);
+              zpn_ = r.ld(oc);
+              x0u = -(u_ - up_ - pp_ + pn_);
+            }
+            URow q(wb + cb, rb, R_KA);
+            ASC_UNROLL
+            for (int i = 0; i < NS; i++) { ka[i] = q.ld(ow); q.next(rb); }
+            static_assert(R_K0 == R_KA + NS, "the gain rows are walked in order");
+            const double k00 = q.ld(ow); q.next(rb);
+            const double k01 = q.ld(ow); q.next(rb);
+            du00 = k00 + k01 * dth + q.ld(ow) * dnu3;
             accel<1>(d, z[IX], z[IY], z[IA], z[IM], 0.0, 0.0, ax, ay, G, nullptr);
             rhs_f<FORM>(d, z, u_, ax, ay, F);
             if (SCHEME == 1) {
@@ -954,7 +993,7 @@
           }
           const double dzm_k = carry_m + incl, dzm_p = dzm_k - x0[IM];
           carry_m += WIDE ? __shfl(incl, 63) : bcast16<15>(incl);
-          if (on) {
+          if (on_) {
             const double du00p = du00 - ka[IM] * dzm_p;
             double rvx[7], rvy[7];
             ainv_vrows<FORM>(G, E, cs, rvx, rvy);
@@ -1074,11 +1113,13 @@
               ASC_FTB(adu, zu, dzb[2 * b + 1]);
             }
             if (live) {
-              ASC_UNROLL
-              for (int i = 0; i < 7; i++) stp[(O_Z + i) * Kp + kn] = dzn[i];
-              stp[O_U * Kp + kn] = du;
-              ASC_UNROLL
-              for (int b = 0; b < 6; b++) stp[(O_ZB + b) * Kp + kn] = dzb[b];
+              URow r(stp + cb);
+              ASC_UNROLL
+              for (int i = 0; i < 7; i++) { r.st(ow, dzn[i]); r.next(rb); }
+              r.st(ow, du);
+              r.next(rb, O_ZB - O_U);
+              ASC_UNROLL
+              for (int b = 0; b < 6; b++) { r.st(ow, dzb[b]); r.next(rb); }
             }
             if constexpr (MP) {
               const double du_p = nl > 0 ? outb[7 * LDW + col - 1] : carry_u;
@@ -1095,7 +1136,12 @@
               gmove += dpp + dpn;
               clu -= x0u * (lu_ + dlu);
               if (live) {
-                stp[O_LU * Kp + kn] = dlu; stp[O_PP * Kp + kn] = dpp; stp[O_PN * Kp + kn] = dpn; stp[O_ZP * Kp + kn] = dzp; stp[O_ZN * Kp + kn] = dzn_;
+                URow r(stp + cb, rb, O_LU);
+                r.st(ow, dlu); r.next(rb);
+                r.st(ow, dpp); r.next(rb);
+                r.st(ow, dpn); r.next(rb);
+                r.st(ow, dzp); r.next(rb);
+                r.st(ow, dzn_);
               }
             }
           }
@@ -1109,7 +1155,7 @@
         for (int i = 0; i < 7; i++) dzK[i] = gsumW<WIDE>(dzK[i]);
         double zK[7];
         ASC_UNROLL
-        for (int i = 0; i < 7; i++) zK[i] = it[(O_Z + i) * Kp + K - 1];
+        for (int i = 0; i < 7; i++) { unsigned o = oc - (unsigned)nl * 8u; zK[i] = URow(it + (K - 1), rb, O_Z + i).ld(o); }
         const Terminal tmK = TERM == 2 ? terminal_eval_any(d, zK) : terminal_eval(d, zK);
         Scal ds;
         ds.th = dth; ds.nu3 = dnu3;
@@ -1136,7 +1182,6 @@
         tc.alpha = apr; tc.adu = adu; tc.mlo = mu * 1e-10; tc.mhi = mu * 1e10; tc.hT = hT; tc.first = false; tc.dcw = dcw;
         tc.stt = trial_scal(d, s, ds, apr, adu, mu, false);
         tc.dt = hT * tc.stt.th; tc.be = tc.dt * d.alpha;
-        double *in = w + (size_t)((1 - (int)sc[X_CUR]) * NIT) * Kp;
         Part P;
         P.clear();
         const int abase = (role < 7 ? 6 * role : 0) * LDW;
@@ -1145,22 +1190,29 @@
         double lown = 0.0;
         double cl = 0.0, ccl = 0.0;
         for (int c = nch - 1; c >= 0; c--) {
+          const unsigned cb = (unsigned)c * CHN;
           const int kn = c * CHN + nl;
           double ccn[7] = {0, 0, 0, 0, 0, 0, 0};
           TrialKeep kp;
           if (kn < K && act) {
             NodeIn n, dn;
-            load_node<MP>(it, Kp, K, kn, n, UINIT);
-            ASC_UNROLL
-            for (int i = 0; i < 7; i++) { dn.z[i] = stp[(O_Z + i) * Kp + kn]; dn.zp[i] = kn > 0 ? stp[(O_Z + i) * Kp + kn - 1] : 0.0; }
-            dn.u = stp[O_U * Kp + kn];
-            ASC_UNROLL
-            for (int b = 0; b < 6; b++) dn.zb[b] = stp[(O_ZB + b) * Kp + kn];
-            if constexpr (MP) {
-              dn.up = kn > 0 ? stp[O_U * Kp + kn - 1] : 0.0;
-              dn.lu = stp[O_LU * Kp + kn];
-              dn.lun = kn + 1 < K ? stp[O_LU * Kp + kn + 1] : 0.0;
-              dn.pp = stp[O_PP * Kp + kn]; dn.pn = stp[O_PN * Kp + kn]; dn.zpp = stp[O_ZP * Kp + kn]; dn.zpn = stp[O_ZN * Kp + kn];
+            load_node<MP>(it + cb, rb, K, kn, oc, n, UINIT);
+            {
+              URow r(stp + cb);
+              ASC_UNROLL
+              for (int i = 0; i < 7; i++) { dn.z[i] = r.ld(ow); dn.zp[i] = kn > 0 ? r.ld(ow, -1) : 0.0; r.next(rb); }
+              dn.u = r.ld(ow);
+              if constexpr (MP) dn.up = kn > 0 ? r.ld(ow, -1) : 0.0;
+              r.next(rb, O_ZB - O_U);
+              ASC_UNROLL
+              for (int b = 0; b < 6; b++) { dn.zb[b] = r.ld(ow); r.next(rb); }
+              if constexpr (MP) {
+                dn.lu = r.ld(ow); dn.lun = kn + 1 < K ? r.ld(ow, 1) : 0.0; r.next(rb);
+                dn.pp = r.ld(ow); r.next(rb);
+                dn.pn = r.ld(ow); r.next(rb);
+                dn.zpp = r.ld(ow); r.next(rb);
+                dn.zpn = r.ld(ow);
+              }
             }
             const double *dz = dn.z;
             double G[8], E[4], H[10], F[7], fl[7], lt[7], ax, ay;
@@ -1242,7 +1294,7 @@
             }
             ASC_UNROLL
             for (int i = 0; i < 7; i++) stage[(6 * i + 5) * LDW + col] = wv[i];
-            trial_primal<SCHEME, FORM, MP, TERM>(d, K, Kp, kn, n, dn, tc, live, in, P, kp);
+            trial_primal<SCHEME, FORM, MP, TERM>(d, K, rb, kn, n, dn, tc, live, in + cb, on, P, kp);
           }
           wsync();
           PROF(7);
@@ -1268,8 +1320,9 @@
               ccl += ccn[i] * dl[i];
             }
             if (live) {
-              ASC_UNROLL
-              for (int i = 0; i < 7; i++) stp[(O_L + i) * Kp + kn] = dl[i];
+              URow r(stp + cb, rb, O_L);
+              ASC_UNROLL
+              for (int i = 0; i < 7; i++) { r.st(ow, dl[i]); r.next(rb); }
             }
           }
           wsync();
@@ -1280,16 +1333,20 @@
               for (int i = 0; i < 7; i++) lds_c[WIDE ? 0 : grp][i] = dl[i];
             }
             double l[7], ln[7], lu = 0.0, lun = 0.0;
+            URow r(it + cb, rb, O_L);
             ASC_UNROLL
             for (int i = 0; i < 7; i++) {
-              l[i] = it[(O_L + i) * Kp + kn] + tc.alpha * dl[i];
-              ln[i] = (kn + 1 < K ? it[(O_L + i) * Kp + kn + 1] : 0.0) + tc.alpha * dln[i];
+              l[i] = r.ld(oc) + tc.alpha * dl[i];
+              ln[i] = (kn + 1 < K ? r.ld(oc, 1) : 0.0) + tc.alpha * dln[i];
+              r.next(rb);
             }
             if constexpr (MP) {
-              lu = it[O_LU * Kp + kn] + tc.alpha * stp[O_LU * Kp + kn];
-              lun = (kn + 1 < K ? it[O_LU * Kp + kn + 1] : 0.0) + tc.alpha * (kn + 1 < K ? stp[O_LU * Kp + kn + 1] : 0.0);
-            }
-            trial_dual<SCHEME, FORM, MP, TERM>(d, K, Kp, kn, kp, l, ln, lu, lun, tc, live, in, P);
+              r.next(rb, O_LU - O_ZB);
+              const URow q(stp + cb, rb, O_LU);
+              lu = r.ld(oc) + tc.alpha * q.ld(ow);
+              lun = (kn + 1 < K ? r.ld(oc, 1) : 0.0) + tc.alpha * (kn + 1 < K ? q.ld(ow, 1) : 0.0);
+            }
+            trial_dual<SCHEME, FORM, MP, TERM>(d, K, rb, kn, kp, l, ln, lu, lun, tc, live, in + cb, on, P);
           }
           PROF(0);
         }
@@ -1330,7 +1387,7 @@
   wsync();
   PROF_END;
   if (live)
-    for (int r = role; r < NSCAL; r += 16) gsc[r] = sc[r];
+    for (int r = role; r < NSCAL; r += 16) { unsigned o = og + (unsigned)r * 8u; URow(gsc).st(o, sc[r]); }
 }
 
 }
@@ -1343,6 +1400,16 @@
   g.K = K; g.nch = (K + ch - 1) / ch; g.Kp = (g.nch * ch + 15) / 16 * 16;
   g.form = form; g.mp = mp ? 1 : 0; g.term = term == 2 ? 2 : 0; g.wide = wide ? 1 : 0;
   return g;
+}
+
+bool persist_geo_ok(int K, int mp) {
+  for (int wide = 0; wide <= 1; wide++)
+    if (geo_of(K, 0, mp, 0, wide).nlp_doubles() * sizeof(double) * NPW >= ((size_t)1 << 32)) return false;
+  return true;
+}
+static int refuse_geo(const Call &c, int K) {
+  snprintf(c.err, c.errlen, "a grid of %d intervals is beyond the persistent kernel's 32-bit lane offsets (four records of an NLP must stay below 4 GiB)", K);
+  return ASCENT_E_ARG;
 }
 
 static size_t level_doubles(int K, int mp) {
@@ -1396,6 +1463,8 @@
   const long batch = c.batch;
   const int scheme = c.scheme, form = c.form, mp = c.mp, term = c.term;
   hipStream_t stream = c.stream;
+  for (int l = 0; l < nlev; l++)
+    if (scheme != 2 && !persist_geo_ok(levels[l] - 1, mp)) return refuse_geo(c, levels[l] - 1);
   double *region[2] = {ws, (double *)((char *)ws + persist_region1_offset(levels, batch, mp))};
   PGeo g = geo_of(levels[nlev - 1] - 1, form, mp, term, wide, scheme);
   double *w = region[(nlev - 1) & 1];
@@ -1418,6 +1487,7 @@
 }
 
 int persist_probe(const Call &c, bool wide, double *ws, const ProbeIO &io) {
+  if (c.scheme != 2 && !persist_geo_ok(c.K, c.mp)) return refuse_geo(c, c.K);
   const PGeo g = geo_of(c.K, c.form, c.mp, c.term, wide, c.scheme);
   const dim3 ng((unsigned)((g.Kp + WAVE - 1) / WAVE), (unsigned)c.batch);
   hipLaunchKernelGGL(p_init, ng, dim3(WAVE), 0, c.stream, c.dp, c.batch, g, ws, io.iterate, 2, 0.1, io.mu, io.dw, 1);
@@ -1428,6 +1498,7 @@
 }
 
 int persist_probe_rows(const Call &c, bool wide, double *ws, const ProbeIO &io) {
+  if (!persist_geo_ok(c.K, 0)) return refuse_geo(c, c.K);
   const PGeo g = geo_of(c.K, c.form, 0, 0, wide);
   const dim3 ng((unsigned)((g.Kp + WAVE - 1) / WAVE), (unsigned)c.batch);
   hipLaunchKernelGGL(p_init, ng, dim3(WAVE), 0, c.stream, c.dp, c.batch, g, ws, io.iterate, 2, 0.1, io.mu, io.mu, 2);
diff --git a/lunar_module_ascent_trajectory_optimiser_amd/csrc/ascent_persist.hpp b/lunar_module_ascent_trajectory_optimiser_amd/csrc/ascent_persist.hpp
--- a/lunar_module_ascent_trajectory_optimiser_amd/csrc/ascent_persist.hpp
+++ b/lunar_module_ascent_trajectory_optimiser_amd/csrc/ascent_persist.hpp
@@ -11,6 +11,7 @@
 size_t persist_region1_offset(const int *levels, long batch, int mp);
 size_t persist_ws_bytes_nested(const int *levels, int nlev, long batch, int mp);
 size_t persist_level_bytes_used(int K, long batch, int mp);
+bool persist_geo_ok(int K, int mp);
 int persist_run_nested(const Call &c, bool wide, const int *levels, int nlev, double *ws, const SolveIO &io, double tol_coarse,
                        double mu_first, double mu_next);
 
diff --git a/lunar_module_ascent_trajectory_optimiser_amd/csrc/ascent_persist_dev.hpp b/lunar_module_ascent_trajectory_optimiser_amd/csrc/ascent_persist_dev.hpp
--- a/lunar_module_ascent_trajectory_optimiser_amd/csrc/ascent_persist_dev.hpp
+++ b/lunar_module_ascent_trajectory_optimiser_amd/csrc/ascent_persist_dev.hpp
@@ -105,23 +105,46 @@
   double z[7], zp[7], l[7], ln[7], zb[6], u;
   double up, lu, lun, pp, pn, zpp, zpn;
 };
+struct URow {
+  typedef __attribute__((address_space(1))) char gchar;
+  gchar *p;
+  ASC_DEV explicit URow(const double *q) : p((gchar *)q) { asm("" : "+s"(p)); }
+  ASC_DEV URow(const double *q, size_t rb, int row) : p((gchar *)q + rb * row) { asm("" : "+s"(p)); }
+  ASC_DEV void next(size_t rb, int rows = 1) { p += rb * rows; asm("" : "+s"(p)); }
+  ASC_DEV double ld(unsigned &off, int dn = 0) const {
+    asm("" : "+v"(off) : "s"(p));
+    return *(const __attribute__((address_space(1))) double *)(p + (size_t)off + dn * 8);
+  }
+  ASC_DEV void st(unsigned &off, double v) const {
+    asm("" : "+v"(off) : "s"(p));
+    *(__attribute__((address_space(1))) double *)(p + (size_t)off) = v;
+  }
+};
+template <int WIDE>
+ASC_DEV void buf_ref(double *wb, unsigned ow, unsigned first, double *&b, unsigned &o) {
+  if constexpr (WIDE) { b = wb + (unsigned)__builtin_amdgcn_readfirstlane((int)first); o = ow; }
+  else { b = wb; o = ow + first * 8u; }
+}
+
+static_assert(O_Z == 0 && O_U == 7 && O_L == 8 && O_ZB == 15 && O_LU == 21 && O_PP == 22 && O_PN == 23 && O_ZP == 24 && O_ZN == 25, "rows are walked in order");
 template <int MP = 0>
-ASC_DEV void load_node(const double *it, int Kp, int K, int k, NodeIn &n, double uinit = 0.0) {
+ASC_DEV void load_node(const double *ub, size_t rb, int K, int k, unsigned &off, NodeIn &n, double uinit = 0.0) {
+  URow r(ub);
   ASC_UNROLL
-  for (int i = 0; i < 7; i++) {
-    n.z[i] = it[(O_Z + i) * Kp + k];
-    n.l[i] = it[(O_L + i) * Kp + k];
-    n.zp[i] = k > 0 ? it[(O_Z + i) * Kp + k - 1] : 0.0;
-    n.ln[i] = k + 1 < K ? it[(O_L + i) * Kp + k + 1] : 0.0;
-  }
-  n.u = it[O_U * Kp + k];
+  for (int i = 0; i < 7; i++) { n.z[i] = r.ld(off); n.zp[i] = k > 0 ? r.ld(off, -1) : 0.0; r.next(rb); }
+  n.u = r.ld(off);
+  if constexpr (MP) n.up = k > 0 ? r.ld(off, -1) : uinit;
+  r.next(rb);
   ASC_UNROLL
-  for (int b = 0; b < 6; b++) n.zb[b] = it[(O_ZB + b) * Kp + k];
+  for (int i = 0; i < 7; i++) { n.l[i] = r.ld(off); n.ln[i] = k + 1 < K ? r.ld(off, 1) : 0.0; r.next(rb); }
+  ASC_UNROLL
+  for (int b = 0; b < 6; b++) { n.zb[b] = r.ld(off); r.next(rb); }
   if constexpr (MP) {
-    n.up = k > 0 ? it[O_U * Kp + k - 1] : uinit;
-    n.lu = it[O_LU * Kp + k];
-    n.lun = k + 1 < K ? it[O_LU * Kp + k + 1] : 0.0;
-    n.pp = it[O_PP * Kp + k]; n.pn = it[O_PN * Kp + k]; n.zpp = it[O_ZP * Kp + k]; n.zpn = it[O_ZN * Kp + k];
+    n.lu = r.ld(off); n.lun = k + 1 < K ? r.ld(off, 1) : 0.0; r.next(rb);
+    n.pp = r.ld(off); r.next(rb);
+    n.pn = r.ld(off); r.next(rb);
+    n.zpp = r.ld(off); r.next(rb);
+    n.zpn = r.ld(off);
   }
 }
 
diff --git a/lunar_module_ascent_trajectory_optimiser_amd/csrc/ascent_solver.hip b/lunar_module_ascent_trajectory_optimiser_amd/csrc/ascent_solver.hip
--- a/lunar_module_ascent_trajectory_optimiser_amd/csrc/ascent_solver.hip
+++ b/lunar_module_ascent_trajectory_optimiser_amd/csrc/ascent_solver.hip
@@ -500,6 +500,8 @@
   if (!o || !out4 || batch <= 0 || o->n_nodes < 3) return ASCENT_E_ARG;
   int levels[8];
   const int nlev = nested_levels(o, levels), mp = (int)o->move_penalty;
+  for (int l = 0; l < nlev; l++)
+    if (!persist_geo_ok(levels[l] - 1, mp)) { snprintf(g_err, sizeof g_err, "a grid of %d nodes is beyond the persistent kernel's 32-bit lane offsets", levels[l]); return ASCENT_E_ARG; }
   out4[0] = (int64_t)persist_ws_bytes_nested(levels, nlev, (long)batch, mp);
   out4[1] = (int64_t)persist_level_bytes_used(levels[0] - 1, (long)batch, mp);
   out4[2] = nlev > 1 ? (int64_t)persist_region1_offset(levels, (long)batch, mp) : 0;
diff --git a/lunar_module_ascent_trajectory_optimiser_amd/distributed.py b/lunar_module_ascent_trajectory_optimiser_amd/distributed.py
--- a/lunar_module_ascent_trajectory_optimiser_amd/distributed.py
+++ b/lunar_module_ascent_trajectory_optimiser_amd/distributed.py
@@ -20,6 +20,8 @@
     import torch
     P = pack(params)
     n = P.shape[0]
+    if kw.get("move_penalty") and not (P[:, 15] > 0).all():
+        raise ValueError("move_penalty needs dcost > 0 (column 15 of the parameter sets) for every problem")
     dist = _dist()
     rank, world = (dist.get_rank(), dist.get_world_size()) if dist else (0, 1)
     if device is None:
diff --git a/lunar_module_ascent_trajectory_optimiser_amd/solver.py b/lunar_module_ascent_trajectory_optimiser_amd/solver.py
--- a/lunar_module_ascent_trajectory_optimiser_amd/solver.py
+++ b/lunar_module_ascent_trajectory_optimiser_amd/solver.py
@@ -10,7 +10,7 @@
 
 TRAJ_FIELDS = ("x", "y", "xdot", "ydot", "xdoubledot", "ydoubledot", "angle", "angledot",
                "angledoubledot", "mass")
-STATUS_NAMES = {0: "converged", 1: "max_iter", 2: "linesearch_failed", 3: "regularisation_failed"}
+STATUS_NAMES = {0: "converged", 1: "max_iter", 2: "linesearch_failed", 3: "regularisation_failed", 4: "bad_dcost"}
 
 
 def blob_rows(nt: int) -> int:
@@ -517,8 +517,6 @@
         return t
     if params_t.dim() != 2 or params_t.shape[1] != 16:
         raise ValueError("params_t must have shape (batch, 16)")
-    if move_penalty and not bool((params_t[:, 15] > 0).all()):
-        raise ValueError("move_penalty needs dcost > 0 (column 15 of params_t) for every problem")
     if warm_start not in (0, 1, 2) or (warm_start and guess_t is None):
         raise ValueError("warm_start 1/2 needs guess_t")
     if guess_t is not None and not (guess_t.device == dev and guess_t.dtype == torch.float64 and guess_t.is_contiguous()
```
